# danieljfarrell/pvtrace

Measured on AMD Instinct MI355X. Metric: photons/sec on 5x5x1 cm Lumogen-F-Red LSC, higher is better.
Workload: dtype f64

## Files before the change

include/pvtrace_hip.h:

```cpp
#ifndef PVTRACE_HIP_H
#define PVTRACE_HIP_H

#include <stdint.h>

#ifdef __cplusplus
extern "C" {
#endif

#define PVT_ABI_VERSION 13

#define PVT_MAX_NODES 128
#define PVT_MAX_RECORDERS 256
#define PVT_MAX_HITS 512

enum {
    PVT_EV_GENERATE = 0, PVT_EV_REFLECT = 1, PVT_EV_TRANSMIT = 2, PVT_EV_ABSORB = 3,
    PVT_EV_NONRADIATIVE = 4, PVT_EV_SCATTER = 5, PVT_EV_EMIT = 6, PVT_EV_EXIT = 7,
    PVT_EV_REACT = 8, PVT_EV_KILL = 9
};
enum { PVT_GEOM_BOX = 0, PVT_GEOM_SPHERE = 1, PVT_GEOM_CYLINDER = 2, PVT_GEOM_MESH = 3 };
enum { PVT_SURF_FRESNEL = 0, PVT_SURF_NULL = 1 };
enum { PVT_COMP_ABSORBER = 0, PVT_COMP_SCATTERER = 1, PVT_COMP_LUMINOPHORE = 2, PVT_COMP_REACTOR = 3 };
enum { PVT_PHASE_ISOTROPIC = 0, PVT_PHASE_HG = 1, PVT_PHASE_CONE = 2,
       PVT_PHASE_LAMBERTIAN = 3,
// ... 213 lines not shown
    double* direction;
    double* normal;
    double* wavelength;
    double* travelled;
    double* duration;
} PvtEventLog;

typedef struct PvtEventRecords {
    int32_t* counts;
    uint64_t* rows;
} PvtEventRecords;

typedef struct PvtScene PvtScene;

int pvt_abi_version(void);
const char* pvt_last_error(void);
int pvt_device_count(void);

int pvt_scene_create(const PvtSceneTables* tables, int device, PvtScene** out);
int pvt_scene_create_ex(const PvtSceneTables* tables, const PvtIndexTables* index_tables, int device, PvtScene** out);
int pvt_scene_create_phase(const PvtSceneTables* tables, const PvtIndexTables* index_tables,
                           const PvtPhaseTables* phase_tables, int device, PvtScene** out);
int pvt_scene_create_rough(const PvtSceneTables* tables, const PvtIndexTables* index_tables,
                           const PvtPhaseTables* phase_tables, const PvtSurfaceTables* surface_tables, int device,
                           PvtScene** out);
int pvt_scene_create_field(const PvtSceneTables* tables, const PvtIndexTables* index_tables,
                           const PvtPhaseTables* phase_tables, const PvtSurfaceTables* surface_tables,
                           const PvtFieldTables* field_tables, int device, PvtScene** out);
int pvt_scene_create_maps(const PvtSceneTables* tables, const PvtIndexTables* index_tables,
                          const PvtPhaseTables* phase_tables, const PvtSurfaceTables* surface_tables,
                          const PvtFieldTables* field_tables, const PvtMapTables* map_tables, int device, PvtScene** out);
int64_t pvt_scene_map_slots(const PvtScene* scene);
int pvt_scene_set_emitter(PvtScene* scene, const PvtEmitterTables* emitter);
void pvt_scene_destroy(PvtScene* scene);

int pvt_trace_device(PvtScene* scene, const PvtRays* rays, const PvtTraceParams* params,
                     const PvtTallies* tallies, const PvtEventLog* log, void* stream);

int pvt_trace_device_records(PvtScene* scene, const PvtRays* rays, const PvtTraceParams* params,
                             const PvtTallies* tallies, const PvtEventRecords* records, void* stream);

int pvt_scene_carry_pending(PvtScene* scene, void* stream);
int pvt_scene_carry_discard(PvtScene* scene, void* stream);
int pvt_scene_trim(PvtScene* scene);

int pvt_unpack_records_device(const PvtEventRecords* records, int64_t n_recorded, int32_t max_events,
                              const PvtEventLog* out, int prefill, void* stream);

int pvt_trace_bundle(const PvtSceneTables* tables, const PvtEmitterTables* emitter,
                     const PvtRays* rays, const PvtTraceParams* params,
                     const PvtTallies* tallies, const PvtEventLog* log, int device,
                     double* kernel_ms);

void pvt_release_cached_memory(void);

int pvt_trace_bundle_multi(const PvtSceneTables* tables, const PvtEmitterTables* emitter,
                           const PvtRays* rays, const PvtTraceParams* params,
                           const PvtTallies* tallies, const PvtEventLog* log,
                           const int* devices, int n_devices, double* kernel_ms);

int pvt_last_multi_reduce(void);

int pvt_shard_range(int64_t n_rays, int shard, int n_shards, int64_t align, int64_t* start, int64_t* stop);

int pvt_emit_device(PvtScene* scene, const PvtTraceParams* params, double* position,
                    double* direction, double* wavelength, void* stream);

int pvt_selftest_math(int fn, const double* x_host, double* y_host, int64_t n, int device);

int pvt_scene_counters(PvtScene* scene, uint64_t* out, int reset);

int pvt_scene_clock(PvtScene* scene, uint64_t* out);

int pvt_scene_launch_span(PvtScene* scene, void* stream, uint64_t* out);

int pvt_scene_launch_info(PvtScene* scene, int32_t* grid, int32_t* block, int32_t* lds_bytes);

enum { PVT_VARIANT_LEAN = 0, PVT_VARIANT_W4 = 1, PVT_VARIANT_GRID = 2, PVT_VARIANT_ROUGH = 3, PVT_VARIANT_MESH = 4 };
int pvt_scene_variant(PvtScene* scene);
int pvt_scene_lean_check(const PvtSceneTables* tables, const PvtIndexTables* index_tables, const PvtPhaseTables* phase_tables,
                         const PvtSurfaceTables* surface_tables, const PvtFieldTables* field_tables,
                         const PvtMapTables* map_tables, int32_t* lean);

int pvt_mesh_bvh_check(const PvtSceneTables* tables, int32_t node, int32_t* n_bvh_nodes,
                       int32_t* n_leaves, int32_t* depth);

int pvt_node_grid_plan(const PvtSceneTables* tables, int32_t* dims, double* lo, double* cell, double* guard,
                       int32_t* odd, uint64_t* masks, int64_t masks_cap);

#ifdef __cplusplus
}
#endif
#endif
```

pvtrace_amd/csrc/pvt_scene_pack.h:

```cpp
#pragma once

namespace {

double cosine_threshold(double crit) {
    if (!(crit < INFINITY)) return -INFINITY;
    auto beyond = [&](double c) { return pvt_acos(c) > crit; };
    if (!beyond(0.0)) return -INFINITY;
    if (beyond(1.0)) return NAN;
    auto bits = [](double v) { uint64_t u; std::memcpy(&u, &v, 8); return u; };
    auto from = [](uint64_t u) { double v; std::memcpy(&v, &u, 8); return v; };
    uint64_t lo = bits(0.0), hi = bits(1.0);
    while (hi - lo > 1) {
        const uint64_t mid = lo + (hi - lo) / 2;
        if (beyond(from(mid))) lo = mid; else hi = mid;
    }
    for (uint64_t k = 1; k <= 1024; k++) {
        if (lo >= k && !beyond(from(lo - k))) return NAN;
        if (hi + k <= bits(1.0) && beyond(from(hi + k))) return NAN;
    }
    return from(hi);
}

bool dev_switch(const char* name) {
    if (!getenv(name)) return false;
// ... 194 lines not shown
                const int n0 = g->n[a];
                int pick = n0;
                for (int v = std::max(1, n0 / 2); v <= std::min(64, 2 * n0 + 1); v++) {
                    if (v == n0) continue;
                    int dims[3] = {g->n[0], g->n[1], g->n[2]};
                    dims[a] = v;
                    if ((long long)dims[0] * dims[1] * dims[2] > kMaxCells) break;
                    const double p = price(dims);
                    if (p < best * 0.98) { best = p; pick = v; }
                }
                g->n[a] = pick;
            }
    }
    g->words = W;
    g->guard = dev_switch("PVT_GRID_DEV_GUARD") ? -1e30 : m;
    file_nodes(g->n, g->cell, g->masks);
    return true;
}

double even_rcp(const double* xs, const double* ys, int n) {
    if (n < 2) return NAN;
    const double w = xs[1] - xs[0];
    if (!(w > 1e-100 && w < 1e100)) return NAN;
    for (int i = 1; i + 1 < n; i++) if (xs[i + 1] - xs[i] != w) return NAN;
    for (int i = 0; i < n; i++) {
        if (ys[i] == 0.0 && std::signbit(ys[i])) return NAN;
        if (!(std::fabs(ys[i]) < 1e100)) return NAN;
        if (i > 0 && ys[i] != ys[i - 1] && std::fabs(ys[i] - ys[i - 1]) < 1e-100) return NAN;
    }
    return 1.0 / w;
}

double even_w(const double* xs, int n, double rcp) {
    if (!(rcp == rcp) || n < 2 || n > (1 << 24)) return NAN;
    const double w = xs[1] - xs[0];
    auto grid = [&](int i) { volatile double prod = (double)i * w; volatile double at = xs[0] + prod; return (double)at; };
    for (int i = 0; i < n; i++)
        if (grid(i) != xs[i]) return NAN;
    auto lands = [&](double x, int want) {
        volatile double diff = x - xs[0];
        volatile double quot = diff * rcp;
        int i = (int)quot;
        i = i < 0 ? 0 : (i > n - 2 ? n - 2 : i);
        double xlo = grid(i);
        if (x < xlo) { i -= 1; xlo = grid(i); }
        double xhi = grid(i + 1);
        if (!(x < xhi)) { i += 1; xlo = xhi; xhi = grid(i + 1); }
        return i == want && xlo <= x && x < xhi;
    };
    for (int i = 0; i < n; i++) {
        const double below = std::nextafter(xs[i], -INFINITY), above = std::nextafter(xs[i], INFINITY);
        if (i > 0 && !lands(below, i - 1)) return NAN;
        if (i > 0 && i < n - 1 && !lands(xs[i], i)) return NAN;
        if (i < n - 1 && !lands(above, i)) return NAN;
    }
    return w;
}

double build_guide(const double* xs, int n, int* guide) {
    if (n < 2 || !(xs[n - 1] > xs[0])) return 0.0;
    const int Kb = n - 1;
    int i = 0;
    for (int b = 0; b <= Kb; b++) {
        const double edge = xs[0] + (double)b * ((xs[n - 1] - xs[0]) / (double)Kb);
        while (i + 1 <= n - 2 && xs[i + 1] <= edge) i++;
        guide[b] = i;
    }
    return (double)Kb / (xs[n - 1] - xs[0]);
}

struct PackedScene {
    Lay lay{};
    std::vector<double> gd;
    std::vector<int> gi;
    int nd_small = 0, ni_small = 0, n_ctab = 0, n_rtab = 0, n_ptab = 0, lazy_root = 0;
    int rough_d = -1;
    std::vector<double> fd;
    std::vector<double> md;
    long long map_slots = 0;
    double lazy_k = 0.0;
    bool exit_observed = false, fuse_exit = false, grid = false, hist_reads_position = false;
    bool lean_ok = false;
    bool lean_even = false;
    int grid_dims[3] = {0, 0, 0};
    std::vector<pvt::BvhNode> bvh_nodes;
    std::vector<pvt::MeshTri> bvh_tris;
    std::vector<int> bvh_roots;
};

int validate_tables(const PvtSceneTables* t, const PvtIndexTables* x, const PvtPhaseTables* ph, const PvtSurfaceTables* rs,
                    const PvtFieldTables* fr, const PvtMapTables* mp) {
    const int N = t->n_nodes, C = t->n_components, R = t->n_recorders, H = t->n_hists, K = t->n_coatings;
    if (t->root_id < 0 || t->root_id >= N) return fail(PVT_ERR_INVALID, "root node out of range");
    for (int n = 0; n < N; n++) {
        const int g = t->geom_type[n];
        if (g < PVT_GEOM_BOX || g > PVT_GEOM_MESH) return fail(PVT_ERR_INVALID, "unknown geometry type");
        if (g != PVT_GEOM_MESH) continue;
        if (!t->mesh_face_start || !t->mesh_face_count || !t->mesh_vertices || !t->mesh_faces || !t->mesh_normals)
            return fail(PVT_ERR_INVALID, "mesh node without mesh tables");
        const long long f0 = t->mesh_face_start[n], fc = t->mesh_face_count[n];
        if (fc <= 0 || f0 < 0 || f0 + fc > t->n_mesh_faces) return fail(PVT_ERR_INVALID, "mesh face range out of bounds");
        if (t->n_mesh_faces >= (1 << 27)) return fail(PVT_ERR_INVALID, "more than 2^27 mesh faces in one scene");
        for (long long k = 3 * f0; k < 3 * (f0 + fc); k++)
            if (t->mesh_faces[k] < 0 || t->mesh_faces[k] >= t->n_mesh_vertices)
                return fail(PVT_ERR_INVALID, "mesh face indexes a missing vertex");
    }
    if (K > 0 && t->n_coat_tables != 0) {
        const int NT = t->n_coat_tables;
        if (NT < 0 || !t->coat_table || !t->ctab_nw || !t->ctab_na || !t->ctab_wl_start || !t->ctab_angle_start ||
            !t->ctab_value_start || !t->ctab_wavelength || !t->ctab_angle || !t->ctab_value)
            return fail(PVT_ERR_INVALID, "coating tables: missing arrays");
        long long total = 0;
        for (int j = 0; j < NT; j++) {
            const long long nw = t->ctab_nw[j], na = t->ctab_na[j];
            const long long w0 = t->ctab_wl_start[j], a0 = t->ctab_angle_start[j], v0 = t->ctab_value_start[j];
            if (nw < 1 || na < 1 || w0 < 0 || a0 < 0 || v0 < 0 || w0 + nw > t->n_ctab_wavelength ||
                a0 + na > t->n_ctab_angle || v0 + nw * na > t->n_ctab_value)
                return fail(PVT_ERR_INVALID, "coating tables: axis or value range out of bounds");
            for (long long i = 0; i < nw; i++)
                if (!std::isfinite(t->ctab_wavelength[w0 + i]) || (i > 0 && !(t->ctab_wavelength[w0 + i] > t->ctab_wavelength[w0 + i - 1])))
                    return fail(PVT_ERR_INVALID, "coating tables: wavelengths must be finite and strictly increasing");
            for (long long i = 0; i < na; i++)
                if (!(t->ctab_angle[a0 + i] >= 0.0 && t->ctab_angle[a0 + i] <= 90.0) || (i > 0 && !(t->ctab_angle[a0 + i] > t->ctab_angle[a0 + i - 1])))
                    return fail(PVT_ERR_INVALID, "coating tables: angles must be strictly increasing, in [0, 90] degrees");
            for (long long i = 0; i < nw * na; i++)
                if (!(t->ctab_value[v0 + i] >= 0.0 && t->ctab_value[v0 + i] <= 1.0))
                    return fail(PVT_ERR_INVALID, "coating tables: values must be in [0, 1]");
            total += nw + na + nw * na;
        }
        if (total > (1ll << 27)) return fail(PVT_ERR_INVALID, "coating tables: more than 2^27 doubles");
        for (int k = 0; k < K; k++)
            if (t->coat_table[k] < -1 || t->coat_table[k] >= NT) return fail(PVT_ERR_INVALID, "coating row names a missing table");
    }
    for (int n = 0; n < N; n++) {
        const double v = t->refractive_index[n];
        if (!(std::isfinite(v) && v > 1e-100 && v < 1e100)) return fail(PVT_ERR_INVALID, "refractive indices must be finite and positive");
    }
    if (x && x->n_tables != 0) {
        const int NT = x->n_tables;
        if (NT < 0 || !x->node_table || !x->table_n || !x->table_start || !x->wavelength || !x->value)
            return fail(PVT_ERR_INVALID, "index tables: missing arrays");
        for (int n = 0; n < N; n++)
            if (x->node_table[n] < -1 || x->node_table[n] >= NT) return fail(PVT_ERR_INVALID, "index tables: node names a missing table");
        long long total = 0;
        for (int j = 0; j < NT; j++) {
            const long long np = x->table_n[j], p0 = x->table_start[j];
            if (np < 1 || p0 < 0 || p0 + np > x->n_points) return fail(PVT_ERR_INVALID, "index tables: point range out of bounds");
            for (long long i = 0; i < np; i++)
                if (!std::isfinite(x->wavelength[p0 + i]) || (i > 0 && !(x->wavelength[p0 + i] > x->wavelength[p0 + i - 1])))
                    return fail(PVT_ERR_INVALID, "index tables: wavelengths must be finite and strictly increasing");
            for (long long i = 0; i < np; i++) {
                const double v = x->value[p0 + i];
                if (!(std::isfinite(v) && v > 1e-100 && v < 1e100)) return fail(PVT_ERR_INVALID, "index tables: values must be finite and positive, in (1e-100, 1e100)");
            }
            total += 2 * np;
        }
        if (total > (1ll << 27)) return fail(PVT_ERR_INVALID, "index tables: more than 2^27 doubles");
    }
    const int NP = ph ? ph->n_tables : 0;
    if (NP < 0 || (NP > 0 && (!ph->comp_table || !ph->table_nw || !ph->table_nmu || !ph->wl_start || !ph->mu_start ||
                              !ph->cdf_start || !ph->wavelength || !ph->mu || !ph->cdf)))
        return fail(PVT_ERR_INVALID, "phase tables: missing arrays");
    for (int c = 0; c < C; c++) {
        const bool tagged = t->comp_phase_type[c] == PVT_PHASE_TABLE;
        if (tagged && NP == 0)
            return fail(PVT_ERR_INVALID, "a component has a tabulated phase function (PVT_PHASE_TABLE): pass its tables to pvt_scene_create_phase");
// ... 592 lines not shown
        for (int n = 0; n < N && inside; n++) {
            if (n == root) continue;
            const double* l2w = t->local_to_world + n * 16;
            const double* gp = t->geom_params + n * 4;
            double radius;
            switch (t->geom_type[n]) {
                case PVT_GEOM_BOX: radius = 0.5 * std::sqrt(gp[0] * gp[0] + gp[1] * gp[1] + gp[2] * gp[2]); break;
                case PVT_GEOM_SPHERE: radius = gp[0]; break;
                case PVT_GEOM_CYLINDER: radius = std::sqrt(gp[1] * gp[1] + 0.25 * gp[0] * gp[0]); break;
                default: radius = INFINITY; break;
            }
            radius *= 1.0 + 1e-12;
            double c[3];
            for (int a = 0; a < 3; a++)
                c[a] = w2l[a * 4] * l2w[3] + w2l[a * 4 + 1] * l2w[7] + w2l[a * 4 + 2] * l2w[11] + w2l[a * 4 + 3];
            if (box) {
                for (int a = 0; a < 3; a++)
                    if (!(0.5 * rp[a] - std::fabs(c[a]) - radius > margin)) inside = false;
            } else {
                if (!(rp[0] - std::sqrt(c[0] * c[0] + c[1] * c[1] + c[2] * c[2]) - radius > margin)) inside = false;
            }
        }
        if (inside) {
            p->lazy_root = box ? 1 : 2;
            p->lazy_k = box ? 0.0 : 1.0 / (2.0 * rp[0]);
        }
    }
    if (p->lazy_root && N == 2 && !getenv("PVT_NO_FUSED_EXIT")) {
        const int child = 1 - root;
        bool ok = t->geom_type[child] == PVT_GEOM_BOX && unrotated(t, child) && t->comp_count[root] == 0;
        for (int r = 0; r < R; r++)
            if (t->rec_node[r] == root) ok = false;
        p->fuse_exit = ok;
    }
}

void prove_lean(const PvtSceneTables* t, PackedScene* p) {
    const Lay& lay = p->lay;
    const std::vector<double>& gd = p->gd;
    const std::vector<int>& gi = p->gi;
    const int N = t->n_nodes, R = t->n_recorders;
    bool all_even = true;
    auto nearly_even = [&](int at, int n) {
        const double x0 = gd[(size_t)at], step = (gd[(size_t)at + n - 1] - x0) / (double)(n - 1);
        if (!(step > 0.0) || !std::isfinite(step)) return false;
        for (int i = 0; i < n; i++)
            if (!(std::fabs(gd[(size_t)at + i] - (x0 + (double)i * step)) <= 1e-9 * step)) return false;
        return true;
    };
    auto grid_kind = [&](int at, int n, double w) { return (n == 1 || w == w) ? 2 : (nearly_even(at, n) ? 1 : 0); };
    bool ok = t->n_coatings == 0 && p->n_ctab == 0 && p->n_rtab == 0 && p->n_ptab == 0 && p->rough_d < 0 && p->fd.empty() &&
              p->md.empty() && p->bvh_nodes.empty() && !p->grid && lay.by_node == 1 && R <= 64;
    for (int n = 0; n < N && ok; n++) {
        unsigned long long bits;
        std::memcpy(&bits, &gd[(size_t)n * ND + ND_BITS], 8);
        const bool ident = (bits & 1ull) != 0;
        const int geom = (int)(((unsigned int)bits >> 8) & 0xffu), rot_class = (int)(unsigned int)(bits >> 32);
        const int* q = gi.data() + n * NI;
        const bool shape_ok = geom == PVT_GEOM_BOX || (geom == PVT_GEOM_SPHERE && n == t->root_id);
        if (!ident || !shape_ok || rot_class != 0 || q[NI_KCOUNT] != 0 || q[NI_CCOUNT] > 2) ok = false;
        for (int k = 0; k < q[NI_CCOUNT] && ok; k++) {
            const int* ci = gi.data() + lay.comp_i + (q[NI_CREC] + k) * CI;
            const double* cd = gd.data() + lay.comp_d + (q[NI_CREC] + k) * CD;
            const bool luminophore = ci[CI_TYPE] == PVT_COMP_LUMINOPHORE;
            if (!luminophore && ci[CI_TYPE] != PVT_COMP_ABSORBER) ok = false;
            if (ci[CI_PHASE] != PVT_PHASE_ISOTROPIC) ok = false;
            const int ka = ci[CI_ABS_HIST] != 0 ? 0 : grid_kind(ci[CI_ABS_X], ci[CI_ABS_N], cd[CD_ABS_W]);
            const int ke = !luminophore ? 2 : (ci[CI_EMS_HIST] != 0 ? 0 : grid_kind(ci[CI_EMS_X], ci[CI_EMS_N], cd[CD_EMS_W]));
            if (ka == 0 || ke == 0) ok = false;
            if (ka != 2 || ke != 2) all_even = false;
        }
    }
    for (int block = 0; block < N * 7 && ok; block++) {
        const int* rec = gi.data() + lay.cand_i + block * 8;
        for (int b = 0; b < 6; b++)
            if (rec[2 + b] >= 0 && !(rec[2 + b] & kRecPlain)) ok = false;
        for (int j = 0; j < rec[1]; j++)
            if (!(gi[(size_t)lay.cand_list + rec[0] + j] & kRecPlain)) ok = false;
    }
    p->lean_ok = ok;
    p->lean_even = ok && all_even;
}

void pack_fields(const PvtSceneTables* t, const PvtFieldTables* fr, PackedScene* p) {
    p->fd.clear();
    if (!fr || fr->n_nodes == 0) return;
    const int N = t->n_nodes;
    bool any = false;
    for (int n = 0; n < N; n++) any = any || fr->node_field[n] >= 0;
    if (!any) return;
    std::vector<double>& fd = p->fd;
    fd.assign((size_t)N, -1.0);
    for (int n = 0; n < N; n++) {
        const int f = fr->node_field[n];
        if (f < 0) continue;
        fd[(size_t)n] = (double)fd.size();
        const size_t at = fd.size();
        fd.resize(at + kFrComp + (size_t)t->comp_count[n], 0.0);
        double* r = fd.data() + at;
        for (int a = 0; a < 3; a++) {
            const double lo = fr->field_lower[f * 3 + a], hi = fr->field_upper[f * 3 + a];
            const int na = fr->field_shape[f * 3 + a];
            r[kFrShape + a] = (double)na;
            r[kFrLower + a] = lo;
            r[kFrH + a] = (hi - lo) / (double)na;
            for (int c = 0; c < 3; c++) r[kFrRot + a * 3 + c] = t->world_to_local[n * 16 + a * 4 + c];
            r[kFrT + a] = t->world_to_local[n * 16 + a * 4 + 3];
        }
    }
    std::vector<long long> value_at((size_t)fr->n_values, -1);
    for (int n = 0; n < N; n++) {
        if (fr->node_field[n] < 0) continue;
        const size_t at = (size_t)fd[(size_t)n];
        for (int k = 0; k < t->comp_count[n]; k++) {
            const int v = fr->comp_values[t->comp_start[n] + k];
            if (value_at[(size_t)v] < 0) {
                value_at[(size_t)v] = (long long)fd.size();
                const double* src = fr->values + fr->values_start[v];
                fd.insert(fd.end(), src, src + fr->values_count[v]);
            }
            fd[at + kFrComp + (size_t)k] = (double)value_at[(size_t)v];
        }
    }
}

void pack_maps(const PvtSceneTables* t, const PvtMapTables* mp, PackedScene* p) {
    p->md.clear();
    p->map_slots = 0;
    if (!mp || mp->n_nodes == 0 || mp->n_maps == 0) return;
    const int N = t->n_nodes;
    std::vector<double>& md = p->md;
    md.assign((size_t)N, -1.0);
    for (int n = 0; n < N; n++) {
        const int count = mp->node_map_count[n];
        if (count == 0) continue;
        md[(size_t)n] = (double)md.size();
        const size_t at = md.size();
        md.resize(at + kMnRec + (size_t)count * kMr, 0.0);
        double* r = md.data() + at;
        r[kMnCount] = (double)count;
        for (int a = 0; a < 3; a++) {
            for (int c = 0; c < 3; c++) r[kMnRot + a * 3 + c] = t->world_to_local[n * 16 + a * 4 + c];
            r[kMnT + a] = t->world_to_local[n * 16 + a * 4 + 3];
        }
        for (int k = 0; k < count; k++) {
            const int m = mp->node_map_start[n] + k;
            double* q = r + kMnRec + k * kMr;
            q[kMrKind] = (double)mp->map_kind[m];
            q[kMrComp] = (double)mp->map_component[m];
            for (int a = 0; a < 3; a++) {
                q[kMrShape + a] = (double)mp->map_shape[m * 3 + a];
                q[kMrLower + a] = mp->map_lower[m * 3 + a];
                q[kMrH + a] = mp->map_h[m * 3 + a];
            }
            q[kMrNw] = (double)mp->map_nw[m];
            q[kMrWlo] = mp->map_wl_start[m];
            q[kMrWhi] = mp->map_wl_stop[m];
            q[kMrOff] = (double)mp->map_offset[m];
        }
    }
    p->map_slots = mp->map_slots;
}

int pack_scene(const PvtSceneTables* t, const PvtIndexTables* x, const PvtPhaseTables* ph, const PvtSurfaceTables* rs,
               const PvtFieldTables* fr, const PvtMapTables* mp, PackedScene* p) {
    int rc = validate_tables(t, x, ph, rs, fr, mp);
    if (rc != PVT_OK) return rc;
    const Classes classes = classify_nodes(t, x);
    Spectra spectra = pool_spectra(t);
    const Records records = component_records(t, ph, spectra, classes.by_node);
    NodeGrid grid;
    p->grid = plan_node_grid(t, &grid);
    for (int a = 0; a < 3; a++) p->grid_dims[a] = p->grid ? grid.n[a] : 0;
    p->n_ctab = t->n_coatings > 0 ? t->n_coat_tables : 0;
    p->n_rtab = 0;
    if (x)
        for (int n = 0; n < t->n_nodes; n++)
            if (x->n_tables > 0 && x->node_table[n] >= 0) p->n_rtab = x->n_tables;
    p->n_ptab = 0;
    if (ph)
        for (int c = 0; c < t->n_components; c++)
            if (ph->n_tables > 0 && ph->comp_table[c] >= 0) p->n_ptab = ph->n_tables;
    p->rough_d = -1;
    if (rs && rs->n_nodes > 0)
        for (int n = 0; n < t->n_nodes; n++)
            if (rs->node_roughness[n] > 0.0) p->rough_d = 0;
    std::vector<int> rtab_at, ptab_at;
    const std::vector<int> ctab_at = lay_out(t, x, ph, classes, spectra, records, grid, p, &rtab_at, &ptab_at);
    rc = fill(t, x, ph, rs, classes, spectra, records, grid, ctab_at, rtab_at, ptab_at, p);
    if (rc != PVT_OK) return rc;
    pack_fields(t, fr, p);
    pack_maps(t, mp, p);
    prove_shortcuts(t, p);
    prove_lean(t, p);
    return PVT_OK;
}

}
```

pvtrace_amd/csrc/pvt_trace.hip:

```cpp
#include <hip/hip_runtime.h>

#include <cmath>
#include <cstdio>
#include <cstdlib>
#include <algorithm>
#include <atomic>
#include <cstring>
#include <chrono>
#include <dlfcn.h>
#include <string>
#include <thread>
#include <mutex>
#include <vector>

#include "../../include/pvtrace_hip.h"
#include "pvt_math.h"
#include "pvt_bvh.h"

#include "pvt_trace_kernel.h"

namespace {

thread_local std::string g_error;

// ... 1 lines not shown
    g_error = msg;
    return code;
}
#define HIP_TRY(expr)                                                                     \
    do {                                                                                  \
        hipError_t e_ = (expr);                                                           \
        if (e_ != hipSuccess)                                                             \
            return fail(PVT_ERR_HIP, std::string(#expr) + ": " + hipGetErrorString(e_)); \
    } while (0)

#if PVT_TIMELINE
constexpr int kTlLaunches = 48, kTlWgs = 1024;
constexpr size_t kTlBytes = (size_t)kTlLaunches * kTlWgs * kWaves * 8 * 8;
unsigned long long* g_timeline = nullptr;
int g_tl_launch = 0, g_tl_grid[kTlLaunches] = {0};
long long g_tl_n[kTlLaunches] = {0};
void timeline_dump();
#endif

template <class T>
int push(std::vector<T>& blob, const T* src, size_t n) {
    int at = (int)blob.size();
    if (n && src) blob.insert(blob.end(), src, src + n);
    return at;
}

}

#include "pvt_scene_pack.h"

struct PvtScene {
    int device = 0;
    Lay lay{};
    EmitOff eoff{};
    int nd = 0, ni = 0;
    int nd_small = 0, ni_small = 0;
    int n_nodes = 0, root = 0, n_rec = 0, total_bins = 0, n_coat = 0, n_ctab = 0, n_rtab = 0, n_lights = 0;
    int rough_d = -1;
    double* d_fd = nullptr;
    double* d_md = nullptr;
    long long map_slots = 0;
    double* d_gd = nullptr;
    int* d_gi = nullptr;
    double* d_ed = nullptr;
    int* d_ei = nullptr;
    pvt::BvhNode* d_bvh = nullptr;
    pvt::MeshTri* d_tris = nullptr;
    pvt::BvhNode* d_bvh_top = nullptr;
    int top_n = 0;
    int meshq = 0;
    unsigned int* d_set_cursor = nullptr;
    unsigned long long* d_counters = nullptr;
    unsigned long long* d_stamp = nullptr;
    unsigned int* d_cursor = nullptr;
    std::mutex slot_mutex;
    std::vector<hipStream_t> slot_of;
    std::vector<unsigned long long*> stage;
    std::vector<size_t> stage_bytes;
    size_t stage_limit = (size_t)1 << 30;
    struct Carry {
        unsigned long long* buf[2] = {nullptr, nullptr};
        int parity = 0;
        int phase = 0;
        bool pending = false;
        long long bound = 0;
        int maxsteps = 0, emit_method = 0;
    };
    std::vector<Carry> carry;
    std::vector<double*> emit_pool;
    std::vector<size_t> emit_pool_bytes;
    unsigned int carry_cap = 0;
    int num_cu = 0;
    int last_grid = 0, last_lds = 0;
    size_t lds_limit = 0;
    int lazy_root = 0;
    double lazy_k = 0.0;
    bool exit_observed = false;
    bool grid = false;
    int grid_dims[3] = {0, 0, 0};
    bool fuse_exit = false;
    bool hist_reads_position = false;
    bool lean_ok = false;
    bool lean_even = false;
    int last_variant = -1;
};

extern "C" {

int pvt_abi_version(void) { return PVT_ABI_VERSION; }
const char* pvt_last_error(void) { return g_error.c_str(); }

int pvt_device_count(void) {
    int n = 0;
    if (hipGetDeviceCount(&n) != hipSuccess) return 0;
    return n;
}

int pvt_scene_set_emitter(PvtScene* s, const PvtEmitterTables* e) {
    if (!s || !e || e->n_lights <= 0) return fail(PVT_ERR_INVALID, "bad emitter");
    HIP_TRY(hipSetDevice(s->device));
    std::vector<double> ed;
    std::vector<int> ei;
    EmitOff o{};
    const int Lt = e->n_lights;
    o.wl_value = push(ed, e->wl_value, Lt);
    o.pos_param = push(ed, e->pos_param, (size_t)Lt * 3);
    o.dir_param = push(ed, e->dir_param, Lt);
    o.l2w = push(ed, e->light_to_world, (size_t)Lt * 16);
    o.spec_x = push(ed, e->spec_x, e->n_spec);
    o.spec_cdf = push(ed, e->spec_cdf, e->n_spec);
    o.wl_type = push(ei, e->wl_type, Lt);
    o.wl_spec_start = push(ei, e->wl_spec_start, Lt);
    o.wl_spec_n = push(ei, e->wl_spec_n, Lt);
    o.pos_type = push(ei, e->pos_type, Lt);
    o.dir_type = push(ei, e->dir_type, Lt);
    ed.push_back(0.0);
    ei.push_back(0);
    if (s->d_ed) { (void)hipFree(s->d_ed); s->d_ed = nullptr; }
    if (s->d_ei) { (void)hipFree(s->d_ei); s->d_ei = nullptr; }
    HIP_TRY(hipMalloc(&s->d_ed, ed.size() * sizeof(double)));
    HIP_TRY(hipMalloc(&s->d_ei, ei.size() * sizeof(int)));
    HIP_TRY(hipMemcpy(s->d_ed, ed.data(), ed.size() * sizeof(double), hipMemcpyHostToDevice));
    HIP_TRY(hipMemcpy(s->d_ei, ei.data(), ei.size() * sizeof(int), hipMemcpyHostToDevice));
    s->eoff = o;
    s->n_lights = Lt;
    return PVT_OK;
}

void pvt_scene_destroy(PvtScene* s) {
    if (!s) return;
#if PVT_TIMELINE
    timeline_dump();
#endif
    (void)hipSetDevice(s->device);
    if (s->d_gd) (void)hipFree(s->d_gd);
    if (s->d_fd) (void)hipFree(s->d_fd);
    if (s->d_md) (void)hipFree(s->d_md);
    if (s->d_gi) (void)hipFree(s->d_gi);
    if (s->d_ed) (void)hipFree(s->d_ed);
    if (s->d_ei) (void)hipFree(s->d_ei);
    if (s->d_cursor) (void)hipFree(s->d_cursor);
    if (s->d_set_cursor) (void)hipFree(s->d_set_cursor);
    if (s->d_counters) (void)hipFree(s->d_counters);
    if (s->d_stamp) (void)hipFree(s->d_stamp);
    if (s->d_bvh) (void)hipFree(s->d_bvh);
    if (s->d_bvh_top) (void)hipFree(s->d_bvh_top);
    if (s->d_tris) (void)hipFree(s->d_tris);
    for (auto* b : s->stage) if (b) (void)hipFree(b);
    for (auto& c : s->carry) for (auto* b : c.buf) if (b) (void)hipFree(b);
    for (auto* b : s->emit_pool) if (b) (void)hipFree(b);
    delete s;
}

}

namespace {

KArgs base_args(const PvtScene* s, const PvtTraceParams* p) {
    KArgs a{};
    a.gd = s->d_gd; a.gi = s->d_gi; a.ed = s->d_ed; a.ei = s->d_ei;
    a.bvh = s->d_bvh; a.tris = s->d_tris;
    a.lay = s->lay; a.eoff = s->eoff;
    a.nd = s->nd; a.ni = s->ni;
    a.nd_lds = 0; a.ni_lds = 0;
    a.n_nodes = s->n_nodes; a.root = s->root; a.n_rec = s->n_rec; a.total_bins = s->total_bins;
    a.n_coat = s->n_coat; a.n_ctab = s->n_ctab; a.n_rtab = s->n_rtab; a.n_lights = s->n_lights;
    a.rough_d = s->rough_d;
    a.fd = s->d_fd;
    a.md = s->d_md;
    a.n_rays = (unsigned int)p->n_rays;
    a.cursor = s->d_cursor;
    a.counters = s->d_counters;
    a.seed = p->seed + p->ray_offset;
    a.emit_seed = p->emit_seed;
    a.ray_offset = p->ray_offset;
    a.maxsteps = p->maxsteps; a.max_events = p->max_events; a.emit_method = p->emit_method;
    a.record_every = p->record_every;
    return a;
}

#ifndef PVT_DEV_VARIANTS
#define PVT_DEV_VARIANTS 0
#endif
template <bool RECORD, int TAB_LDS, int SEENW>
hipError_t launch_rough_variant(bool emit, int grid, size_t lds, hipStream_t st, const KArgs& a) {
#if PVT_DEV_VARIANTS
    (void)emit; (void)grid; (void)lds; (void)st; (void)a;
    return hipErrorNotSupported;
#else
    const bool mesh = a.bvh != nullptr;
    if constexpr (TAB_LDS == 1) {
        if (a.lay.grid_d >= 0 && !mesh) {
            if (emit) hipLaunchKernelGGL((trace_kernel_rough_grid<RECORD, SEENW, true>), dim3(grid), dim3(kBlock), lds, st, a);
            else hipLaunchKernelGGL((trace_kernel_rough_grid<RECORD, SEENW, false>), dim3(grid), dim3(kBlock), lds, st, a);
            return hipGetLastError();
        }
    }
    constexpr int MESH_TAB = TAB_LDS == 2 ? 0 : TAB_LDS;
    if (mesh && TAB_LDS == 2) return hipErrorNotSupported;
    if (emit) {
        if (mesh) hipLaunchKernelGGL((trace_kernel_rough<RECORD, MESH_TAB, SEENW, true, true>), dim3(grid), dim3(kBlock), lds, st, a);
        else hipLaunchKernelGGL((trace_kernel_rough_w4<RECORD, TAB_LDS, SEENW, true>), dim3(grid), dim3(kBlock), lds, st, a);
    } else {
        if (mesh) hipLaunchKernelGGL((trace_kernel_rough<RECORD, MESH_TAB, SEENW, false, true>), dim3(grid), dim3(kBlock), lds, st, a);
        else hipLaunchKernelGGL((trace_kernel_rough_w4<RECORD, TAB_LDS, SEENW, false>), dim3(grid), dim3(kBlock), lds, st, a);
    }
    return hipGetLastError();
#endif
}

int variant_of(const PvtScene* s, bool tab_lds) {
    if (s->rough_d >= 0 || s->d_fd || s->d_md) return PVT_VARIANT_ROUGH;
    if (s->d_bvh) return PVT_VARIANT_MESH;
    if (tab_lds && s->lay.grid_d >= 0) return PVT_VARIANT_GRID;
    if (tab_lds && s->lean_ok && s->n_rec <= 64) return PVT_VARIANT_LEAN;
    return PVT_VARIANT_W4;
}

template <bool RECORD>
hipError_t launch_lean_variant(bool even, bool emit, int grid, size_t lds, hipStream_t st, const KArgs& a) {
#if PVT_DEV_VARIANTS
    if (emit || RECORD) return hipErrorNotSupported;
    if (even) hipLaunchKernelGGL((trace_kernel_lean_w4<false, false, true>), dim3(grid), dim3(kBlock), lds, st, a);
    else hipLaunchKernelGGL((trace_kernel_lean_w4<false, false, false>), dim3(grid), dim3(kBlock), lds, st, a);
#else
    if (even) {
        if (emit) hipLaunchKernelGGL((trace_kernel_lean_w4<RECORD, true, true>), dim3(grid), dim3(kBlock), lds, st, a);
        else hipLaunchKernelGGL((trace_kernel_lean_w4<RECORD, false, true>), dim3(grid), dim3(kBlock), lds, st, a);
    } else {
        if (emit) hipLaunchKernelGGL((trace_kernel_lean_w4<RECORD, true, false>), dim3(grid), dim3(kBlock), lds, st, a);
        else hipLaunchKernelGGL((trace_kernel_lean_w4<RECORD, false, false>), dim3(grid), dim3(kBlock), lds, st, a);
    }
#endif
    return hipGetLastError();
}

template <bool RECORD, int TAB_LDS, int SEENW>
hipError_t launch_variant(bool emit, int grid, size_t lds, hipStream_t st, const KArgs& a) {
    if (a.rough_d >= 0 || a.fd != nullptr || a.md != nullptr) return launch_rough_variant<RECORD, TAB_LDS, SEENW>(emit, grid, lds, st, a);
    const bool mesh = a.bvh != nullptr;
    if constexpr (TAB_LDS == 1 && (!PVT_DEV_VARIANTS || SEENW == 1) && PVT_DEV_VARIANTS != 2) {
        if (a.lay.grid_d >= 0 && !mesh && (!PVT_DEV_VARIANTS || !emit)) {
            if (emit && !PVT_DEV_VARIANTS) hipLaunchKernelGGL((trace_kernel_grid<RECORD, SEENW, !PVT_DEV_VARIANTS>), dim3(grid), dim3(kBlock), lds, st, a);
            else hipLaunchKernelGGL((trace_kernel_grid<RECORD, SEENW, false>), dim3(grid), dim3(kBlock), lds, st, a);
            return hipGetLastError();
        }
    }
#if PVT_DEV_VARIANTS == 2
    if (emit || !mesh || TAB_LDS != 1 || SEENW != 1) return hipErrorNotSupported;
    if constexpr (TAB_LDS == 1 && SEENW == 1) hipLaunchKernelGGL((trace_kernel<RECORD, 1, 1, false, true>), dim3(grid), dim3(kBlock), lds, st, a);
#elif PVT_DEV_VARIANTS
    if (emit || mesh || TAB_LDS != 1 || SEENW != 1) return hipErrorNotSupported;
    if constexpr (TAB_LDS == 1 && SEENW == 1) {
        if constexpr (RECORD) hipLaunchKernelGGL((trace_kernel_w4<true, 1, 1, false>), dim3(grid), dim3(kBlock), lds, st, a);
        else hipLaunchKernelGGL((trace_kernel_w4<false, 1, 1, false>), dim3(grid), dim3(kBlock), lds, st, a);
    }
#else
    constexpr int MESH_TAB = TAB_LDS == 2 ? 0 : TAB_LDS;
    if (mesh && TAB_LDS == 2) return hipErrorNotSupported;
    if (emit) {
        if (mesh) hipLaunchKernelGGL((trace_kernel<RECORD, MESH_TAB, SEENW, true, true>), dim3(grid), dim3(kBlock), lds, st, a);
        else if constexpr (RECORD) hipLaunchKernelGGL((trace_kernel_w4<true, TAB_LDS, SEENW, true>), dim3(grid), dim3(kBlock), lds, st, a);
        else hipLaunchKernelGGL((trace_kernel_w4<false, TAB_LDS, SEENW, true>), dim3(grid), dim3(kBlock), lds, st, a);
    } else {
        if (mesh) hipLaunchKernelGGL((trace_kernel<RECORD, MESH_TAB, SEENW, false, true>), dim3(grid), dim3(kBlock), lds, st, a);
        else if constexpr (RECORD) hipLaunchKernelGGL((trace_kernel_w4<true, TAB_LDS, SEENW, false>), dim3(grid), dim3(kBlock), lds, st, a);
        else hipLaunchKernelGGL((trace_kernel_w4<false, TAB_LDS, SEENW, false>), dim3(grid), dim3(kBlock), lds, st, a);
    }
#endif
    return hipGetLastError();
}

template <bool RECORD, int TAB_LDS>
hipError_t launch_seen(int n_rec, int lean, bool emit, int grid, size_t lds, hipStream_t st, const KArgs& a) {
    if constexpr (TAB_LDS == 1 && PVT_DEV_VARIANTS != 2) {
        if (lean) return launch_lean_variant<RECORD>(lean == kLeanEven, emit, grid, lds, st, a);
    }
    if (n_rec <= 64) return launch_variant<RECORD, TAB_LDS, 1>(emit, grid, lds, st, a);
    return launch_variant<RECORD, TAB_LDS, 4>(emit, grid, lds, st, a);
}

}

namespace {

int slot_of_stream(PvtScene* s, hipStream_t st) {
    std::lock_guard<std::mutex> lock(s->slot_mutex);
    size_t slot = 0;
    while (slot < s->slot_of.size() && s->slot_of[slot] != st) slot++;
    if (slot == s->slot_of.size()) {
        if (slot >= (size_t)kCursorSlots) return -1;
        s->slot_of.push_back(st);
        s->stage.push_back(nullptr);
        s->stage_bytes.push_back(0);
        s->carry.emplace_back();
        s->emit_pool.push_back(nullptr);
        s->emit_pool_bytes.push_back(0);
    }
    return (int)slot;
}

int check_trace_args(PvtScene* s, const PvtRays* rays, const PvtTraceParams* p, const PvtTallies* tl) {
    if (!s || !p || !tl) return fail(PVT_ERR_INVALID, "null argument");
    if (p->n_rays < 0 || p->n_rays > 0x7fffffffLL)
        return fail(PVT_ERR_INVALID, "n_rays must fit in 31 bits per bundle");
    if (p->max_events < 2 && p->record_every > 0) return fail(PVT_ERR_INVALID, "max_events must be >= 2");
    if (!rays && !s->d_ed && p->n_rays > 0) return fail(PVT_ERR_INVALID, "no rays and no emitter");
    if ((p->flags & PVT_FLAG_CARRY_OUT) && (p->record_every > 0 || p->tally_bundle > 0))
        return fail(PVT_ERR_INVALID, "PVT_FLAG_CARRY_OUT is for plain tally launches (record_every == 0, no tally sets)");
    if (p->tally_bundle > 0 && p->record_every > 0) return fail(PVT_ERR_INVALID, "tally_bundle needs record_every == 0");
    return PVT_OK;
}

struct LdsPlan { size_t bytes; bool tab_lds, small_lds; int bins_in_lds, xslots, tq_pos; bool ok; };
LdsPlan plan_lds(const PvtScene* s, bool record) {
    LdsPlan lp{0, false, false, 0, 0, 0, true};
    const size_t reserved = (size_t)s->meshq * kBlock * 4 + (size_t)s->top_n * sizeof(pvt::BvhNode);
    const size_t acc_bytes = (size_t)s->n_rec * (8 * 8 + 8) + (size_t)((s->n_rec + 1) & ~1) * 4 + CTL_WORDS * 4;
    const size_t tab_bytes = (size_t)s->nd * 8 + (size_t)((s->ni + 1) & ~1) * 4;
    const size_t bins_bytes = ((size_t)s->total_bins * 4 + 7) & ~(size_t)7;
    const size_t lds_limit = s->lds_limit - reserved;
    const size_t budget = (64 * 1024 < s->lds_limit ? 64 * 1024 : s->lds_limit) - reserved;
    lp.tq_pos = s->hist_reads_position ? 1 : 0;
    const size_t tq_bytes = (size_t)kWaves * kTallyQ * ((lp.tq_pos ? 7 : 4) * 8 + 4);
    if (acc_bytes + tq_bytes > lds_limit) { lp.ok = false; return lp; }
    const char* force = getenv("PVT_TABLES");
    lp.tab_lds = acc_bytes + tq_bytes + tab_bytes <= budget && !force;
    const size_t small_bytes = (size_t)s->nd_small * 8 + (size_t)((s->ni_small + 1) & ~1) * 4;
    lp.small_lds = !lp.tab_lds && s->meshq == 0 && acc_bytes + tq_bytes + small_bytes <= 40 * 1024 && acc_bytes + tq_bytes + small_bytes <= budget &&
                   !(force && force[0] == 'g');
    size_t lds = acc_bytes + tq_bytes + (lp.tab_lds ? tab_bytes : lp.small_lds ? small_bytes : 0);
    lp.bins_in_lds = (lds + bins_bytes <= budget) ? 1 : 0;
    if (lp.bins_in_lds) lds += bins_bytes;
    const size_t xw = 14 + (s->n_rec <= 64 ? 1 : 4) + (record ? 1 : 0);
    const size_t xbytes = (size_t)kXSlots * xw * 8;
    if (s->meshq == 0 && lds + xbytes <= 40 * 1024 && lds + xbytes <= lds_limit) {
        lp.xslots = kXSlots;
        lds += xbytes;
    }
    lp.bytes = (lds + 15) & ~(size_t)15;
    return lp;
}

int trace_launch(PvtScene* s, const PvtRays* rays, const PvtTraceParams* p, const PvtTallies* tl,
                 unsigned long long* log_rows, int* log_counts, hipStream_t st) {
    const int slot = slot_of_stream(s, st);
    if (slot < 0)
        return fail(PVT_ERR_INVALID, "more than 64 HIP streams are tracing this scene; create one scene per group of streams");
    PvtScene::Carry& carry = s->carry[(size_t)slot];
    const bool carry_in = carry.pending;
    if (p->n_rays == 0 && !carry_in) return PVT_OK;
    if (carry_in && (p->record_every > 0 || p->tally_bundle > 0))
        return fail(PVT_ERR_INVALID, "photons parked by the previous launch on this stream (PVT_FLAG_CARRY_OUT) are waiting: "
                                     "finish them with a plain tally launch (n_rays may be 0) first");
    if (carry_in && (p->maxsteps != carry.maxsteps || p->emit_method != carry.emit_method))
        return fail(PVT_ERR_INVALID, "photons parked by the previous launch on this stream were traced with maxsteps " +
                                     std::to_string(carry.maxsteps) + ", emit_method " + std::to_string(carry.emit_method) +
                                     "; this launch asks for " + std::to_string(p->maxsteps) + ", " + std::to_string(p->emit_method) +
// ... 41 lines not shown
    static unsigned long long* g_stats = nullptr;
    if (!g_stats) (void)hipMalloc(&g_stats, 256);
    (void)hipMemsetAsync(g_stats, 0, 256, st);
    a.cursor = reinterpret_cast<unsigned int*>(g_stats);
    a.cursor_next = nullptr;
#endif

    const LdsPlan lp = plan_lds(s, record);
    if (!lp.ok) return fail(PVT_ERR_INVALID, "recorder accumulators exceed LDS");
    a.tq_pos = lp.tq_pos;
    a.bins_in_lds = lp.bins_in_lds;
    a.xslots = lp.xslots;
    const bool tab_lds = lp.tab_lds;
    if (lp.small_lds) { a.nd_lds = s->nd_small; a.ni_lds = s->ni_small; }
    size_t lds = lp.bytes;
    a.meshq_off = -1;
    a.top_off = 0; a.top_n = 0; a.bvh_top = nullptr;
    if (a.bvh) {
        a.meshq_off = (int)lds;
        lds += (size_t)s->meshq * kBlock * 4;
        a.top_off = (int)lds; a.top_n = s->top_n; a.bvh_top = s->d_bvh_top;
        lds += (size_t)s->top_n * sizeof(pvt::BvhNode);
        if (lds > s->lds_limit) return fail(PVT_ERR_INVALID, "mesh staging exceeds LDS");
    }

    long long blocks_for_rays = (p->n_rays + (carry_in ? carry.bound : 0) + kBlock - 1) / kBlock;
    double per_cu = p->workgroups_per_cu > 0 ? (double)p->workgroups_per_cu : 4.0;
    long long grid = (long long)((double)s->num_cu * per_cu);
    if (grid > blocks_for_rays) grid = blocks_for_rays;
    if (grid < 1) grid = 1;
    if (carry_in && grid * kBlock < carry.bound) grid = (carry.bound + kBlock - 1) / kBlock;
    if (n_sets) {
        long long per_set = grid / n_sets;
        const long long for_rays = (p->tally_bundle + kBlock - 1) / kBlock;
        if (per_set > for_rays) per_set = for_rays;
        if (per_set < 1) per_set = 1;
        grid = per_set * n_sets;
        a.set_size = (unsigned int)p->tally_bundle;
        a.wgs_per_set = (int)per_set;
        a.set_stride_i = p->tally_stride_i64;
        a.set_stride_d = p->tally_stride_f64;
    }
    s->last_grid = (int)grid;
    s->last_lds = (int)lds;

    bool carry_out = (p->flags & PVT_FLAG_CARRY_OUT) != 0 && !record && !n_sets;
    if (carry_in || carry_out) {
        if (!s->carry_cap) s->carry_cap = (unsigned int)((long long)s->num_cu * 4 * kBlock);
        if (grid * kBlock > (long long)s->carry_cap) carry_out = false;
        const size_t bytes = (size_t)s->carry_cap * kCarryStride * 8;
        for (int q = 0; q < 2; q++)
            if (!carry.buf[q]) HIP_TRY(hipMalloc(&carry.buf[q], bytes));
        a.carry_cap = s->carry_cap;
        a.carry_in = carry.buf[carry.parity ^ 1];
        a.carry_out = carry.buf[carry.parity];
        a.carry_in_count = blocks + 4 * ((carry.phase + 2) % 3) + 2;
        a.carry_flags = (carry_in ? 1 : 0) | (carry_out ? 2 : 0);
    }

#if PVT_TIMELINE
    if (getenv("PVT_TIMELINE_FILE")) {
        if (!g_timeline) { (void)hipMalloc(&g_timeline, kTlBytes); (void)hipMemset(g_timeline, 0, kTlBytes); }
        const int from = getenv("PVT_TIMELINE_FROM") ? atoi(getenv("PVT_TIMELINE_FROM")) : 0;
        const int k = g_tl_launch++ - from;
        if (k >= 0 && k < kTlLaunches && grid <= kTlWgs) {
            a.timeline = g_timeline + (size_t)k * kTlWgs * kWaves * 8;
            g_tl_grid[k] = (int)grid; g_tl_n[k] = p->n_rays;
        }
    }
#endif
    const bool emit = rays == nullptr && s->d_ed != nullptr;
    if (emit) {
        const size_t need = (size_t)grid * kWaves * 7 * 64 * sizeof(double);
        if (s->emit_pool_bytes[(size_t)slot] < need) {
            if (s->emit_pool[(size_t)slot]) { HIP_TRY(hipStreamSynchronize(st)); (void)hipFree(s->emit_pool[(size_t)slot]); s->emit_pool[(size_t)slot] = nullptr; s->emit_pool_bytes[(size_t)slot] = 0; }
            const size_t bytes = need < ((size_t)s->num_cu * 4 * kWaves * 7 * 64 * sizeof(double)) ? (size_t)s->num_cu * 4 * kWaves * 7 * 64 * sizeof(double) : need;
            HIP_TRY(hipMalloc(&s->emit_pool[(size_t)slot], bytes));
            s->emit_pool_bytes[(size_t)slot] = bytes;
        }
        a.emit_pool = s->emit_pool[(size_t)slot];
    }
    hipError_t e;
    s->last_variant = variant_of(s, tab_lds);
    const int lean = s->last_variant != PVT_VARIANT_LEAN ? kLeanOff : (s->lean_even ? kLeanEven : kLeanSearched);
    if (record) {
        e = tab_lds ? launch_seen<true, 1>(s->n_rec, lean, emit, (int)grid, lds, st, a)
            : lp.small_lds ? launch_seen<true, 2>(s->n_rec, lean, emit, (int)grid, lds, st, a)
                           : launch_seen<true, 0>(s->n_rec, lean, emit, (int)grid, lds, st, a);
    } else {
        e = tab_lds ? launch_seen<false, 1>(s->n_rec, lean, emit, (int)grid, lds, st, a)
            : lp.small_lds ? launch_seen<false, 2>(s->n_rec, lean, emit, (int)grid, lds, st, a)
                           : launch_seen<false, 0>(s->n_rec, lean, emit, (int)grid, lds, st, a);
    }
    if (e != hipSuccess) return fail(PVT_ERR_HIP, std::string("trace_kernel launch: ") + hipGetErrorString(e));
    if (!n_sets) carry.phase = (carry.phase + 1) % 3;
    if (carry_in || carry_out) {
        carry.pending = carry_out;
        carry.bound = carry_out ? grid * kBlock : 0;
        carry.maxsteps = p->maxsteps;
        carry.emit_method = p->emit_method;
        carry.parity ^= 1;
    }
#if PVT_STATS
    {
        unsigned long long c[32];
        (void)hipStreamSynchronize(st);
        (void)hipMemcpy(c, a.cursor, 256, hipMemcpyDeviceToHost);
        fprintf(stderr, "[pvt stats] waves %llu  wave-iterations %llu (drain %llu)  lane-steps %llu (drain %llu)  "
                "mean live lanes/iter %.1f (bulk %.1f, drain %.1f)  iters/wave %.1f (drain %.1f)\n",
                c[5], c[1], c[3], c[2], c[4], (double)c[2] / c[1], (double)(c[2] - c[4]) / (double)(c[1] - c[3] + 1e-9),
                (double)c[4] / (c[3] + 1e-9), (double)c[1] / c[5], (double)c[3] / c[5]);
        fprintf(stderr, "[pvt stats] solo-wave cycles: refill %llu nodes %llu absorb %llu frame %llu trig %llu surface %llu tally %llu (solo waves %llu)\n",
                c[9], c[10], c[11], c[12], c[13], c[14], c[15], c[16]);
        const double bi = (double)(c[1] - c[3]) + 1e-9;
        if (a.lay.grid_d >= 0)
            fprintf(stderr, "[pvt stats] grid walk per wave-iteration: cell rounds %.2f  node-test trips %.2f  (lanes per trip %.1f, lanes per cell round %.1f)\n",
                    (double)c[25] / c[1], (double)c[26] / c[1], (double)c[27] / (c[26] + 1e-9), (double)c[28] / (c[25] + 1e-9));
        if (a.bvh)
            fprintf(stderr, "[pvt stats] mesh walk per wave-iteration: box trips %.2f (lanes per trip %.1f)  triangle trips %.2f (lanes per trip %.1f);  per lane-step: boxes %.2f triangles %.2f\n",
                    (double)c[25] / c[1], (double)c[26] / (c[25] + 1e-9), (double)c[27] / c[1], (double)c[28] / (c[27] + 1e-9),
                    (double)c[26] / c[2], (double)c[28] / c[2]);
        fprintf(stderr, "[pvt stats] bulk lanes/iteration: live %.1f absorbed %.1f re-emitted %.1f surface %.1f exit %.1f terminal-selector %.1f terminal %.1f\n",
                c[17] / bi, c[18] / bi, c[19] / bi, c[20] / bi, c[21] / bi, c[22] / bi, c[23] / bi);
    }
#endif
    return PVT_OK;
}

#if PVT_TIMELINE
void timeline_dump() {
    const char* path = getenv("PVT_TIMELINE_FILE");
    if (!path || !g_timeline) return;
    (void)hipDeviceSynchronize();
    std::vector<unsigned long long> host(kTlBytes / 8);
    (void)hipMemcpy(host.data(), g_timeline, kTlBytes, hipMemcpyDeviceToHost);
    if (FILE* fp = fopen(path, "wb")) {
        for (int k = 0; k < kTlLaunches; k++) {
            if (!g_tl_grid[k]) continue;
            unsigned long long head[4] = {0xABCDull, (unsigned long long)k, (unsigned long long)g_tl_grid[k], (unsigned long long)g_tl_n[k]};
            fwrite(head, 8, 4, fp);
            fwrite(host.data() + (size_t)k * kTlWgs * kWaves * 8, 8, (size_t)g_tl_grid[k] * kWaves * 8, fp);
        }
        fclose(fp);
    }
}
#endif

int unpack_launch(const unsigned long long* rows, const int* counts, long long n_recorded, int max_events,
                  const PvtEventLog* out, bool prefill, hipStream_t st) {
    if (n_recorded <= 0) return PVT_OK;
    const int rays_per_block = max_events >= kBlock ? 1 : kBlock / max_events;
    const long long gx = (n_recorded + rays_per_block - 1) / rays_per_block;
    const int gy = rays_per_block > 1 ? 1 : (max_events + kBlock - 1) / kBlock;
    if (gx > 0x7fffffffLL) return fail(PVT_ERR_INVALID, "too many recorded rays for one unpack launch");
    hipLaunchKernelGGL(unpack_log_kernel, dim3((unsigned)gx, (unsigned)gy), dim3(kBlock), 0, st, rows, counts, *out,
                       n_recorded, max_events, rays_per_block, prefill ? 1 : 0);
    hipError_t e = hipGetLastError();
    if (e != hipSuccess) return fail(PVT_ERR_HIP, std::string("unpack_log_kernel launch: ") + hipGetErrorString(e));
    return PVT_OK;
}

}

extern "C" {

int pvt_scene_create(const PvtSceneTables* t, int device, PvtScene** out) {
    return pvt_scene_create_ex(t, nullptr, device, out);
}

int pvt_scene_create_ex(const PvtSceneTables* t, const PvtIndexTables* x, int device, PvtScene** out) {
    return pvt_scene_create_phase(t, x, nullptr, device, out);
}

int pvt_scene_create_phase(const PvtSceneTables* t, const PvtIndexTables* x, const PvtPhaseTables* ph, int device, PvtScene** out) {
    return pvt_scene_create_rough(t, x, ph, nullptr, device, out);
}

int pvt_scene_create_rough(const PvtSceneTables* t, const PvtIndexTables* x, const PvtPhaseTables* ph,
                           const PvtSurfaceTables* rs, int device, PvtScene** out) {
    return pvt_scene_create_field(t, x, ph, rs, nullptr, device, out);
}

int pvt_scene_create_field(const PvtSceneTables* t, const PvtIndexTables* x, const PvtPhaseTables* ph,
                           const PvtSurfaceTables* rs, const PvtFieldTables* fr, int device, PvtScene** out) {
    return pvt_scene_create_maps(t, x, ph, rs, fr, nullptr, device, out);
}

int64_t pvt_scene_map_slots(const PvtScene* s) { return s ? (int64_t)s->map_slots : 0; }

int pvt_scene_create_maps(const PvtSceneTables* t, const PvtIndexTables* x, const PvtPhaseTables* ph,
                          const PvtSurfaceTables* rs, const PvtFieldTables* fr, const PvtMapTables* mp, int device,
                          PvtScene** out) {
    if (!t || !out) return fail(PVT_ERR_INVALID, "null argument");
    if (t->n_nodes <= 0) return fail(PVT_ERR_INVALID, "scene has no nodes");
    if (t->n_nodes > PVT_MAX_NODES) return fail(PVT_ERR_TOO_MANY_NODES, "more than 128 geometry nodes");
    if (t->n_recorders > PVT_MAX_RECORDERS) return fail(PVT_ERR_INVALID, "more than 256 recorders");
    if (pvt_device_count() <= device) return fail(PVT_ERR_NO_DEVICE, "no such HIP device");
    HIP_TRY(hipSetDevice(device));
    PackedScene packed;
    const int rc = pack_scene(t, x, ph, rs, fr, mp, &packed);
    if (rc != PVT_OK) return rc;

    struct Owner {
        PvtScene* p;
        ~Owner() { if (p) pvt_scene_destroy(p); }
    } owner{new PvtScene()};
    PvtScene* s = owner.p;
    s->stage.reserve(kCursorSlots); s->stage_bytes.reserve(kCursorSlots); s->carry.reserve(kCursorSlots);
    s->emit_pool.reserve(kCursorSlots); s->emit_pool_bytes.reserve(kCursorSlots);
    s->device = device;
    s->lay = packed.lay;
    s->nd = (int)packed.gd.size(); s->ni = (int)packed.gi.size();
    s->nd_small = packed.nd_small; s->ni_small = packed.ni_small;
    s->n_nodes = t->n_nodes; s->root = t->root_id; s->n_rec = t->n_recorders;
    s->total_bins = t->total_bins; s->n_coat = t->n_coatings; s->n_ctab = packed.n_ctab; s->n_rtab = packed.n_rtab;
    s->rough_d = packed.rough_d;
    s->lazy_root = packed.lazy_root; s->lazy_k = packed.lazy_k;
    s->exit_observed = packed.exit_observed; s->fuse_exit = packed.fuse_exit; s->hist_reads_position = packed.hist_reads_position;
    s->grid = packed.grid;
    s->lean_ok = packed.lean_ok && !getenv("PVT_NO_LEAN");
    s->lean_even = s->lean_ok && packed.lean_even;
    for (int a = 0; a < 3; a++) s->grid_dims[a] = packed.grid_dims[a];
    hipDeviceProp_t prop;
    HIP_TRY(hipGetDeviceProperties(&prop, device));
    s->num_cu = prop.multiProcessorCount;
    s->lds_limit = prop.sharedMemPerBlock;
    if (const char* env = getenv("PVT_STAGE_BYTES")) s->stage_limit = (size_t)atoll(env);
    HIP_TRY(hipMalloc(&s->d_gd, packed.gd.size() * sizeof(double)));
    HIP_TRY(hipMalloc(&s->d_gi, packed.gi.size() * sizeof(int)));
    HIP_TRY(hipMalloc(&s->d_cursor, 64 * kCursorSlots + 256));
    HIP_TRY(hipMemset(s->d_cursor, 0, 64 * kCursorSlots + 256));
    HIP_TRY(hipMalloc(&s->d_set_cursor, (size_t)kCursorSlots * kMaxSets * 4));
    HIP_TRY(hipMalloc(&s->d_counters, 64 * 8 * 8));
    HIP_TRY(hipMemset(s->d_counters, 0, 64 * 8 * 8));
    HIP_TRY(hipMalloc(&s->d_stamp, (size_t)kCursorSlots * 2 * 8));
    HIP_TRY(hipMemset(s->d_stamp, 0, (size_t)kCursorSlots * 2 * 8));
    if (!packed.bvh_nodes.empty()) {
        s->meshq = 1;
        for (int r : packed.bvh_roots)
            if (packed.bvh_nodes[r].skip - r > 16) s->meshq = kMeshQ;
        const LdsPlan tally = plan_lds(s, false), hist = plan_lds(s, true);
        const size_t other = (tally.bytes > hist.bytes ? tally.bytes : hist.bytes) + (size_t)s->meshq * kBlock * 4;
        const size_t per_wg = (size_t)39 * 1024 * 4 / kMeshWaves;
        size_t room = tally.ok && hist.ok && other < per_wg ? per_wg - other : 0;
        if (room > 32 * 1024) room = 32 * 1024;
        if (const char* env = getenv("PVT_MESH_TOP_BYTES")) {
            const size_t asked = (size_t)atoll(env);
            room = asked < room ? asked : room;
        }
        std::vector<pvt::BvhNode> top;
        pvt::stage_top(packed.bvh_nodes, packed.bvh_roots, room / sizeof(pvt::BvhNode), top);
        s->top_n = (int)top.size();
        const LdsPlan tally2 = plan_lds(s, false), hist2 = plan_lds(s, true);
        const size_t with_top = (size_t)s->meshq * kBlock * 4 + (size_t)s->top_n * sizeof(pvt::BvhNode);
        if (tally2.ok != tally.ok || hist2.ok != hist.ok || tally2.tab_lds != tally.tab_lds || hist2.tab_lds != hist.tab_lds ||
            tally2.bytes + with_top > s->lds_limit || hist2.bytes + with_top > s->lds_limit)
            return fail(PVT_ERR_INVALID, "internal: the LDS plan of a mesh scene changed when the copy of its trees' top levels was added");
        if (s->top_n > 0) {
            HIP_TRY(hipMalloc(&s->d_bvh_top, top.size() * sizeof(pvt::BvhNode)));
            HIP_TRY(hipMemcpy(s->d_bvh_top, top.data(), top.size() * sizeof(pvt::BvhNode), hipMemcpyHostToDevice));
        }
        packed.bvh_nodes.push_back(pvt::BvhNode{});
        HIP_TRY(hipMalloc(&s->d_bvh, packed.bvh_nodes.size() * sizeof(pvt::BvhNode)));
        HIP_TRY(hipMalloc(&s->d_tris, packed.bvh_tris.size() * sizeof(pvt::MeshTri)));
        HIP_TRY(hipMemcpy(s->d_bvh, packed.bvh_nodes.data(), packed.bvh_nodes.size() * sizeof(pvt::BvhNode), hipMemcpyHostToDevice));
        HIP_TRY(hipMemcpy(s->d_tris, packed.bvh_tris.data(), packed.bvh_tris.size() * sizeof(pvt::MeshTri), hipMemcpyHostToDevice));
    }
    HIP_TRY(hipMemcpy(s->d_gd, packed.gd.data(), packed.gd.size() * sizeof(double), hipMemcpyHostToDevice));
    HIP_TRY(hipMemcpy(s->d_gi, packed.gi.data(), packed.gi.size() * sizeof(int), hipMemcpyHostToDevice));
    if (!packed.fd.empty()) {
        HIP_TRY(hipMalloc(&s->d_fd, packed.fd.size() * sizeof(double)));
        HIP_TRY(hipMemcpy(s->d_fd, packed.fd.data(), packed.fd.size() * sizeof(double), hipMemcpyHostToDevice));
    }
    if (!packed.md.empty()) {
        HIP_TRY(hipMalloc(&s->d_md, packed.md.size() * sizeof(double)));
        HIP_TRY(hipMemcpy(s->d_md, packed.md.data(), packed.md.size() * sizeof(double), hipMemcpyHostToDevice));
        s->map_slots = packed.map_slots;
    }
    owner.p = nullptr;
    *out = s;
    return PVT_OK;
}

int pvt_trace_device_records(PvtScene* s, const PvtRays* rays, const PvtTraceParams* p, const PvtTallies* tl,
                             const PvtEventRecords* rec, void* stream) {
    int rc = check_trace_args(s, rays, p, tl);
    if (rc != PVT_OK) return rc;
    if (p->record_every > 0 && (!rec || !rec->rows || !rec->counts))
        return fail(PVT_ERR_INVALID, "record_every > 0 needs event records");
    return trace_launch(s, rays, p, tl, rec ? reinterpret_cast<unsigned long long*>(rec->rows) : nullptr, rec ? rec->counts : nullptr,
                        reinterpret_cast<hipStream_t>(stream));
}

int pvt_scene_carry_pending(PvtScene* s, void* stream) {
    if (!s) return 0;
    std::lock_guard<std::mutex> lock(s->slot_mutex);
    for (size_t k = 0; k < s->slot_of.size(); k++)
        if (s->slot_of[k] == reinterpret_cast<hipStream_t>(stream)) return s->carry[k].pending ? 1 : 0;
    return 0;
}

int pvt_scene_carry_discard(PvtScene* s, void* stream) {
    if (!s) return fail(PVT_ERR_INVALID, "null scene");
    std::lock_guard<std::mutex> lock(s->slot_mutex);
// ... 98 lines not shown
    hipLaunchKernelGGL(emit_kernel, dim3(grid), dim3(kBlock), 0, reinterpret_cast<hipStream_t>(stream), a,
                       position, direction, wavelength);
    HIP_TRY(hipGetLastError());
    return PVT_OK;
}

int pvt_selftest_math(int fn, const double* x_host, double* y_host, int64_t n, int device) {
    if (!x_host || !y_host || n < 0) return fail(PVT_ERR_INVALID, "bad argument");
    if (n == 0) return PVT_OK;
    if (pvt_device_count() <= device) return fail(PVT_ERR_NO_DEVICE, "no such HIP device");
    HIP_TRY(hipSetDevice(device));
    double *dx = nullptr, *dy = nullptr;
    HIP_TRY(hipMalloc(&dx, (size_t)n * 8));
    HIP_TRY(hipMalloc(&dy, (size_t)n * 8));
    HIP_TRY(hipMemcpy(dx, x_host, (size_t)n * 8, hipMemcpyHostToDevice));
    hipLaunchKernelGGL(math_kernel, dim3((unsigned)((n + kBlock - 1) / kBlock)), dim3(kBlock), 0, nullptr, fn, dx, dy,
                       (long long)n);
    HIP_TRY(hipGetLastError());
    HIP_TRY(hipMemcpy(y_host, dy, (size_t)n * 8, hipMemcpyDeviceToHost));
    (void)hipFree(dx);
    (void)hipFree(dy);
    return PVT_OK;
}

int pvt_scene_counters(PvtScene* s, uint64_t* out, int reset) {
    if (!s || !out) return fail(PVT_ERR_INVALID, "null argument");
    HIP_TRY(hipSetDevice(s->device));
    unsigned long long rows[64 * 8];
    HIP_TRY(hipMemcpy(rows, s->d_counters, sizeof rows, hipMemcpyDeviceToHost));
    for (int k = 0; k < 4; k++) out[k] = 0;
    for (int r = 0; r < 64; r++)
        for (int k = 0; k < 4; k++) out[k] += rows[r * 8 + k];
    if (reset) HIP_TRY(hipMemset(s->d_counters, 0, sizeof rows));
    return PVT_OK;
}

int pvt_scene_clock(PvtScene* s, uint64_t* out) {
    if (!s || !out) return fail(PVT_ERR_INVALID, "null argument");
    HIP_TRY(hipSetDevice(s->device));
    unsigned long long rows[64 * 8];
    HIP_TRY(hipMemcpy(rows, s->d_counters, sizeof rows, hipMemcpyDeviceToHost));
    out[0] = out[1] = 0;
    for (int r = 0; r < 64; r++) { out[0] += rows[r * 8 + 4]; out[1] += rows[r * 8 + 5]; }
    return PVT_OK;
}

int pvt_scene_launch_span(PvtScene* s, void* stream, uint64_t* out) {
    if (!s || !out) return fail(PVT_ERR_INVALID, "null argument");
    HIP_TRY(hipSetDevice(s->device));
    out[0] = out[1] = 0;
    size_t k = 0;
    {
        std::lock_guard<std::mutex> lock(s->slot_mutex);
        while (k < s->slot_of.size() && s->slot_of[k] != reinterpret_cast<hipStream_t>(stream)) k++;
        if (k == s->slot_of.size()) return fail(PVT_ERR_INVALID, "no launch on this stream yet");
    }
    HIP_TRY(hipStreamSynchronize(reinterpret_cast<hipStream_t>(stream)));
    HIP_TRY(hipMemcpy(out, s->d_stamp + 2 * k, 16, hipMemcpyDeviceToHost));
    return PVT_OK;
}

int pvt_scene_launch_info(PvtScene* s, int32_t* grid, int32_t* block, int32_t* lds_bytes) {
    if (!s) return fail(PVT_ERR_INVALID, "null scene");
    if (grid) *grid = s->last_grid;
    if (block) *block = kBlock;
    if (lds_bytes) *lds_bytes = s->last_lds;
    return PVT_OK;
}

int pvt_scene_variant(PvtScene* s) {
    if (!s) return fail(PVT_ERR_INVALID, "null scene");
    if (s->last_variant >= 0) return s->last_variant;
    return variant_of(s, plan_lds(s, false).tab_lds);
}

int pvt_scene_lean_check(const PvtSceneTables* t, const PvtIndexTables* x, const PvtPhaseTables* ph, const PvtSurfaceTables* rs,
                         const PvtFieldTables* fr, const PvtMapTables* mp, int32_t* lean) {
    if (!t || !lean) return fail(PVT_ERR_INVALID, "null argument");
    if (t->n_nodes <= 0 || t->n_nodes > PVT_MAX_NODES || t->n_recorders > PVT_MAX_RECORDERS) return fail(PVT_ERR_INVALID, "bad argument");
    PackedScene packed;
    const int rc = pack_scene(t, x, ph, rs, fr, mp, &packed);
    if (rc != PVT_OK) return rc;
    *lean = packed.lean_ok ? (packed.lean_even ? 2 : 1) : 0;
    return PVT_OK;
}

int pvt_mesh_bvh_check(const PvtSceneTables* t, int32_t node, int32_t* n_bvh_nodes, int32_t* n_leaves,
                       int32_t* depth_out) {
    if (!t || node < 0 || node >= t->n_nodes || t->geom_type[node] != PVT_GEOM_MESH)
        return fail(PVT_ERR_INVALID, "not a mesh node");
    const int f0 = t->mesh_face_start[node], fc = t->mesh_face_count[node];
    if (fc <= 0 || f0 < 0 || f0 + fc > t->n_mesh_faces) return fail(PVT_ERR_INVALID, "mesh face range out of bounds");
    std::vector<pvt::BvhNode> nodes;
    std::vector<pvt::MeshTri> tris;
    double centre[3];
    const int root = pvt::BvhBuilder(t->mesh_vertices, t->mesh_faces, t->mesh_normals, nodes, tris).add_mesh(f0, fc, centre);
    if (root != 0 || nodes.size() < 2 || nodes[0].skip != (int)nodes.size()) return fail(PVT_ERR_INVALID, "root skip link");
    std::vector<int> seen(fc, 0);
    int leaves = 0, records = 0, max_depth = 0;
    struct Open { int id, parent, depth, skip; };
    std::vector<Open> todo{{0, -1, 1, (int)nodes.size()}};
    std::vector<char> visited(nodes.size(), 0);
    while (!todo.empty()) {
        const Open o = todo.back();
        todo.pop_back();
        if (o.id < 0 || o.id >= (int)nodes.size() || visited[o.id]++) return fail(PVT_ERR_INVALID, "child link out of range or shared");
        const pvt::BvhNode& b = nodes[o.id];
        records += 1;
        max_depth = std::max(max_depth, o.depth);
        if (b.skip != o.skip) return fail(PVT_ERR_INVALID, "skip link: a left child's is its sibling, a right child's its parent's");
        for (int a = 0; a < 3; a++) {
            if (!(b.lo[a] <= b.hi[a])) return fail(PVT_ERR_INVALID, "empty box");
            if (o.parent >= 0 && (b.lo[a] < nodes[o.parent].lo[a] || b.hi[a] > nodes[o.parent].hi[a]))
                return fail(PVT_ERR_INVALID, "child box not inside its parent");
        }
        if (b.link < 0) {
            leaves += 1;
            const int tri = b.link & pvt::kIndexMask;
            if (tri >= (int)tris.size()) return fail(PVT_ERR_INVALID, "triangle record out of range");
            const pvt::MeshTri& tr = tris[tri];
            const long long local = tr.face - f0;
            if (local < 0 || local >= fc || seen[local]++) return fail(PVT_ERR_INVALID, "face missing or duplicated");
            for (int c = 0; c < 3; c++)
                for (int a = 0; a < 3; a++) {
                    if (tr.v[3 * c + a] != t->mesh_vertices[3 * (size_t)t->mesh_faces[3 * (size_t)tr.face + c] + a])
                        return fail(PVT_ERR_INVALID, "gathered vertex differs from the table");
                    if (tr.v[3 * c + a] - centre[a] < b.lo[a] || tr.v[3 * c + a] - centre[a] > b.hi[a])
                        return fail(PVT_ERR_INVALID, "triangle outside its leaf box");
                }
        } else {
            const int c = b.link;
            if (c <= o.id || (c & 1) != 0) return fail(PVT_ERR_INVALID, "children not a pair on one 64-byte line after their parent");
            todo.push_back({c + 1, o.id, o.depth + 1, o.skip});
            todo.push_back({c, o.id, o.depth + 1, c + 1});
        }
    }
    for (int k = 0; k < fc; k++) if (seen[k] != 1) return fail(PVT_ERR_INVALID, "face missing from the tree");
    if (records + 1 != (int)nodes.size() || visited[1]) return fail(PVT_ERR_INVALID, "records outside the tree");
    auto replay = [](const std::vector<pvt::BvhNode>& plain, const std::vector<pvt::BvhNode>& staged,
                     const std::vector<pvt::BvhNode>& top, int root) -> const char* {
        const int end = plain[root].skip;
        std::vector<int> cursor_of((size_t)(end - root) + 1, -1);
        cursor_of[(size_t)(end - root)] = end;
        std::vector<int> order;
        int c = pvt::first_cursor(staged, root);
        for (int i = root; i != end; i = pvt::next_cursor(plain[i], true)) {
            if (c == end) return "staged walk ends early";
            if ((c & pvt::kTopFlag) ? (size_t)(c & pvt::kIndexMask) >= top.size() : (c < root || c >= end)) return "cursor out of range";
            if (cursor_of[(size_t)(i - root)] >= 0) return "plain walk visits a record twice";
            cursor_of[(size_t)(i - root)] = c;
            order.push_back(i);
            const pvt::BvhNode& rec = pvt::at_cursor(staged, top, c);
            for (int a = 0; a < 3; a++)
                if (rec.lo[a] != plain[i].lo[a] || rec.hi[a] != plain[i].hi[a]) return "staged walk out of order";
            if ((plain[i].link < 0) != (rec.link < 0) || (plain[i].link < 0 && rec.link != plain[i].link)) return "staged leaf differs";
            c = pvt::next_cursor(rec, true);
            if (order.size() > (size_t)(end - root)) return "plain walk does not end";
        }
        if (c != end) return "staged walk does not end at the tree's end";
        for (int i : order) {
            const pvt::BvhNode& rec = pvt::at_cursor(staged, top, cursor_of[(size_t)(i - root)]);
            if (pvt::next_cursor(rec, false) != cursor_of[(size_t)(plain[i].skip - root)]) return "staged skip link differs";
        }
        return nullptr;
    };
    for (size_t budget : {(size_t)3, (size_t)7, (size_t)64, (size_t)768, nodes.size()}) {
// ... 583 lines not shown
```

pvtrace_amd/csrc/pvt_trace_kernel.h:

```cpp
#pragma once
constexpr int kMeshWaves = 4;
#ifndef PVT_STATS
#define PVT_STATS 0
#endif
#ifndef PVT_TIMELINE
#define PVT_TIMELINE 0
#endif

namespace {

constexpr int kBlock = 256;
constexpr int kChunk = 64;
constexpr int kEndClaim = 64;
constexpr int kClaim = kChunk;
constexpr int kWaves = kBlock / 64;
constexpr int kCursorSlots = 64;
constexpr int kMaxSets = 1024;
constexpr int kRecPlain = 1 << 30;
constexpr int kTallyQ = 64;
constexpr int kXSlots = 72;
enum { CTL_EXHAUSTED = 0, CTL_DONE = 1, CTL_IN = 2, CTL_LIVE = 6, CTL_COUNT = 16, CTL_CLOCK = 22, CTL_WORDS = 26 };
constexpr double kEps = 2.220446049250313e-13;
constexpr double kAlphaZero = 1e-8;
constexpr double kCcm = 2.99792458e10;
// ... 112 lines not shown
    r.s2 = splitmix64(st);
    r.s3 = splitmix64(st);
}
__device__ __forceinline__ double rng_uniform(Rng& r) {
    unsigned long long result = r.s0 + r.s3;
    unsigned long long t = r.s1 << 17;
    r.s2 ^= r.s0;
    r.s3 ^= r.s1;
    r.s1 ^= r.s2;
    r.s0 ^= r.s3;
    r.s2 ^= t;
    r.s3 = (r.s3 << 45) | (r.s3 >> 19);
    const double hi = (double)(unsigned int)(result >> 32), lo = (double)(unsigned int)((unsigned int)result >> 11);
    return __builtin_fma(lo, 1.0 / 9007199254740992.0, hi * (1.0 / 4294967296.0));
}

__device__ __forceinline__ double div_normal(double x, double y) {
    double r = __builtin_amdgcn_rcp(y);
    double e = __builtin_fma(-y, r, 1.0);
    r = __builtin_fma(r, e, r);
    e = __builtin_fma(-y, r, 1.0);
    r = __builtin_fma(r, e, r);
    const double q = x * r;
    e = __builtin_fma(-y, q, x);
    return __builtin_fma(e, r, q);
}
__device__ __forceinline__ double sqrt_normal(double x) {
    const double y = __builtin_amdgcn_rsq(x);
    double g = x * y, h = y * 0.5;
    const double r = __builtin_fma(-h, g, 0.5);
    g = __builtin_fma(g, r, g);
    h = __builtin_fma(h, r, h);
    double d = __builtin_fma(-g, g, x);
    g = __builtin_fma(d, h, g);
    d = __builtin_fma(-g, g, x);
    g = __builtin_fma(d, h, g);
    return __builtin_amdgcn_class(x, 0x260) ? x : g;
}
__device__ __forceinline__ double sqrt1m2_normal(double c) { return sqrt_normal((1.0 - c) * (1.0 + c)); }
__device__ __forceinline__ double rcp_normal(double x) {
    double r = __builtin_amdgcn_rcp(x);
    double e = __builtin_fma(-x, r, 1.0);
    r = __builtin_fma(r, e, r);
    e = __builtin_fma(-x, r, 1.0);
    r = __builtin_fma(r, e, r);
    e = __builtin_fma(-x, r, 1.0);
    return __builtin_fma(e, r, r);
}

typedef const __attribute__((address_space(4))) double* CDoubles;
typedef const __attribute__((address_space(4))) int* CInts;

template <int TAB_LDS>
struct Tables {
    CDoubles gd;
    CInts gi;
    const double* ld;
    const int* li;
    const double* __restrict__ hd;
    const int* __restrict__ hi;
    __device__ __forceinline__ double du(int i) const { return gd[i]; }
    __device__ __forceinline__ int iu(int i) const { return gi[i]; }
    __device__ __forceinline__ double dv(int i) const { return TAB_LDS != 0 ? ld[i] : hd[i]; }
    __device__ __forceinline__ int iv(int i) const { return TAB_LDS != 0 ? li[i] : hi[i]; }
    __device__ __forceinline__ double sd(int i) const { return TAB_LDS == 1 ? ld[i] : hd[i]; }
    __device__ __forceinline__ int si(int i) const { return TAB_LDS == 1 ? li[i] : hi[i]; }
};

struct V3 {
    double x, y, z;
};
__device__ __forceinline__ double dot3(const V3& a, const V3& b) { return a.x * b.x + a.y * b.y + a.z * b.z; }

__device__ __forceinline__ double div_known(double x, double y, double z) {
    double q = x * z;
    double r = __builtin_fma(-q, y, x);
    q = __builtin_fma(r, z, q);
    r = __builtin_fma(-q, y, x);
    return __builtin_fma(r, z, q);
}
constexpr double kRcpCcm = 1.0 / kCcm;

enum { kInterpAny = 0, kInterpEven, kInterpByGuide, kInterpNoHist };
enum { kLeanOff = 0, kLeanSearched, kLeanEven };
template <int TAB_LDS, int KIND = kInterpAny>
__device__ __forceinline__ double interp_clamped(const Tables<TAB_LDS>& T, double x, int xs, int ys, int n,
                                                 int guide, double scale, int hist, double rcp,
                                                 double w = __builtin_nan(""), double yw = __builtin_nan("")) {
    auto end = [&](int i) { return T.sd(i); };
    if (n == 1) return end(ys);
    constexpr bool kAny = KIND == kInterpAny;
    constexpr bool kNoHist = KIND == kInterpNoHist;
    const bool even = KIND == kInterpEven || (kAny && !hist && w == w) || (kNoHist && w == w);
    const double x0 = end(xs), xl = even ? x0 + (double)(n - 1) * w : end(xs + n - 1);
    if (x <= x0) return end(ys);
    if ((kAny && hist) ? x > xl : x >= xl) return (KIND == kInterpByGuide || ((kAny || kNoHist) && yw == yw)) ? end(ys) + (double)(n - 1) * yw : end(ys + n - 1);
    if (even) {
        int i = (int)((x - x0) * rcp);
        double xlo = x0 + (double)i * w, xhi = x0 + (double)(i + 1) * w;
        if (__ballot(x < xlo || !(x < xhi)) != 0ull) {
            if (x < xlo) { i -= 1; xhi = xlo; xlo = x0 + (double)i * w; }
            else if (!(x < xhi)) { i += 1; xlo = xhi; xhi = x0 + (double)(i + 1) * w; }
        }
        const double ylo = T.sd(ys + i), yhi = T.sd(ys + i + 1);
        return ylo + div_known((yhi - ylo) * (x - xlo), xhi - xlo, rcp);
    }
    int b = (int)((x - x0) * scale);
    b = b < 0 ? 0 : (b > n - 2 ? n - 2 : b);
    int lo = T.si(guide + b), hi = T.si(guide + b + 1) + 1;
    if (hi > n - 1) hi = n - 1;
    double xlo = T.sd(xs + lo), xhi = T.sd(xs + hi);
    if (kAny && hist) {
        if (!(xlo < x)) lo = 0;
        if (!(x <= xhi)) hi = n - 1;
        while (hi - lo > 1) {
            const int mid = (lo + hi) >> 1;
            if (T.sd(xs + mid) < x) lo = mid; else hi = mid;
        }
        return T.sd(ys + hi);
    }
    if (__ballot(!(xlo <= x) || !(x < xhi)) != 0ull) {
        if (!(xlo <= x)) { lo = 0; xlo = x0; }
        if (!(x < xhi)) { hi = n - 1; xhi = xl; }
    }
    while (hi - lo > 1) {
        const int mid = (lo + hi) >> 1;
        const double xm = T.sd(xs + mid);
        if (xm <= x) { lo = mid; xlo = xm; } else { hi = mid; xhi = xm; }
    }
    double ylo, yhi;
    if (KIND == kInterpByGuide || ((kAny || kNoHist) && yw == yw)) {
        const double y0 = end(ys);
        ylo = y0 + (double)lo * yw; yhi = y0 + (double)hi * yw;
    } else {
        ylo = T.sd(ys + lo); yhi = T.sd(ys + hi);
    }
    if (xhi == xlo) return ylo;
    const double num = (yhi - ylo) * (x - xlo), width = xhi - xlo;
    return ylo + (rcp == rcp ? div_known(num, width, rcp) : num / width);
}
__device__ __forceinline__ void coat_bracket(const double* xs, int n, double x, int& lo, int& hi, double& t) {
    lo = 0; hi = 0; t = 0.0;
    if (!(x > xs[0])) return;
    if (!(x < xs[n - 1])) { lo = n - 1; hi = n - 1; return; }
    int a = 0, b = n - 1;
    while (b - a > 1) {
        const int m = (a + b) >> 1;
        if (xs[m] <= x) a = m; else b = m;
    }
    const double xa = xs[a];
    lo = a; hi = b; t = (x - xa) / (xs[b] - xa);
}
__device__ __forceinline__ double coat_table_r(const double* wls, int nw, const double* angs, int na, const double* vals,
                                               double wl, double c1) {
    int w0, w1, a0, a1;
    double tw, ta;
    coat_bracket(wls, nw, wl, w0, w1, tw);
    coat_bracket(angs, na, pvt_acos(c1), a0, a1, ta);
    const double* v0 = vals + a0 * nw;
    const double* v1 = vals + a1 * nw;
    const double p0 = v0[w0], r0 = p0 + tw * (v0[w1] - p0);
    const double p1 = v1[w0], r1 = p1 + tw * (v1[w1] - p1);
    return r0 + ta * (r1 - r0);
}
__device__ __attribute__((noinline)) double coat_table_r_call(const double* wls, int nw, const double* angs, int na,
                                                              const double* vals, double wl, double c1) {
    return coat_table_r(wls, nw, angs, na, vals, wl, c1);
// ... 469 lines not shown
}

struct Accum {
    unsigned int* cross;
    unsigned int* distinct;
    double* sums;
    unsigned int* bins;
};

template <int SEENW>
struct Seen {
    unsigned long long w[SEENW];
};

template <bool RECORD, int TAB_LDS, int SEENW, bool MESH, bool GRID, bool ROUGH = false, int LEAN = 0>
__device__ void tail_run(const KArgs* kernel_args, int total, unsigned int lds);

template <int TAB_LDS>
__device__ __attribute__((noinline)) void leave_workgroup(const KArgs* kernel_args) {
    extern __shared__ double smem[];
    const unsigned long long bits = (unsigned long long)kernel_args;
    const unsigned int lo = __builtin_amdgcn_readfirstlane((unsigned int)bits), hi = __builtin_amdgcn_readfirstlane((unsigned int)(bits >> 32));
    const __attribute__((address_space(4))) KArgs* ak = (const __attribute__((address_space(4))) KArgs*)(((unsigned long long)hi << 32) | lo);
    const KArgs& A = *(const KArgs*)ak;
    const int lane = threadIdx.x & 63;
    const int nd_lds = TAB_LDS == 1 ? A.nd : TAB_LDS == 2 ? A.nd_lds : 0;
    const int ni_stage = TAB_LDS == 1 ? A.ni : TAB_LDS == 2 ? A.ni_lds : 0;
    const int ni_lds = (ni_stage + 1) & ~1;
    int* lds_i = reinterpret_cast<int*>(smem + nd_lds);
    double* acc_sums = reinterpret_cast<double*>(lds_i + ni_lds);
    unsigned long long* acc_cross = reinterpret_cast<unsigned long long*>(acc_sums + A.n_rec * 8);
    unsigned int* acc_distinct = reinterpret_cast<unsigned int*>(acc_cross + A.n_rec);
    unsigned int* acc_bins = acc_distinct + ((A.n_rec + 1) & ~1);
    int* ctl = reinterpret_cast<int*>(acc_bins + ((A.bins_in_lds ? A.total_bins : 0) + 1 & ~1));
    const unsigned int set = A.set_size ? blockIdx.x / (unsigned int)A.wgs_per_set : 0u;
    __threadfence_block();
    int order = 0;
    if (lane == 0) order = atomicAdd(&ctl[CTL_DONE], 1);
    order = __builtin_amdgcn_readfirstlane(order);
    if (order != kWaves - 1) return;
    __threadfence_block();
    {
        unsigned long long* ctr = A.counters;
        if (ctr && lane < 4) {
            const unsigned long long* cnt = reinterpret_cast<const unsigned long long*>(ctl + CTL_COUNT);
            const unsigned long long v = lane == 3 ? (unsigned long long)kWaves : cnt[lane];
            if (v) atomicAdd(ctr + (blockIdx.x & 63u) * 8u + lane, v);
        }
        if (lane == 0) {
            const unsigned long long* t0 = reinterpret_cast<const unsigned long long*>(ctl + CTL_CLOCK);
            const unsigned long long real = wall_clock64(), cyc = __builtin_readcyclecounter();
            if (ctr) {
                atomicAdd(ctr + (blockIdx.x & 63u) * 8u + 4u, cyc - t0[1]);
                atomicAdd(ctr + (blockIdx.x & 63u) * 8u + 5u, real - t0[0]);
            }
            if (A.stamp) atomicMax(A.stamp + 1, real);
        }
    }
    unsigned long long* const out_distinct = reinterpret_cast<unsigned long long*>(A.rec_distinct) + (long long)set * A.set_stride_i;
    unsigned long long* const out_crossings = reinterpret_cast<unsigned long long*>(A.rec_crossings) + (long long)set * A.set_stride_i;
    unsigned long long* const out_bins = reinterpret_cast<unsigned long long*>(A.rec_bins) + (long long)set * A.set_stride_i;
    double* const out_sums = A.rec_sums + (long long)set * A.set_stride_d;
    for (int i = lane; i < A.n_rec; i += 64) {
        const unsigned long long c = acc_cross[i];
        const unsigned int d = acc_distinct[i];
        if (c) atomicAdd(out_crossings + i, c);
        if (d) atomicAdd(out_distinct + i, (unsigned long long)d);
    }
    for (int i = lane; i < A.n_rec * 8; i += 64) {
        double v = acc_sums[i];
        if (v != 0.0) atomicAdd(out_sums + i, v);
    }
    if (A.bins_in_lds)
        for (int i = lane; i < A.total_bins; i += 64) {
            unsigned int v = acc_bins[i];
            if (v) atomicAdd(out_bins + i, (unsigned long long)v);
        }
}

template <bool RECORD, int TAB_LDS, int SEENW, bool EMIT, bool MESH, bool GRID = false, bool TAIL = false, bool ROUGH = false,
          int LEAN = 0>
__device__ __forceinline__ void trace_body(const KArgs& A, int tail_total = 0, unsigned int tail_lds = 0u) {
    static_assert(!LEAN || (!MESH && !GRID && !ROUGH && TAB_LDS == 1 && SEENW == 1), "the lean variants: plain scenes only");
    extern __shared__ double smem_of_kernel[];
    double* const smem = TAIL ? (double*)(__attribute__((address_space(3))) double*)(unsigned long long)tail_lds
                              : (double*)smem_of_kernel;
    constexpr int kAbsKind = LEAN == kLeanEven ? kInterpEven : LEAN ? kInterpNoHist : kInterpAny;
    constexpr int kCdfKind = LEAN == kLeanEven ? kInterpByGuide : LEAN ? kInterpNoHist : kInterpAny;
    auto held = [](int v) __attribute__((always_inline)) -> int {
        if constexpr (TAIL) asm volatile("" : "+s"(v));
        return v;
    };
    const int k_root = held(A.root), k_maxsteps = held(A.maxsteps), k_nodes = held(A.n_nodes);
#if PVT_TIMELINE
    unsigned long long tl_t[6] = {(unsigned long long)wall_clock64(), 0, 0, 0, 0, 0};
    unsigned long long tl_iters = 0;
    const unsigned long long tl_c0 = __builtin_readcyclecounter();
#endif
    Lay L = A.lay;
    if constexpr (TAIL) {
        L.comp_d = held(L.comp_d); L.rec_d = held(L.rec_d); L.hist_d = held(L.hist_d); L.coat_d = held(L.coat_d);
        L.comp_i = held(L.comp_i); L.rec_i = held(L.rec_i); L.hist_i = held(L.hist_i); L.coat_i = held(L.coat_i);
        L.cand_i = held(L.cand_i); L.cand_list = held(L.cand_list); L.crit_d = held(L.crit_d); L.ccrit_d = held(L.ccrit_d);
        L.grid_d = held(L.grid_d); L.rot_d = held(L.rot_d); L.ncls_d = held(L.ncls_d); L.n_cls = held(L.n_cls);
    }
    enum { UF_COATED = 0, UF_FUSE_EXIT, UF_CRIT, UF_HAS_REC, UF_TQ_POS, UF_BINS_LDS, UF_EMIT_FULL, UF_EMIT_KT, UF_LAZY1, UF_LAZY2, UF_BY_NODE,
           UF_TAIL_LAZY1, UF_TAIL_LAZY2, UF_CTAB, UF_DISP, UF_ROUGH, UF_FIELD, UF_VMAP };
    unsigned int uflags_ =
        (A.n_coat > 0 ? 1u << UF_COATED : 0u) | (A.fuse_exit != 0 ? 1u << UF_FUSE_EXIT : 0u) | (L.crit_d >= 0 ? 1u << UF_CRIT : 0u) |
        (A.n_rec > 0 ? 1u << UF_HAS_REC : 0u) | (A.tq_pos ? 1u << UF_TQ_POS : 0u) | (A.bins_in_lds ? 1u << UF_BINS_LDS : 0u) |
        (A.emit_method == PVT_EMIT_FULL ? 1u << UF_EMIT_FULL : 0u) | (A.emit_method == PVT_EMIT_KT ? 1u << UF_EMIT_KT : 0u) |
        (A.lazy_root == 1 ? 1u << UF_LAZY1 : 0u) | (A.lazy_root == 2 ? 1u << UF_LAZY2 : 0u) | (L.by_node ? 1u << UF_BY_NODE : 0u) |
        (A.n_ctab > 0 ? 1u << UF_CTAB : 0u) | (A.n_rtab > 0 ? 1u << UF_DISP : 0u) |
        (ROUGH && A.rough_d >= 0 ? 1u << UF_ROUGH : 0u) |
        (ROUGH && A.fd != nullptr ? 1u << UF_FIELD : 0u) |
        (ROUGH && A.md != nullptr ? 1u << UF_VMAP : 0u);
    if constexpr (TAIL) {
        if (A.lazy_root == 0) uflags_ |= (A.lazy_tail == 1 ? 1u << UF_TAIL_LAZY1 : 0u) | (A.lazy_tail == 2 ? 1u << UF_TAIL_LAZY2 : 0u);
    }
    const unsigned int uflags = uflags_;
    auto uf = [&](int bit) -> bool {
        if constexpr (LEAN != kLeanOff) {
            if (bit == UF_COATED || bit == UF_CTAB || bit == UF_DISP || bit == UF_ROUGH || bit == UF_FIELD || bit == UF_VMAP) return false;
            if (bit == UF_BY_NODE) return true;
        }
        unsigned int f = uflags;
        asm volatile("" : "+s"(f));
        return ((f >> bit) & 1u) != 0u;
    };

    double* lds_d = smem;
    const int nd_lds = TAB_LDS == 1 ? A.nd : TAB_LDS == 2 ? A.nd_lds : 0;
    const int ni_stage = TAB_LDS == 1 ? A.ni : TAB_LDS == 2 ? A.ni_lds : 0;
    const int ni_lds = (ni_stage + 1) & ~1;
    int* lds_i = reinterpret_cast<int*>(lds_d + nd_lds);
    double* acc_sums = reinterpret_cast<double*>(lds_i + ni_lds);
    unsigned long long* acc_cross = reinterpret_cast<unsigned long long*>(acc_sums + A.n_rec * 8);
    unsigned int* acc_distinct = reinterpret_cast<unsigned int*>(acc_cross + A.n_rec);
    unsigned int* acc_bins = acc_distinct + ((A.n_rec + 1) & ~1);
    int* ctl = reinterpret_cast<int*>(acc_bins + ((A.bins_in_lds ? A.total_bins : 0) + 1 & ~1));
    unsigned long long* xbuf = reinterpret_cast<unsigned long long*>(ctl + CTL_WORDS);
    constexpr int kXWords = 14 + SEENW + (RECORD ? 1 : 0);
    const int tq_doubles = A.tq_pos ? 7 : 4;
    double* const tq_d = reinterpret_cast<double*>(xbuf + kXWords * A.xslots) + (threadIdx.x >> 6) * (tq_doubles * kTallyQ);
    int* const tq_r = reinterpret_cast<int*>(reinterpret_cast<double*>(xbuf + kXWords * A.xslots) + kWaves * tq_doubles * kTallyQ)
                      + (threadIdx.x >> 6) * kTallyQ;
    int tq_n = 0;
    if constexpr (!TAIL) {
    if (threadIdx.x < CTL_WORDS) ctl[threadIdx.x] = 0;
    if (blockIdx.x == 0 && threadIdx.x < 4 && A.cursor_next) A.cursor_next[threadIdx.x] = 0u;
    if constexpr (MESH) {
        typedef unsigned int Word4 __attribute__((ext_vector_type(4)));
        Word4* dst = reinterpret_cast<Word4*>(reinterpret_cast<char*>(smem) + A.top_off);
        const Word4* src = reinterpret_cast<const Word4*>(A.bvh_top);
        for (int i = threadIdx.x; i < A.top_n * 2; i += kBlock) dst[i] = src[i];
    }
    if constexpr (TAB_LDS != 0) {
        for (int i = threadIdx.x; i < nd_lds; i += kBlock) lds_d[i] = A.gd[i];
        for (int i = threadIdx.x; i < ni_stage; i += kBlock) lds_i[i] = A.gi[i];
    }
    for (int i = threadIdx.x; i < A.n_rec * 8; i += kBlock) acc_sums[i] = 0.0;
    for (int i = threadIdx.x; i < A.n_rec; i += kBlock) { acc_cross[i] = 0ull; acc_distinct[i] = 0u; }
    if (A.bins_in_lds)
        for (int i = threadIdx.x; i < A.total_bins; i += kBlock) acc_bins[i] = 0u;
    __syncthreads();
    if (threadIdx.x == 0) {
        unsigned long long* t0 = reinterpret_cast<unsigned long long*>(ctl + CTL_CLOCK);
        t0[0] = wall_clock64(); t0[1] = __builtin_readcyclecounter();
        if (blockIdx.x == 0 && A.stamp) A.stamp[0] = t0[0];
    }
    }
#if PVT_TIMELINE
    tl_t[1] = wall_clock64();
#endif

    Tables<TAB_LDS> T{(CDoubles)A.gd, (CInts)A.gi, TAB_LDS != 0 ? lds_d : A.gd, TAB_LDS != 0 ? lds_i : A.gi, A.gd, A.gi};

    auto node_bits = [&](int node) -> unsigned long long { return pvt_d2u(T.dv(node * ND + ND_BITS)); };
    auto node_ident = [](unsigned long long bits) -> bool { return LEAN || (bits & 1ull) != 0; };
    auto node_geom = [](unsigned long long bits) -> int {
        const int g = (int)(((unsigned int)bits >> 8) & 0xffu);
        return LEAN ? (g == PVT_GEOM_SPHERE ? (int)PVT_GEOM_SPHERE : (int)PVT_GEOM_BOX) : g;
    };
    auto node_rot = [&](unsigned long long bits) -> int { return L.rot_d + (int)(unsigned int)(bits >> 32) * RT; };

    auto shape_hits = [](int gt, double g0, double g1, double g2, const V3& o, const V3& d, double inv0, double inv1, double inv2,
                         auto&& fold) __attribute__((always_inline)) {
        if (gt == PVT_GEOM_BOX) {
            double tmin = -INFINITY, tmax = INFINITY;
            bool miss = false;
            const double oo[3] = {o.x, o.y, o.z}, dd[3] = {d.x, d.y, d.z}, gpar[3] = {g0, g1, g2}, inv[3] = {inv0, inv1, inv2};
            if (__ballot(pvt_fabs(dd[0]) < 1e-300 || pvt_fabs(dd[1]) < 1e-300 || pvt_fabs(dd[2]) < 1e-300) == 0ull) {
#pragma unroll
                for (int a = 0; a < 3; a++) {
                    const double sz = gpar[a];
                    const double ta = (-0.5 * sz - oo[a]) * inv[a], tb = (0.5 * sz - oo[a]) * inv[a];
                    tmin = __builtin_fmax(tmin, __builtin_fmin(ta, tb));
                    tmax = __builtin_fmin(tmax, __builtin_fmax(ta, tb));
                }
            } else
#pragma unroll
            for (int a = 0; a < 3; a++) {
                double sz = gpar[a];
                double lo = -0.5 * sz, hi = 0.5 * sz;
                if (pvt_fabs(dd[a]) < 1e-300) {
                    if (oo[a] < lo || oo[a] > hi) miss = true;
                } else {
                    const double ta = (lo - oo[a]) * inv[a], tb = (hi - oo[a]) * inv[a];
                    tmin = __builtin_fmax(tmin, __builtin_fmin(ta, tb));
                    tmax = __builtin_fmin(tmax, __builtin_fmax(ta, tb));
                }
            }
            if (!miss && !(tmax < tmin)) {
                if (tmin > kEps) fold(tmin);
                if (tmax > kEps) fold(tmax);
            }
        } else if (gt == PVT_GEOM_SPHERE) {
            double radius = g0;
            double a = dot3(d, d), b = 2.0 * dot3(d, o), c = dot3(o, o) - radius * radius;
            double disc = b * b - 4.0 * a * c;
            if (!(disc < 0.0)) {
                double sq = pvt_sqrt(disc);
                double t = (-b - sq) / (2.0 * a);
                if (t > kEps) fold(t);
                t = (-b + sq) / (2.0 * a);
                if (t > kEps) fold(t);
            }
        } else {
            double half = 0.5 * g0, radius = g1;
            double a = d.x * d.x + d.y * d.y;
            if (a > 1e-300) {
                double b = 2.0 * (o.x * d.x + o.y * d.y);
                double c = o.x * o.x + o.y * o.y - radius * radius;
                double disc = b * b - 4.0 * a * c;
                if (disc >= 0.0) {
                    double sq = pvt_sqrt(disc);
                    double t = (-b - sq) / (2.0 * a);
                    double z = o.z + t * d.z;
                    if (z > -half && z < half && t > kEps) fold(t);
                    t = (-b + sq) / (2.0 * a);
                    z = o.z + t * d.z;
                    if (z > -half && z < half && t > kEps) fold(t);
                }
            }
            if (pvt_fabs(d.z) > 1e-300) {
                double t = (-half - o.z) / d.z;
                double x = o.x + t * d.x, y = o.y + t * d.y;
                if (x * x + y * y <= radius * radius && t > kEps) fold(t);
                t = (half - o.z) / d.z;
                x = o.x + t * d.x;
                y = o.y + t * d.y;
                if (x * x + y * y <= radius * radius && t > kEps) fold(t);
            }
        }
    };

    const int lane = threadIdx.x & 63;
    auto rank_in = [](unsigned long long mask) -> unsigned int {
        return __builtin_amdgcn_mbcnt_hi((unsigned int)(mask >> 32), __builtin_amdgcn_mbcnt_lo((unsigned int)mask, 0u));
    };

    const unsigned int set = A.set_size ? blockIdx.x / (unsigned int)A.wgs_per_set : 0u;
    const unsigned int ray_lo = set * A.set_size;
    const unsigned int n_local = A.set_size ? (A.n_rays - ray_lo < A.set_size ? A.n_rays - ray_lo : A.set_size) : A.n_rays;
    unsigned int* const cursor = A.cursor + set;

    bool alive = false;
    V3 pos{0, 0, 0}, dir{0, 0, 1};
    double wl = 0.0, travelled = 0.0, duration = 0.0;
    Rng rng{0, 0, 0, 0};
    int count = 0, source = -1, nev = 0;
    unsigned int c_iters = 0u, c_steps = 0u, c_fused = 0u;
    int ac_node = -1;
    unsigned long long ac_wl = 0ull;
    double ac_alpha = 0.0, ac_pre0 = 0.0;
    unsigned long long* const ac_lds = xbuf + lane;
    V3 hr_t{0, 0, 0}, hr_g{0, 0, 0};
    unsigned long long hr_bits = 0ull;
    int hr_surf = 0;
    double hr_n2 = 0.0, hr_rn2 = 0.0, hr_cc = 0.0;
    constexpr bool kHoist = TAIL;
    auto index_at = [&](int node, double n) -> double {
        const int k = uf(UF_BY_NODE) ? node : T.iv(node * NI + NI_NCLS);
        const int q = L.ncls_d + 2 * L.n_cls;
        const double* tab = TAB_LDS == 1 ? T.ld : T.hd;
        if constexpr (MESH || SEENW == 1) return index_class_n_call((TAB_LDS != 0 ? T.ld : T.hd) + q, tab, k, n, wl);
        const int np = (int)T.dv(q + 2 * k + 1);
        if (np == 0) return n;
        return index_table_n(tab + (int)T.dv(q + 2 * k), np, wl);
    };
    int rec_slot = -1;
    Seen<SEENW> seen;
#pragma unroll
    for (int w = 0; w < SEENW; w++) seen.w[w] = 0ull;

#if PVT_STATS
    unsigned long long st_iters = 0, st_lane_steps = 0, st_drain_iters = 0, st_drain_lane_steps = 0;
    unsigned long long st_t[8] = {0, 0, 0, 0, 0, 0, 0, 0}, st_mark = 0;
#define PVT_MARK(k) do { unsigned long long now_ = __builtin_readcyclecounter(); if (ws & WS_SOLO) st_t[k] += now_ - st_mark; st_mark = now_; } while (0)
    unsigned long long st_c[8] = {0, 0, 0, 0, 0, 0, 0, 0};
    unsigned long long st_g[4] = {0, 0, 0, 0};
#define PVT_COUNT(k, pred) do { unsigned long long b_ = __ballot(pred); if (!(ws & WS_EXHAUSTED)) st_c[k] += __popcll(b_); } while (0)
#else
#define PVT_MARK(k) do {} while (0)
#define PVT_COUNT(k, pred) do {} while (0)
#endif
    const unsigned int wgs_in_set = A.set_size ? (unsigned int)A.wgs_per_set : gridDim.x;
    const unsigned int waves_in_set = wgs_in_set * kWaves;
    const unsigned int wave_in_set = (blockIdx.x - set * (A.set_size ? (unsigned int)A.wgs_per_set : 0u)) * kWaves +
                                     (unsigned int)__builtin_amdgcn_readfirstlane((int)(threadIdx.x >> 6));
    const unsigned int w_first = wave_in_set * (unsigned int)kClaim;
    unsigned int w_next = w_first, w_end = w_first, w_base = 0;
    unsigned int w_claim_end = w_first < n_local ? (n_local - w_first < (unsigned int)kClaim ? n_local : w_first + kClaim) : w_first;
    unsigned int c_next = 0, c_end = 0;
    enum { WS_EXHAUSTED = 1, WS_COUNTED = 2, WS_REGIME = 4, WS_SOLO = 8, WS_CARRY_IN = 16, WS_C_FIRST = 32 };
    unsigned int ws = WS_C_FIRST | ((!RECORD && (A.carry_flags & 1) != 0) ? WS_CARRY_IN : 0u);
    const bool seed_pool = A.xslots * (14 + SEENW) >= kWaves * 4 * 64;
    const int pool_at = __builtin_amdgcn_readfirstlane((int)(threadIdx.x >> 6)) * 4 * 64;
    const int wave = __builtin_amdgcn_readfirstlane((int)(threadIdx.x >> 6));
    int members = 0, parity = 0;
    int tail_n = 0;
    constexpr bool kTailCall = !TAIL && !MESH && !(GRID && RECORD);

    auto tally_flush = [&]() {
        if (lane < tq_n) {
            const int r = tq_r[lane];
            const double q_wl = tq_d[lane], q_angle = pvt_acos(tq_d[kTallyQ + lane]);
            const double q_duration = tq_d[2 * kTallyQ + lane], q_travelled = tq_d[3 * kTallyQ + lane];
            const int ri = L.rec_i + r * RI;
            atomicAdd(&acc_distinct[r], 1u);
            double* sp = acc_sums + r * 8;
            atomicAdd(&sp[0], q_wl); atomicAdd(&sp[1], q_wl * q_wl);
            atomicAdd(&sp[2], q_angle); atomicAdd(&sp[3], q_angle * q_angle);
            atomicAdd(&sp[4], q_duration); atomicAdd(&sp[5], q_duration * q_duration);
            atomicAdd(&sp[6], q_travelled); atomicAdd(&sp[7], q_travelled * q_travelled);
            const int h0 = T.iv(ri + RI_HSTART), h1 = h0 + T.iv(ri + RI_HN);
            for (int h = h0; h < h1; h++) {
                const int hi_ = L.hist_i + h * HI, hd_ = L.hist_d + h * HD;
                const int pa = T.iv(hi_ + HI_PA), pb = T.iv(hi_ + HI_PB);
                const int na = T.iv(hi_ + HI_NA), nb = T.iv(hi_ + HI_NB);
                auto prop = [&](int pr) -> double {
                    if (pr < 4) return pr == 0 ? q_wl : pr == 1 ? q_angle : pr == 2 ? q_duration : q_travelled;
                    return tq_d[pr * kTallyQ + lane];
                };
                const double la = T.dv(hd_ + HD_LO_A), ha = T.dv(hd_ + HD_HI_A);
                const double ra = T.dv(hd_ + HD_RA);
                const double qa = ra == ra ? div_known(prop(pa) - la, ha - la, ra) : (prop(pa) - la) / (ha - la);
                const int ia = (int)(qa * na);
                if (ia < 0 || ia >= na) continue;
                int slot = T.iv(hi_ + HI_OFF) + ia;
                if (pb >= 0) {
                    const double lb = T.dv(hd_ + HD_LO_B), hb = T.dv(hd_ + HD_HI_B);
                    const double rb = T.dv(hd_ + HD_RB);
                    const double qb = rb == rb ? div_known(prop(pb) - lb, hb - lb, rb) : (prop(pb) - lb) / (hb - lb);
                    const int ib = (int)(qb * nb);
                    if (ib < 0 || ib >= nb) continue;
                    slot = T.iv(hi_ + HI_OFF) + ia * nb + ib;
                }
                if (uf(UF_BINS_LDS)) atomicAdd(&acc_bins[slot], 1u);
                else atomicAdd(reinterpret_cast<unsigned long long*>(A.rec_bins) + (long long)set * A.set_stride_i + slot, 1ull);
            }
        }
        tq_n = 0;
    };
    if constexpr (TAIL) {
        constexpr int X = kXSlots;
        const int slot = lane;
        ws = WS_EXHAUSTED | WS_COUNTED | WS_SOLO;
        alive = slot < tail_total;
        if (alive) {
            pos = V3{pvt_u2d(xbuf[0 * X + slot]), pvt_u2d(xbuf[1 * X + slot]), pvt_u2d(xbuf[2 * X + slot])};
            dir = V3{pvt_u2d(xbuf[3 * X + slot]), pvt_u2d(xbuf[4 * X + slot]), pvt_u2d(xbuf[5 * X + slot])};
// ... 252 lines not shown
                if constexpr (kTailCall) {
                    if (keep == 1) {
                        tail_n = total;
                        alive = false;
                        break;
                    }
                }
                const int slot = pos_in_set * 64 + lane;
                alive = slot < total;
                if (alive) {
                    pos = V3{pvt_u2d(xbuf[0 * X + slot]), pvt_u2d(xbuf[1 * X + slot]), pvt_u2d(xbuf[2 * X + slot])};
                    dir = V3{pvt_u2d(xbuf[3 * X + slot]), pvt_u2d(xbuf[4 * X + slot]), pvt_u2d(xbuf[5 * X + slot])};
                    wl = pvt_u2d(xbuf[6 * X + slot]); travelled = pvt_u2d(xbuf[7 * X + slot]); duration = pvt_u2d(xbuf[8 * X + slot]);
                    rng.s0 = xbuf[9 * X + slot]; rng.s1 = xbuf[10 * X + slot]; rng.s2 = xbuf[11 * X + slot]; rng.s3 = xbuf[12 * X + slot];
                    const unsigned long long cs_ = xbuf[13 * X + slot];
                    count = (int)(unsigned int)cs_;
                    source = (int)(unsigned int)(cs_ >> 32);
#pragma unroll
                    for (int w = 0; w < SEENW; w++) seen.w[w] = xbuf[(14 + w) * X + slot];
                    if constexpr (RECORD) {
                        const unsigned long long rn_ = xbuf[(14 + SEENW) * X + slot];
                        rec_slot = (int)(unsigned int)rn_;
                        nev = (int)(unsigned int)(rn_ >> 32);
                    }
                }
                int kept = 0, m2 = 0;
#pragma unroll
                for (int w = 0; w < kWaves; w++)
                    if (((members >> w) & 1) && kept < keep) { m2 |= 1 << w; kept += 1; }
                members = m2;
                if (keep == 1) ws = (ws & ~(unsigned int)WS_REGIME) | WS_SOLO;
            }
        }
        }
#if PVT_STATS
        {
            unsigned long long live = __popcll(__ballot(alive));
            st_iters += 1; st_lane_steps += live;
            if (ws & WS_EXHAUSTED) { st_drain_iters += 1; st_drain_lane_steps += live; }
        }
#endif

        c_iters += 1u;
#if PVT_TIMELINE
        if (tl_iters == 0) tl_t[2] = wall_clock64();
        if ((ws & WS_EXHAUSTED) && tl_t[3] == 0) tl_t[3] = wall_clock64();
        tl_iters += 1;
#endif
        PVT_MARK(0);
        PVT_COUNT(0, alive);
        int ev_kind = -1, ev_hit = -1, ev_container = -1, ev_adjacent = -1, ev_component = -1;
        bool ev_normal = false, terminal = false;
        int t_sel = -1, t_node = -1;
        bool t_normal = false;
        double t_cos = 1.0;
        V3 nrm{0, 0, 0};
        int tri1 = -1;
        bool em = false;

        enum { CLS_NONE = 0, CLS_SURF, CLS_EXIT, CLS_ABS };
        int cls = CLS_NONE;
        int hit = -1, container = -1, adjacent = -1;
        double t0 = 0.0;
        bool pend = false;
        if (alive) {
            count += 1;
            bool budget_kill = false;
            if constexpr (RECORD) budget_kill = (rec_slot >= 0 && nev >= A.max_events - 1);
            if (budget_kill) {
                ev_kind = PVT_EV_KILL;
                terminal = true;
            } else {
                int nhits = 0, n1 = -1, n2 = -1, cnode = -1;
                tri1 = -1;
                double t1 = INFINITY, t2 = INFINITY, cbest = INFINITY;
                int c2node = -1;
                double c2best = INFINITY;
                V3 d{0, 0, 0};
                double inv[3] = {0, 0, 0};
                bool inv_ok = false;
                int rot = -1;
                const bool lazy_exact = TAIL && !MESH && (uf(UF_TAIL_LAZY1) || uf(UF_TAIL_LAZY2));
                const int lazy_root = MESH ? 0 : (lazy_exact ? (uf(UF_TAIL_LAZY1) ? 1 : 2)
                                                              : (RECORD ? 0 : (uf(UF_LAZY1) ? 1 : (uf(UF_LAZY2) ? 2 : 0))));
                auto fold_by_key = [&](double t, int node, int& nl, double& tfirst) __attribute__((always_inline)) {
                    const double a1 = t1, a2 = t2, tf = tfirst;
                    const int m1 = n1, m2 = n2, have = nhits, l = nl;
                    const bool none = have == 0;
                    const bool nearest = none || t < a1 || (t == a1 && node < m1);
                    const bool second = !nearest && (m2 < 0 || t < a2 || (t == a2 && node < m2));
                    const bool shift = nearest && !none;
                    tfirst = l == 0 ? t : tf;
                    nl = l + 1;
                    t1 = nearest ? t : a1;
                    n1 = nearest ? node : m1;
                    t2 = shift ? a1 : (second ? t : a2);
                    n2 = shift ? m1 : (second ? node : m2);
                    nhits = have + 1;
                };
                if constexpr (GRID) {
                    const int gb = L.grid_d;
                    const unsigned long long gbits = pvt_d2u(T.du(gb + 13));
                    const double guard = T.du(gb + 12);
                    const double invw0 = rcp_normal(dir.x), invw1 = rcp_normal(dir.y), invw2 = rcp_normal(dir.z);
                    const double invw[3] = {invw0, invw1, invw2};
                    const double pw[3] = {pos.x, pos.y, pos.z}, dw[3] = {dir.x, dir.y, dir.z};
                    double t_in = 0.0, t_out = INFINITY;
                    bool walk = true;
#pragma unroll
                    for (int a = 0; a < 3; a++) {
                        const double lo = T.du(gb + a), hi = T.du(gb + 3 + a);
                        if (pvt_fabs(dw[a]) < 1e-20) {
                            if (pw[a] < lo || pw[a] > hi) walk = false;
                        } else {
                            const double ta = (lo - pw[a]) * invw[a], tb = (hi - pw[a]) * invw[a];
                            t_in = __builtin_fmax(t_in, __builtin_fmin(ta, tb));
                            t_out = __builtin_fmin(t_out, __builtin_fmax(ta, tb));
                        }
                    }
                    if (!(t_in <= t_out)) walk = false;
                    double tm0 = INFINITY, tm1 = INFINITY, tm2 = INFINITY;
                    unsigned int remv = 0;
                    int ci = 0;
                    {
                        int stride = 1;
#pragma unroll
                        for (int a = 0; a < 3; a++) {
                            const int na = (int)((unsigned int)(gbits >> (8 * a)) & 0xffu);
                            const double lo = T.du(gb + a), cell = T.du(gb + 6 + a), rcell = T.du(gb + 9 + a);
                            const double at = pw[a] + dw[a] * t_in;
                            int c = (int)((at - lo) * rcell);
                            c = c < 0 ? 0 : (c > na - 1 ? na - 1 : c);
                            const bool par = pvt_fabs(dw[a]) < 1e-20, neg = dw[a] < 0.0;
                            const double tma = par ? INFINITY : ((lo + (double)(c + (neg ? 0 : 1)) * cell) - pw[a]) * invw[a];
                            if (a == 0) tm0 = tma; else if (a == 1) tm1 = tma; else tm2 = tma;
                            remv |= (unsigned int)(neg ? c : na - 1 - c) << (8 * a);
                            if (neg) remv |= 1u << (24 + a);
                            ci += c * stride;
                            stride *= na;
                        }
                    }
                    const int words = (int)((unsigned int)(gbits >> 24) & 0xfu);
                    const bool odd = ((gbits >> 28) & 1ull) != 0;
                    unsigned long long seen_lo = 0ull, seen_hi = 0ull;
                    auto visit = [&](int node) __attribute__((always_inline)) {
                        const int hn = node * ND;
                        const double tx = T.dv(hn + ND_T), ty = T.dv(hn + ND_T + 1), tz = T.dv(hn + ND_T + 2);
                        const double g0 = T.dv(hn + ND_PARAMS), g1 = T.dv(hn + ND_PARAMS + 1), g2 = T.dv(hn + ND_PARAMS + 2);
                        const unsigned long long hb = pvt_d2u(T.dv(hn + ND_BITS));
                        int gt = (int)(((unsigned int)hb >> 8) & 0xffu);
                        V3 o, dl;
                        double il0, il1, il2;
                        if ((hb & 1ull) != 0) {
                            o.x = pos.x + tx; o.y = pos.y + ty; o.z = pos.z + tz;
                            dl = dir;
                            il0 = invw0; il1 = invw1; il2 = invw2;
                        } else {
                            const int rm = L.rot_d + (int)(unsigned int)(hb >> 32) * RT + RT_W2L;
                            o.x = T.dv(rm + 0) * pos.x + T.dv(rm + 1) * pos.y + T.dv(rm + 2) * pos.z + tx;
                            o.y = T.dv(rm + 3) * pos.x + T.dv(rm + 4) * pos.y + T.dv(rm + 5) * pos.z + ty;
                            o.z = T.dv(rm + 6) * pos.x + T.dv(rm + 7) * pos.y + T.dv(rm + 8) * pos.z + tz;
                            dl.x = T.dv(rm + 0) * dir.x + T.dv(rm + 1) * dir.y + T.dv(rm + 2) * dir.z;
                            dl.y = T.dv(rm + 3) * dir.x + T.dv(rm + 4) * dir.y + T.dv(rm + 5) * dir.z;
                            dl.z = T.dv(rm + 6) * dir.x + T.dv(rm + 7) * dir.y + T.dv(rm + 8) * dir.z;
                            il0 = rcp_normal(dl.x); il1 = rcp_normal(dl.y); il2 = rcp_normal(dl.z);
                        }
                        bool root_known = false;
                        if (lazy_root && node == k_root) {
                            double bound;
                            if (lazy_root == 1) {
                                bound = __builtin_fmin(__builtin_fmin(0.5 * g0 - pvt_fabs(o.x), 0.5 * g1 - pvt_fabs(o.y)), 0.5 * g2 - pvt_fabs(o.z));
                            } else {
                                bound = (g0 * g0 - dot3(o, o)) * A.lazy_k;
                            }
                            const bool undecided = !(bound > 0.0) || (nhits > 0 && !(t1 < bound)) || (nhits >= 2 && !(t2 < bound)) ||
                                                   (cnode >= 0 && !(cbest < bound)) || (lazy_exact && nhits == 0);
                            {
                                const double a1 = t1, a2 = t2;
                                const int m1 = n1, m2 = n2, have = nhits, cn = cnode;
                                const bool known = !undecided;
                                t1 = known && have == 0 ? bound : a1; n1 = known && have == 0 ? node : m1;
                                t2 = known && have == 1 ? INFINITY : a2; n2 = known && have == 1 ? node : m2;
                                nhits = have + (known ? 1 : 0);
                                cnode = known && cn < 0 ? node : cn;
                                root_known = known;
                                gt = known ? -1 : gt;
                            }
                        }
                        int nl = 0;
                        double tfirst = 0.0;
                        auto fold = [&](double t) __attribute__((always_inline)) { fold_by_key(t, node, nl, tfirst); };
                        if (gt >= 0) shape_hits(gt, g0, g1, g2, o, dl, il0, il1, il2, fold);
                        {
                            const double cb = cbest;
                            const int cn = cnode;
                            const bool holds = nl == 1 && !root_known && (tfirst < cb || (tfirst == cb && node < cn));
                            cbest = holds ? tfirst : cb;
                            cnode = holds ? node : cn;
                        }
                    };
                    auto next_cell = [&]() __attribute__((always_inline)) {
                        const double t_cell = __builtin_fmin(tm0, __builtin_fmin(tm1, tm2));
                        const bool enough = nhits >= 2 && t2 + guard < t_cell && (!odd || (cnode >= 0 && cbest + guard < t_cell));
                        const int ax = (tm0 <= tm1 && tm0 <= tm2) ? 0 : (tm1 <= tm2 ? 1 : 2);
                        const unsigned int left = (remv >> (8 * ax)) & 0xffu;
                        if (enough || left == 0u || !(t_cell < INFINITY)) {
                            walk = false;
                        } else {
                            remv -= 1u << (8 * ax);
                            const int nx = (int)((unsigned int)gbits & 0xffu), ny = (int)((unsigned int)(gbits >> 8) & 0xffu);
                            const int stride = ax == 0 ? 1 : (ax == 1 ? nx : nx * ny);
                            ci += ((remv >> (24 + ax)) & 1u) ? -stride : stride;
                            if (ax == 0) tm0 = __builtin_fma(pvt_fabs(invw0), T.du(gb + 6), tm0);
                            else if (ax == 1) tm1 = __builtin_fma(pvt_fabs(invw1), T.du(gb + 7), tm1);
                            else tm2 = __builtin_fma(pvt_fabs(invw2), T.du(gb + 8), tm2);
                        }
                    };
                    bool root_todo = true;
                    auto untested = [&](unsigned long long& m_lo, unsigned long long& m_hi) __attribute__((always_inline)) {
                        const int at = gb + 14 + ci * words;
                        m_lo = pvt_d2u(T.dv(at)) & ~seen_lo;
                        m_hi = words > 1 ? pvt_d2u(T.dv(at + 1)) & ~seen_hi : 0ull;
                    };
                    for (;;) {
                        if (__ballot(walk || root_todo) == 0ull) break;
                        unsigned long long m_lo = 0ull, m_hi = 0ull;
                        if (walk) {
                            untested(m_lo, m_hi);
                            if ((m_lo | m_hi) == 0ull) {
                                next_cell();
                                if (walk) untested(m_lo, m_hi);
                            }
                        }
                        bool test = false;
                        int node = k_root;
                        if (m_lo != 0ull) { node = __builtin_ctzll(m_lo); seen_lo |= m_lo & (0ull - m_lo); test = true; }
                        else if (m_hi != 0ull) { node = 64 + __builtin_ctzll(m_hi); seen_hi |= m_hi & (0ull - m_hi); test = true; }
                        else if (!walk && root_todo) { root_todo = false; test = true; }
#if PVT_STATS
                        st_g[0] += 1; st_g[1] += 1; st_g[2] += __popcll(__ballot(test)); st_g[3] += __popcll(__ballot(!test));
#endif
                        if (test) visit(node);
                    }
                }
                for (int k = 0; k < (GRID ? 0 : k_nodes); k++) {
                    const int node = !lazy_root ? k : (k == k_nodes - 1 ? k_root : (k < k_root ? k : k + 1));
                    const int hn = node * ND;
                    const double tx = T.du(hn + ND_T), ty = T.du(hn + ND_T + 1), tz = T.du(hn + ND_T + 2);
                    const double gpar[3] = {T.du(hn + ND_PARAMS), T.du(hn + ND_PARAMS + 1), T.du(hn + ND_PARAMS + 2)};
                    const unsigned long long hbits = pvt_d2u(T.du(hn + ND_BITS));
                    const bool ident = node_ident(hbits);
                    const int rc = LEAN ? 0 : (int)(unsigned int)(hbits >> 32);
                    V3 o;
                    if (ident) {
                        o.x = pos.x + tx; o.y = pos.y + ty; o.z = pos.z + tz;
                    } else {
                        const int rm = L.rot_d + rc * RT + RT_W2L;
                        o.x = T.du(rm + 0) * pos.x + T.du(rm + 1) * pos.y + T.du(rm + 2) * pos.z + tx;
                        o.y = T.du(rm + 3) * pos.x + T.du(rm + 4) * pos.y + T.du(rm + 5) * pos.z + ty;
                        o.z = T.du(rm + 6) * pos.x + T.du(rm + 7) * pos.y + T.du(rm + 8) * pos.z + tz;
                    }
                    if (rc != rot) {
                        if (ident) {
                            d = dir;
                        } else {
                            const int rm = L.rot_d + rc * RT + RT_W2L;
                            d.x = T.du(rm + 0) * dir.x + T.du(rm + 1) * dir.y + T.du(rm + 2) * dir.z;
                            d.y = T.du(rm + 3) * dir.x + T.du(rm + 4) * dir.y + T.du(rm + 5) * dir.z;
                            d.z = T.du(rm + 6) * dir.x + T.du(rm + 7) * dir.y + T.du(rm + 8) * dir.z;
                        }
                        rot = rc;
                        inv_ok = false;
                    }
                const int gt = node_geom(hbits);
                int nl = 0;
                double tfirst = 0.0;
                bool root_known = false;
                if (lazy_root && node == k_root) {
                    double bound;
                    if (lazy_root == 1) {
                        const double mx = 0.5 * gpar[0] - pvt_fabs(o.x), my = 0.5 * gpar[1] - pvt_fabs(o.y),
                                     mz = 0.5 * gpar[2] - pvt_fabs(o.z);
                        bound = __builtin_fmin(__builtin_fmin(mx, my), mz);
                    } else {
                        const double radius = gpar[0];
                        bound = (radius * radius - dot3(o, o)) * A.lazy_k;
                    }
                    const bool undecided = !(bound > 0.0) || (nhits > 0 && !(t1 < bound)) || (nhits >= 2 && !(t2 < bound)) ||
                                           (cnode >= 0 && !(cbest < bound)) || (lazy_exact && nhits == 0);
                    if (!undecided) {
                        if (nhits == 0) { t1 = bound; n1 = node; }
                        else if (nhits == 1) { t2 = INFINITY; n2 = node; }
                        nhits += 1;
                        if (cnode < 0) cnode = node;
                        root_known = true;
                    }
                }
                auto fold = [&](double t) __attribute__((always_inline)) {
                    if (nl == 0) tfirst = t;
                    nl += 1;
                    if (nhits == 0) { t1 = t; n1 = node; }
                    else if (t < t1) { t2 = t1; n2 = n1; t1 = t; n1 = node; }
                    else if (n2 < 0 || t < t2) { t2 = t; n2 = node; }
                    nhits += 1;
                };
                if (root_known) {
                } else if (MESH && gt == PVT_GEOM_MESH) {
                    const double oo[3] = {o.x, o.y, o.z}, dd[3] = {d.x, d.y, d.z};
                    const double ax = pvt_fabs(d.x), ay = pvt_fabs(d.y), az = pvt_fabs(d.z);
                    const int kz = (ax >= ay && ax >= az) ? 0 : (ay >= az ? 1 : 2);
                    int kx = kz == 2 ? 0 : kz + 1, ky = kx == 2 ? 0 : kx + 1;
                    auto pick = [](const double* v, int k) { return k == 0 ? v[0] : (k == 1 ? v[1] : v[2]); };
                    const double dz = pick(dd, kz);
                    if (dz < 0.0) { int tmp = kx; kx = ky; ky = tmp; }
                    double shx, shy, shz;
                    {
                        const double sx_ = pick(dd, kx), sy_ = pick(dd, ky);
                        auto ordinary = [](double x) { return x == 0.0 || (pvt_fabs(x) > 1e-280 && pvt_fabs(x) < 1e280); };
                        if (__ballot(!(pvt_fabs(dz) > 1e-100 && pvt_fabs(dz) < 1e100) || !ordinary(sx_) || !ordinary(sy_)) == 0ull) {
                            shx = div_normal(sx_, dz); shy = div_normal(sy_, dz); shz = rcp_normal(dz);
                        } else {
                            shx = sx_ / dz; shy = sy_ / dz; shz = 1.0 / dz;
                        }
                    }
                    double minv[3];
#pragma unroll
                    for (int a = 0; a < 3; a++) minv[a] = pvt_fabs(dd[a]) < 1e-300 ? 1e300 : rcp_normal(dd[a]);
                    long long f1 = -1, f2 = -1;
// ... 151 lines not shown
                        tmin = __builtin_fmax(tmin, __builtin_fmin(ta, tb));
                        tmax = __builtin_fmin(tmax, __builtin_fmax(ta, tb));
                    }
                }
                if (!miss && !(tmax < tmin)) {
                    if (tmin > kEps) fold(tmin);
                    if (tmax > kEps) fold(tmax);
                }
            } else if (gt == PVT_GEOM_SPHERE) {
                    double radius = gpar[0];
                    double a = dot3(d, d), b = 2.0 * dot3(d, o), c = dot3(o, o) - radius * radius;
                    double disc = b * b - 4.0 * a * c;
                    if (!(disc < 0.0)) {
                        double sq = pvt_sqrt(disc);
                        double t = (-b - sq) / (2.0 * a);
                        if (t > kEps) fold(t);
                        t = (-b + sq) / (2.0 * a);
                        if (t > kEps) fold(t);
                    }
                } else {
                    double half = 0.5 * gpar[0], radius = gpar[1];
                    double a = d.x * d.x + d.y * d.y;
                    if (a > 1e-300) {
                        double b = 2.0 * (o.x * d.x + o.y * d.y);
                        double c = o.x * o.x + o.y * o.y - radius * radius;
                        double disc = b * b - 4.0 * a * c;
                        if (disc >= 0.0) {
                            double sq = pvt_sqrt(disc);
                            double t = (-b - sq) / (2.0 * a);
                            double z = o.z + t * d.z;
                            if (z > -half && z < half && t > kEps) fold(t);
                            t = (-b + sq) / (2.0 * a);
                            z = o.z + t * d.z;
                            if (z > -half && z < half && t > kEps) fold(t);
                        }
                    }
                    if (pvt_fabs(d.z) > 1e-300) {
                        double t = (-half - o.z) / d.z;
                        double x = o.x + t * d.x, y = o.y + t * d.y;
                        if (x * x + y * y <= radius * radius && t > kEps) fold(t);
                        t = (half - o.z) / d.z;
                        x = o.x + t * d.x;
                        y = o.y + t * d.y;
                        if (x * x + y * y <= radius * radius && t > kEps) fold(t);
                    }
                }
                    const bool holds = (MESH && gt == PVT_GEOM_MESH) ? (nl & 1) != 0 : nl == 1;
                    if (holds && !root_known) {
                        if (tfirst < cbest) {
                            if constexpr (MESH) { c2best = cbest; c2node = cnode; }
                            cbest = tfirst; cnode = node;
                        } else if (MESH && tfirst < c2best) { c2best = tfirst; c2node = node; }
                    }
                }

                PVT_MARK(1);
                if (nhits == 0) {
                    terminal = true;
                } else {
                    hit = n1;
                    t0 = t1;
                    if (nhits == 1) { container = hit; adjacent = -1; }
                    else {
                        container = (cnode >= 0) ? cnode : hit;
                        adjacent = (container == hit) ? n2 : hit;
                        if constexpr (MESH) {
                            if (container == hit && c2node >= 0 && node_geom(node_bits(hit)) == PVT_GEOM_MESH) adjacent = c2node;
                        }
                    }
                    ev_container = container;
                    if (count > k_maxsteps) {
                        ev_kind = PVT_EV_KILL;
                        terminal = true;
                        t_sel = PVT_REC_KILLED; t_node = container;
                    } else {
                        pend = true;
                    }
                }
            }
        }
        double alpha = 0.0, pre0 = 0.0, n_container = 1.0;
        int cbase = 0, ccount = 0, crec = 0;
        if (pend) {
            n_container = T.dv(container * ND + ND_N);
            if (uf(UF_DISP)) n_container = index_at(container, n_container);
            cbase = T.iv(container * NI + NI_CSTART); ccount = T.iv(container * NI + NI_CCOUNT);
            if (uf(UF_BY_NODE)) crec = cbase;
            else crec = T.iv(container * NI + NI_CREC);
            if constexpr (TAIL) {
                const int hn = hit * ND;
                hr_t = V3{T.dv(hn + ND_T), T.dv(hn + ND_T + 1), T.dv(hn + ND_T + 2)};
                hr_g = V3{T.dv(hn + ND_PARAMS), T.dv(hn + ND_PARAMS + 1), T.dv(hn + ND_PARAMS + 2)};
                hr_bits = pvt_d2u(T.dv(hn + ND_BITS));
                hr_surf = T.iv(hit * NI + NI_SURF);
                if (adjacent >= 0) {
                    int kc = container, ka = adjacent;
                    if (!uf(UF_BY_NODE)) { kc = T.iv(container * NI + NI_NCLS); ka = T.iv(adjacent * NI + NI_NCLS); }
                    hr_n2 = T.dv(adjacent * ND + ND_N);
                    hr_rn2 = T.dv(L.ncls_d + ka * 2 + 1);
                    hr_cc = uf(UF_CRIT) ? T.dv(L.ccrit_d + kc * L.n_cls + ka) : __builtin_nan("");
                    if (uf(UF_DISP)) { hr_n2 = index_at(adjacent, hr_n2); hr_rn2 = div_normal(1.0, hr_n2); }
                }
            }
            bool known = false;
            if constexpr (TAIL) {
                ac_node = (int)(unsigned int)ac_lds[0]; ac_wl = ac_lds[64];
                ac_alpha = pvt_u2d(ac_lds[128]); ac_pre0 = pvt_u2d(ac_lds[192]);
            }
            if constexpr (TAIL) known = container == ac_node && pvt_d2u(wl) == ac_wl;
            if (hit != k_root && !known) {
                for (int k = 0; k < ccount; k++) {
                    const int ci = L.comp_i + (crec + k) * CI, cd = L.comp_d + (crec + k) * CD;
                    alpha += interp_clamped<TAB_LDS, kAbsKind>(T, wl, T.iv(ci + CI_ABS_X), T.iv(ci + CI_ABS_Y), T.iv(ci + CI_ABS_N),
                                                            T.iv(ci + CI_ABS_G), T.dv(cd + CD_ABS_SCALE), T.iv(ci + CI_ABS_HIST),
                                                            T.dv(cd + CD_ABS_RCP), T.dv(cd + CD_ABS_W));
                    if (k == 0) pre0 = alpha;
                }
                if constexpr (TAIL) {
                    ac_lds[0] = (unsigned long long)(unsigned int)container; ac_lds[64] = pvt_d2u(wl);
                    ac_lds[128] = pvt_d2u(alpha); ac_lds[192] = pvt_d2u(pre0);
                }
            }
            if constexpr (TAIL) {
                if (known && hit != k_root) { alpha = ac_alpha; pre0 = ac_pre0; }
            }
        }
        int comp = -1;
        int frec = -1, fcell = 0;
        if (pend) {
            double depth = INFINITY;
            if constexpr (!ROUGH) {
                if (hit != k_root && alpha > kAlphaZero) depth = div_normal(-pvt_log(1.0 - rng_uniform(rng)), alpha);
            } else {
                if (hit != k_root && alpha > kAlphaZero) {
                    const double tau = -pvt_log(1.0 - rng_uniform(rng));
                    if (uf(UF_FIELD)) frec = (int)A.fd[container];
                    if (frec >= 0) {
                        const FieldMarch fm = field_march_call<TAB_LDS>(T, A.fd, frec, L.comp_i + crec * CI, L.comp_d + crec * CD, ccount,
                                                                        wl, pos.x, pos.y, pos.z, dir.x, dir.y, dir.z, tau, t0);
                        depth = fm.depth;
                        if (fm.depth < t0) { alpha = fm.alpha; pre0 = fm.pre0; fcell = fm.cell; }
                    } else {
                        depth = div_normal(tau, alpha);
                    }
                }
            }
            {
                const double adv = __builtin_fmin(depth, t0);
                pos.x = pos.x + dir.x * adv; pos.y = pos.y + dir.y * adv; pos.z = pos.z + dir.z * adv;
                travelled += adv;
                duration += div_known(adv * n_container, kCcm, kRcpCcm);
            }
            if (hit == k_root) {
                ev_kind = PVT_EV_EXIT; ev_hit = hit; ev_adjacent = adjacent;
                terminal = true;
                t_sel = PVT_REC_EXIT; t_node = hit; t_normal = true;
                cls = CLS_EXIT;
            } else {
                if (depth < t0) {
                    const double target = rng_uniform(rng) * alpha;
                    comp = cbase;
                    if (LEAN || ccount <= 2) {
                        comp = (ccount == 2 && !(target <= pre0)) ? cbase + 1 : cbase;
                    } else {
                        double running = 0.0;
                        for (int k = 0; k < ccount; k++) {
                            const int ci = L.comp_i + (crec + k) * CI, cd = L.comp_d + (crec + k) * CD;
                            double term = interp_clamped<TAB_LDS>(T, wl, T.iv(ci + CI_ABS_X), T.iv(ci + CI_ABS_Y), T.iv(ci + CI_ABS_N),
                                                                  T.iv(ci + CI_ABS_G), T.dv(cd + CD_ABS_SCALE), T.iv(ci + CI_ABS_HIST),
                                                                  T.dv(cd + CD_ABS_RCP), T.dv(cd + CD_ABS_W));
                            if constexpr (ROUGH) {
                                if (frec >= 0) term = term * A.fd[(int)A.fd[frec + kFrComp + k] + fcell];
                            }
                            running += term;
                            if (target <= running) { comp = cbase + k; break; }
                        }
                    }
                    log_row<RECORD, TAIL>(A, rec_slot, nev, PVT_EV_ABSORB, -1, container, -1, comp, source, pos,
                                    dir, false, pos, wl, travelled, duration);
                    ev_component = comp;
                    cls = CLS_ABS;
                } else {
                    ev_hit = hit;
// ... 40 lines not shown
                        em_turn = g2;
                        em_c = sqrt1m2_normal(em_s);
                    } else {
                        if (tabled && ptab[0] > 1.0) u1 = rng_uniform(rng);
                        double g1 = rng_uniform(rng), g2 = rng_uniform(rng);
                        em_turn = g1;
                        em_c = 2.0 * g2 - 1.0;
                        em_s = sqrt1m2_normal(em_c);
                        u3 = g2;
                    }
                    if (tabled) {
                        if constexpr (MESH || SEENW == 1) dir = phase_table_turn_call(ptab, wl, u1, em_turn, u3, dir.x, dir.y, dir.z);
                        else dir = phase_table_turn(ptab, wl, u1, em_turn, u3, dir.x, dir.y, dir.z);
                    } else {
                        double sp, cp;
                        pvt_sincos2pi(em_turn, &sp, &cp);
                        dir = V3{em_s * cp, em_s * sp, em_c};
                    }
                    em = true;
                    source = cu;
                    if (LEAN || ctype == PVT_COMP_LUMINOPHORE) {
                        const int ex = T.iv(ci + CI_EMS_X), ec = T.iv(ci + CI_EMS_CDF), en = T.iv(ci + CI_EMS_N);
                        const int eh = T.iv(ci + CI_EMS_HIST);
                        const double ew = T.dv(cd + CD_EMS_W);
                        double p1;
                        if (uf(UF_EMIT_FULL)) {
                            p1 = 0.0;
                        } else {
                            double e_nm = wl;
                            if (uf(UF_EMIT_KT)) {
                                const double kb_ev = 1.380649e-23 / 1.60217662e-19;
                                double e_ev = div_normal(1240.0, e_nm) + 1.5 * kb_ev * 300.0;
                                e_nm = div_normal(1240.0, e_ev);
                            }
                            p1 = interp_clamped<TAB_LDS, kAbsKind>(T, e_nm, ex, ec, en, T.iv(ci + CI_EMS_GX), T.dv(cd + CD_EMS_SCALE_X),
                                                                              eh, T.dv(cd + CD_EMS_RCP_X), ew);
                        }
                        double gamma = p1 + (1.0 - p1) * rng_uniform(rng);
                        wl = interp_clamped<TAB_LDS, kCdfKind>(T, gamma, ec, ex, en, T.iv(ci + CI_EMS_GC), T.dv(cd + CD_EMS_SCALE_C), eh,
                                                                    T.dv(cd + CD_EMS_RCP_C), __builtin_nan(""), eh ? __builtin_nan("") : ew);
                        tau = T.dv(cd + CD_TAU_RAD);
                        ev_kind = PVT_EV_EMIT;
                    } else {
                        ev_kind = PVT_EV_SCATTER;
                    }
                } else {
                    tau = T.dv(cd + CD_TAU_NR);
                    if (!LEAN && ctype == PVT_COMP_REACTOR) { ev_kind = PVT_EV_REACT; t_sel = PVT_REC_REACTED; }
                    else { ev_kind = PVT_EV_NONRADIATIVE; t_sel = PVT_REC_LOST; }
                    t_node = container;
                    terminal = true;
                }
                if (tau > 0.0) duration += -pvt_log(1.0 - rng_uniform(rng)) * tau;
            }
        }

        if constexpr (ROUGH) {
            if (uf(UF_VMAP)) {
                if (cls == CLS_ABS)
                    volume_map_call(A.md, reinterpret_cast<unsigned long long*>(A.rec_bins) + (long long)set * A.set_stride_i + A.total_bins,
                                    container, comp, ev_kind, pos.x, pos.y, pos.z, wl_abs, wl);
            }
        }
        PVT_MARK(2);
        PVT_COUNT(1, alive && ev_component >= 0);
        PVT_COUNT(2, em);
        PVT_COUNT(3, alive && t_normal && ev_kind != PVT_EV_EXIT);
        PVT_COUNT(4, alive && ev_kind == PVT_EV_EXIT);
        PVT_COUNT(5, alive && t_sel >= 0);
        PVT_COUNT(6, alive && terminal);
        auto local_point = [&]() -> V3 {
            if constexpr (kHoist) {
                if (t_normal) {
                    if (node_ident(hr_bits)) return V3{pos.x + hr_t.x, pos.y + hr_t.y, pos.z + hr_t.z};
                    const int m = node_rot(hr_bits) + RT_W2L;
                    return V3{T.dv(m + 0) * pos.x + T.dv(m + 1) * pos.y + T.dv(m + 2) * pos.z + hr_t.x,
                              T.dv(m + 3) * pos.x + T.dv(m + 4) * pos.y + T.dv(m + 5) * pos.z + hr_t.y,
                              T.dv(m + 6) * pos.x + T.dv(m + 7) * pos.y + T.dv(m + 8) * pos.z + hr_t.z};
                }
            }
            const int tr = t_node * ND + ND_T;
            const unsigned long long tb = node_bits(t_node);
            if (node_ident(tb))
                return V3{pos.x + T.dv(tr), pos.y + T.dv(tr + 1), pos.z + T.dv(tr + 2)};
            const int m = node_rot(tb) + RT_W2L;
            return V3{T.dv(m + 0) * pos.x + T.dv(m + 1) * pos.y + T.dv(m + 2) * pos.z + T.dv(tr),
                      T.dv(m + 3) * pos.x + T.dv(m + 4) * pos.y + T.dv(m + 5) * pos.z + T.dv(tr + 1),
                      T.dv(m + 6) * pos.x + T.dv(m + 7) * pos.y + T.dv(m + 8) * pos.z + T.dv(tr + 2)};
        };
        auto local_normal = [&](const V3& lp) -> V3 {
            const int gp = t_node * ND + ND_PARAMS;
            const int gt = kHoist ? node_geom(hr_bits) : node_geom(node_bits(t_node));
            auto param = [&](int a) -> double {
                if constexpr (kHoist) return a == 0 ? hr_g.x : (a == 1 ? hr_g.y : hr_g.z);
                return T.dv(gp + a);
            };
            if (MESH && gt == PVT_GEOM_MESH) {
                const pvt::MeshTri* tr = A.tris + tri1;
                return V3{tr->n[0], tr->n[1], tr->n[2]};
            }
            if (gt == PVT_GEOM_BOX) {
                const double hx = 0.5 * param(0), hy = 0.5 * param(1), hz = 0.5 * param(2);
                const double mx = pvt_fabs(lp.x - (-1.0) * hx), px = pvt_fabs(lp.x - hx);
                const double my = pvt_fabs(lp.y - (-1.0) * hy), py = pvt_fabs(lp.y - hy);
                const double mz = pvt_fabs(lp.z - (-1.0) * hz), pz = pvt_fabs(lp.z - hz);
                const double cx = __builtin_fmin(px, mx), cy = __builtin_fmin(py, my), cz = __builtin_fmin(pz, mz);
                const bool use_y = cy < cx;
                const double cxy = __builtin_fmin(cy, cx);
                const bool use_z = cz < cxy;
                const double sx = px < mx ? 1.0 : -1.0, sy = py < my ? 1.0 : -1.0, sz = pz < mz ? 1.0 : -1.0;
                return V3{(!use_y && !use_z) ? sx : 0.0, (use_y && !use_z) ? sy : 0.0, use_z ? sz : 0.0};
            }
            if (gt == PVT_GEOM_SPHERE) {
                double mag = pvt_sqrt(dot3(lp, lp));
                return V3{lp.x / mag, lp.y / mag, lp.z / mag};
            }
            double half = 0.5 * param(0);
            double tol = 1e-8 + 1e-5 * pvt_fabs(half);
            if (pvt_fabs(lp.z + half) <= tol) return V3{0.0, 0.0, -1.0};
            if (pvt_fabs(lp.z - half) <= tol) return V3{0.0, 0.0, 1.0};
            double r = pvt_sqrt(lp.x * lp.x + lp.y * lp.y);
            return V3{lp.x / r, lp.y / r, 0.0};
        };
        if (alive && t_normal) {
            const V3 nloc = local_normal(local_point());
            const unsigned long long tb = kHoist ? hr_bits : node_bits(t_node);
            if (node_ident(tb)) {
                nrm = nloc;
            } else {
                const int q = node_rot(tb) + RT_L2W;
                nrm.x = T.dv(q + 0) * nloc.x + T.dv(q + 1) * nloc.y + T.dv(q + 2) * nloc.z;
                nrm.y = T.dv(q + 3) * nloc.x + T.dv(q + 4) * nloc.y + T.dv(q + 5) * nloc.z;
                nrm.z = T.dv(q + 6) * nloc.x + T.dv(q + 7) * nloc.y + T.dv(q + 8) * nloc.z;
            }
        }

        PVT_MARK(3);
        const bool surf = alive && t_normal && ev_kind != PVT_EV_EXIT;
        bool flip = false;
        double ddot = 0.0;
        double ac_arg = 1.0;
        if (alive && t_normal) {
            if (ev_kind == PVT_EV_EXIT) {
                ac_arg = __builtin_fmin(pvt_fabs(dot3(nrm, dir)), 1.0);
            } else {
                ddot = dot3(nrm, dir);
                if (ddot < 0.0) {
                    flip = true;
                    ddot = -ddot;
                }
                ac_arg = __builtin_fmin(ddot, 1.0);
            }
        }
        if (alive && t_normal) t_cos = ac_arg;
        const bool fres = surf && (kHoist ? hr_surf : T.iv(ev_hit * NI + NI_SURF)) == PVT_SURF_FRESNEL;
        const double c1 = ac_arg, s1 = fres ? sqrt1m2_normal(ac_arg) : 0.0;

        PVT_MARK(4);
        if (surf) {
            const int hit = ev_hit, container = ev_container, adjacent = ev_adjacent;
            double r = 0.0, n1 = 0.0, n2 = 0.0, rn2 = 0.0;
            if (fres) {
                n1 = kHoist ? n_container : T.dv(container * ND + ND_N);
                n2 = kHoist ? hr_n2 : T.dv(adjacent * ND + ND_N);
                int kc = container, ka = adjacent;
                if (!kHoist && !uf(UF_BY_NODE)) { kc = T.iv(container * NI + NI_NCLS); ka = T.iv(adjacent * NI + NI_NCLS); }
                const int ncls_d = L.ncls_d, n_cls = L.n_cls;
                rn2 = kHoist ? hr_rn2 : T.dv(ncls_d + ka * 2 + 1);
                if (!kHoist && uf(UF_DISP)) {
                    n1 = n_container;
                    n2 = index_at(adjacent, n2);
                    rn2 = div_normal(1.0, n2);
                }
                bool tir;
                const bool crit_tab = uf(UF_CRIT);
                const double cc = kHoist ? hr_cc : (crit_tab ? T.dv(L.ccrit_d + kc * n_cls + ka) : __builtin_nan(""));
                if (cc == cc) tir = c1 < cc;
                else {
                    if (kHoist && !uf(UF_BY_NODE)) { kc = T.iv(container * NI + NI_NCLS); ka = T.iv(adjacent * NI + NI_NCLS); }
                    const double crit = crit_tab ? T.dv(L.crit_d + kc * n_cls + ka) : __builtin_nan("");
                    if (crit == crit) tir = pvt_acos(c1) > crit;
                    else tir = n2 < n1 && pvt_acos(c1) > pvt_asin(uf(UF_DISP) ? div_normal(n2, n1) : div_known(n2, n1, T.dv(ncls_d + kc * 2 + 1)));
                }
                if (tir) {
                    r = 1.0;
                } else {
                    double q = div_known(n1, n2, rn2) * s1;
                    double k = sqrt_normal(1.0 - q * q);
                    double rs1 = n1 * c1 - n2 * k, rs2 = n1 * c1 + n2 * k;
                    const double as = div_normal(rs1, rs2);
                    double rs = as * as;
                    double rp1 = n1 * k - n2 * c1, rp2 = n1 * k + n2 * c1;
                    const double ap = div_normal(rp1, rp2);
                    double rp = ap * ap;
                    r = 0.5 * (rs + rp);
                }
            }
            int coat = -1;
            if (uf(UF_COATED) && fres) {
                const int cs = T.iv(hit * NI + NI_KSTART), ce = cs + T.iv(hit * NI + NI_KCOUNT);
                V3 lpos{0, 0, 0}, nloc = nrm;
                if (cs < ce) {
                    lpos = local_point();
                    if (!node_ident(kHoist ? hr_bits : node_bits(hit))) nloc = local_normal(lpos);
                }
                const double nl3[3] = {nloc.x, nloc.y, nloc.z}, pl3[3] = {lpos.x, lpos.y, lpos.z};
                for (int c = cs; c < ce && coat < 0; c++) {
                    bool ok = true;
#pragma unroll
                    for (int a = 0; a < 3; a++) {
                        double f = T.dv(L.coat_d + c * KD + KD_FACET + a);
                        if (pvt_fabs(nl3[a] - f) > 1e-8 + 1e-5 * pvt_fabs(f)) ok = false;
                        if (!(pl3[a] > T.dv(L.coat_d + c * KD + KD_LO + a) && pl3[a] < T.dv(L.coat_d + c * KD + KD_HI + a))) ok = false;
                    }
                    if (ok) coat = c;
                }
                if (coat >= 0) {
                    double cr = T.dv(L.coat_d + coat * KD + KD_REFL);
                    const bool keep_tir = r == 1.0 && T.iv(L.coat_i + coat * KI + KI_TMODE) != 1;
                    if (uf(UF_CTAB) && !keep_tir) {
                        const int q = L.coat_i + coat * KI, nw = T.iv(q + KI_TNW);
                        if (nw > 0) {
                            const double* tab = TAB_LDS == 1 ? T.ld : T.hd;
                            const double *wls = tab + T.iv(q + KI_TW), *angs = tab + T.iv(q + KI_TA), *vals = tab + T.iv(q + KI_TV);
                            const int na = T.iv(q + KI_TNA);
                            if constexpr (MESH) cr = coat_table_r_call(wls, nw, angs, na, vals, wl, c1);
                            else cr = coat_table_r(wls, nw, angs, na, vals, wl, c1);
                        }
                    }
                    if (cr >= 0.0 && !keep_tir) r = cr;
                }
            }
            bool rough = false, rough_reflect = false;
            if constexpr (ROUGH) {
              if (uf(UF_ROUGH) && fres && coat < 0) {
                const double alpha = T.sd(A.rough_d + hit);
                if (alpha > 0.0) {
                    const RoughEvent e = rough_event_call(alpha, nrm.x, nrm.y, nrm.z, dir.x, dir.y, dir.z, n1, n2, rng.s0, rng.s1,
                                                          rng.s2, rng.s3);
                    dir = V3{e.dx, e.dy, e.dz};
                    rng = Rng{e.s0, e.s1, e.s2, e.s3};
                    rough = true;
                    rough_reflect = e.reflect != 0;
                }
              }
            }
            double u = 1.0;
            if (r > 0.0 && !rough) u = rng_uniform(rng);
            if (rough ? rough_reflect : u < r) {
                bool lamb = false;
                if (coat >= 0) lamb = T.iv(L.coat_i + coat * KI + KI_RMODE) == 1;
                if (lamb) {
                    double side = dot3(nrm, dir) < 0.0 ? 1.0 : -1.0;
                    V3 nloc = nrm;
                    if (!node_ident(node_bits(hit))) nloc = local_normal(local_point());
                    V3 mm{side * nloc.x, side * nloc.y, side * nloc.z};
                    double p1 = rng_uniform(rng), p2 = rng_uniform(rng);
                    V3 sd = lambert_direction(p1, p2);
                    double sign = mm.z < 0.0 ? -1.0 : 1.0;
                    double a = -1.0 / (sign + mm.z);
                    double b = mm.x * mm.y * a;
                    V3 t1v{1.0 + sign * mm.x * mm.x * a, sign * b, -sign * mm.x};
                    V3 t2v{b, sign + mm.y * mm.y * a, -mm.y};
                    V3 dl{sd.x * t1v.x + sd.y * t2v.x + sd.z * mm.x, sd.x * t1v.y + sd.y * t2v.y + sd.z * mm.y,
                          sd.x * t1v.z + sd.y * t2v.z + sd.z * mm.z};
                    const int q = node_rot(node_bits(hit)) + RT_L2W;
                    dir.x = T.dv(q + 0) * dl.x + T.dv(q + 1) * dl.y + T.dv(q + 2) * dl.z;
                    dir.y = T.dv(q + 3) * dl.x + T.dv(q + 4) * dl.y + T.dv(q + 5) * dl.z;
                    dir.z = T.dv(q + 6) * dl.x + T.dv(q + 7) * dl.y + T.dv(q + 8) * dl.z;
                } else if (!rough) {
                    const V3 nf{flip ? -nrm.x : nrm.x, flip ? -nrm.y : nrm.y, flip ? -nrm.z : nrm.z};
                    const double dd = ddot;
                    dir = V3{dir.x - 2.0 * dd * nf.x, dir.y - 2.0 * dd * nf.y, dir.z - 2.0 * dd * nf.z};
                }
                ev_kind = PVT_EV_REFLECT;
                t_sel = (container != hit) ? PVT_REC_REFLECTED : -1;
            } else {
                bool matched = false;
                if (coat >= 0) matched = T.iv(L.coat_i + coat * KI + KI_TMODE) == 1;
                if (fres && !matched && !rough) {
                    double n = div_known(n1, n2, rn2);
                    const V3 nf{flip ? -nrm.x : nrm.x, flip ? -nrm.y : nrm.y, flip ? -nrm.z : nrm.z};
                    const double dd = ddot;
                    double c = sqrt_normal(1.0 - n * n * (1.0 - dd * dd));
                    double sign = dd < 0.0 ? -1.0 : 1.0;
                    double k = sign * (c - sign * n * dd);
                    dir = V3{n * dir.x + k * nf.x, n * dir.y + k * nf.y, n * dir.z + k * nf.z};
                }
                ev_kind = PVT_EV_TRANSMIT;
                t_sel = (container == hit) ? PVT_REC_ESCAPING : PVT_REC_ENTERING;
            }
            if (!RECORD && !MESH && uf(UF_FUSE_EXIT) && !terminal && count < k_maxsteps &&
                (ev_kind == PVT_EV_REFLECT ? container == k_root : adjacent == k_root)) {
                const V3 lp = local_point();
                const int gp = hit * ND + ND_PARAMS;
                const double h = kHoist ? 0.5 * (pvt_fabs(nrm.x) * hr_g.x + pvt_fabs(nrm.y) * hr_g.y + pvt_fabs(nrm.z) * hr_g.z)
                                        : 0.5 * (pvt_fabs(nrm.x) * T.dv(gp) + pvt_fabs(nrm.y) * T.dv(gp + 1) + pvt_fabs(nrm.z) * T.dv(gp + 2));
                const double g = h - dot3(nrm, lp), dn = dot3(nrm, dir);
                if (dn > 0.0 && g <= (0.5 * kEps) * dn) {
                    terminal = true;
                    c_fused += 1u;
                }
            }
        }

        PVT_MARK(5);
        if (alive && ev_kind >= 0)
            log_row<RECORD, TAIL>(A, rec_slot, nev, ev_kind, ev_hit, ev_container, ev_adjacent, ev_component, source, pos,
                            dir, ev_normal, nrm, wl, travelled, duration);

        if (uf(UF_HAS_REC)) {
            int cs = 0, cn = 0, rbin = -1;
            if (alive && t_sel >= 0) {
                int cb = t_node;
                bool listened = true;
                if (!uf(UF_BY_NODE)) {
                    cb = T.iv(t_node * NI + NI_CAND);
                    listened = cb >= 0;
                    cb = listened ? cb : 0;
                }
                const int key = L.cand_i + (cb * 7 + t_sel) * 8;
                if (listened) {
                    cs = T.iv(key);
                    cn = T.iv(key + 1);
                }
                if (listened && t_normal) {
                    const double ax = pvt_fabs(nrm.x), ay = pvt_fabs(nrm.y), az = pvt_fabs(nrm.z);
                    int b = (ax >= ay && ax >= az) ? (nrm.x > 0.0 ? 1 : 0)
                          : (ay >= az)             ? (nrm.y > 0.0 ? 3 : 2)
                                                   : (nrm.z > 0.0 ? 5 : 4);
                    rbin = T.iv(key + 2 + b);
                }
            }
            const int nb = rbin >= 0 ? 1 : 0, ntrips = nb + cn;
            for (int j = 0;; j++) {
                const unsigned long long trip = __ballot(j < ntrips);
                if (trip == 0ull) break;
                if (tq_n + __popcll(trip) > kTallyQ) tally_flush();
                bool push = false;
                int push_r = 0;
                if (j < ntrips) {
                    const int entry = j < nb ? rbin : T.iv(L.cand_list + cs + j - nb);
                    const int r = entry & (kRecPlain - 1);
                    const int ri = L.rec_i + r * RI;
                    bool match = true;
                    const bool plain = LEAN || (entry & kRecPlain) != 0;
                    const int smode = plain ? 0 : T.iv(ri + RI_SRC_MODE);
                    if (smode != 0) {
                        if (smode == 1) match = source < 0;
                        else if (smode == 2) match = source >= 0;
                        else match = source == T.iv(ri + RI_SRC_ID);
                    }
                    if (!plain && match && T.iv(ri + RI_HAS_FACET) != 0) {
                        const int rd = L.rec_d + r * RD;
                        const double atol = T.dv(rd + RD_ATOL);
                        if (!t_normal) match = false;
                        else if (pvt_fabs(T.dv(rd + RD_FACET) - nrm.x) > atol) match = false;
                        else if (pvt_fabs(T.dv(rd + RD_FACET + 1) - nrm.y) > atol) match = false;
                        else if (pvt_fabs(T.dv(rd + RD_FACET + 2) - nrm.z) > atol) match = false;
                    }
                    if (match) {
                        atomicAdd(&acc_cross[r], 1ull);
                        const unsigned long long bit = 1ull << (r & 63);
                        bool first;
                        if constexpr (SEENW == 1) {
                            first = !(seen.w[0] & bit);
                            seen.w[0] |= bit;
                        } else {
                            const int w = r >> 6;
                            const unsigned long long cur = w == 0 ? seen.w[0] : w == 1 ? seen.w[1] : w == 2 ? seen.w[2] : seen.w[3];
                            first = !(cur & bit);
                            if (w == 0) seen.w[0] |= bit; else if (w == 1) seen.w[1] |= bit;
                            else if (w == 2) seen.w[2] |= bit; else seen.w[3] |= bit;
                        }
                        push = first;
                        push_r = r;
                    }
                }
                const unsigned long long pm = __ballot(push);
                if (pm != 0ull) {
                    const int at = tq_n + (int)rank_in(pm);
                    if (push) {
                        tq_r[at] = push_r;
                        tq_d[at] = wl; tq_d[kTallyQ + at] = t_cos; tq_d[2 * kTallyQ + at] = duration; tq_d[3 * kTallyQ + at] = travelled;
// ... 27 lines not shown
        atomicAdd(c + 15, (ws & WS_SOLO) ? 1ull : 0ull);
        for (int k = 0; k < 8; k++) atomicAdd(c + 16 + k, st_c[k]);
        for (int k = 0; k < 4; k++) atomicAdd(c + 24 + k, st_g[k]);
    }
#endif
#if PVT_TIMELINE
    if (!TAIL && A.timeline && lane == 0) {
        unsigned long long* o = A.timeline + ((unsigned long long)blockIdx.x * kWaves + (threadIdx.x >> 6)) * 8;
        o[0] = tl_t[0]; o[1] = tl_t[1]; o[2] = tl_t[2]; o[3] = tl_t[3]; o[4] = wall_clock64(); o[5] = tl_iters;
        o[6] = __builtin_readcyclecounter() - tl_c0;
        o[7] = 1ull | ((ws & WS_SOLO) || tail_n > 0 ? 2ull : 0ull) | ((unsigned long long)(__builtin_amdgcn_s_getreg(20 | (3 << 11)) & 15u) << 2) |
               ((unsigned long long)__builtin_amdgcn_s_getreg(4 | (31 << 11)) << 32);
    }
#endif
    tally_flush();
    {
        unsigned long long* const cnt = reinterpret_cast<unsigned long long*>(ctl + CTL_COUNT);
        if (lane == 0) atomicAdd(cnt, (unsigned long long)c_iters);
        atomicAdd(cnt + 1, (unsigned long long)c_steps);
        atomicAdd(cnt + 2, (unsigned long long)c_fused);
    }
#if PVT_TIMELINE
    if constexpr (TAIL) {
        if (A.timeline && lane == 0) {
            unsigned long long* o = A.timeline + ((unsigned long long)blockIdx.x * kWaves + (threadIdx.x >> 6)) * 8;
            o[1] = tl_t[0]; o[4] = wall_clock64(); o[5] |= tl_iters << 32;
        }
    }
#endif
    if constexpr (TAIL) return;
    {
        const __attribute__((address_space(4))) KArgs* ak =
            (const __attribute__((address_space(4))) KArgs*)__builtin_amdgcn_kernarg_segment_ptr();
        if constexpr (kTailCall) {
            if (tail_n > 0) {
                unsigned int lds_at = (unsigned int)(unsigned long long)(__attribute__((address_space(3))) double*)smem_of_kernel;
                asm volatile("" : "+s"(lds_at));
                tail_run<RECORD, TAB_LDS, SEENW, MESH, GRID, ROUGH, LEAN>((const KArgs*)ak, tail_n, lds_at);
            }
        }
        leave_workgroup<TAB_LDS>((const KArgs*)ak);
    }

}

template <bool RECORD, int TAB_LDS, int SEENW, bool MESH, bool GRID, bool ROUGH, int LEAN>
__device__ __attribute__((noinline)) void tail_run(const KArgs* kernel_args, int total, unsigned int lds) {
    const unsigned long long bits = (unsigned long long)kernel_args;
    const unsigned int lo = __builtin_amdgcn_readfirstlane((unsigned int)bits), hi = __builtin_amdgcn_readfirstlane((unsigned int)(bits >> 32));
    const __attribute__((address_space(4))) KArgs* ak = (const __attribute__((address_space(4))) KArgs*)(((unsigned long long)hi << 32) | lo);
    trace_body<RECORD, TAB_LDS, SEENW, false, MESH, GRID, true, ROUGH, LEAN>(*(const KArgs*)ak, __builtin_amdgcn_readfirstlane(total),
                                                                __builtin_amdgcn_readfirstlane(lds));
}

template <bool RECORD, int TAB_LDS, int SEENW, bool EMIT, bool MESH>
__global__ void __launch_bounds__(kBlock) __attribute__((amdgpu_waves_per_eu(kMeshWaves, kMeshWaves))) trace_kernel(KArgs A) {
    trace_body<RECORD, TAB_LDS, SEENW, EMIT, MESH>(A);
}
template <bool RECORD, int TAB_LDS, int SEENW, bool EMIT>
__global__ void __launch_bounds__(kBlock) __attribute__((amdgpu_waves_per_eu(4, 4))) trace_kernel_w4(KArgs A) {
    trace_body<RECORD, TAB_LDS, SEENW, EMIT, false>(A);
}
template <bool RECORD, int SEENW, bool EMIT>
__global__ void __launch_bounds__(kBlock) __attribute__((amdgpu_waves_per_eu(4, 4))) trace_kernel_grid(KArgs A) {
    trace_body<RECORD, 1, SEENW, EMIT, false, true>(A);
}
template <bool RECORD, int TAB_LDS, int SEENW, bool EMIT, bool MESH>
__global__ void __launch_bounds__(kBlock) __attribute__((amdgpu_waves_per_eu(kMeshWaves, kMeshWaves))) trace_kernel_rough(KArgs A) {
    trace_body<RECORD, TAB_LDS, SEENW, EMIT, MESH, false, false, true>(A);
}
template <bool RECORD, int TAB_LDS, int SEENW, bool EMIT>
__global__ void __launch_bounds__(kBlock) __attribute__((amdgpu_waves_per_eu(4, 4))) trace_kernel_rough_w4(KArgs A) {
    trace_body<RECORD, TAB_LDS, SEENW, EMIT, false, false, false, true>(A);
}
template <bool RECORD, int SEENW, bool EMIT>
__global__ void __launch_bounds__(kBlock) __attribute__((amdgpu_waves_per_eu(4, 4))) trace_kernel_rough_grid(KArgs A) {
    trace_body<RECORD, 1, SEENW, EMIT, false, true, false, true>(A);
}
template <bool RECORD, bool EMIT, bool EVEN>
__global__ void __launch_bounds__(kBlock) __attribute__((amdgpu_waves_per_eu(4, 4))) trace_kernel_lean_w4(KArgs A) {
    trace_body<RECORD, 1, 1, EMIT, false, false, false, false, EVEN ? kLeanEven : kLeanSearched>(A);
}

}
```

pvtrace_amd/engine/native.py:

```python
import ctypes as C
import os
import threading

import numpy as np

_HERE = os.path.dirname(os.path.abspath(__file__))
LIB_PATH = os.environ.get(
    "PVT_LIB", os.path.join(os.path.dirname(_HERE), "csrc", "libpvtrace_hip.so"))

_p_i32 = C.POINTER(C.c_int32)
_p_f64 = C.POINTER(C.c_double)
_p_i64 = C.POINTER(C.c_int64)
_p_u8 = C.POINTER(C.c_uint8)


class EngineUnavailableError(RuntimeError):
    """The HIP engine cannot run here (library not built, or no MI355X visible)."""


class PvtSceneTables(C.Structure):
    _fields_ = [
        ("n_nodes", C.c_int32), ("root_id", C.c_int32), ("n_components", C.c_int32),
        ("n_abs", C.c_int32), ("n_ems", C.c_int32), ("n_recorders", C.c_int32),
        ("n_hists", C.c_int32), ("total_bins", C.c_int32), ("n_coatings", C.c_int32),
# ... 295 lines not shown

def num_recorded(n_rays, record_every):
    return (n_rays + record_every - 1) // record_every if record_every > 0 else 0


EVENT_LOG_COLUMNS = (
    ("kind", np.uint8, 1), ("hit", np.int32, 1), ("container", np.int32, 1),
    ("adjacent", np.int32, 1), ("component", np.int32, 1), ("source", np.int32, 1),
    ("position", np.float64, 3), ("direction", np.float64, 3), ("normal", np.float64, 3),
    ("wavelength", np.float64, 1), ("travelled", np.float64, 1), ("duration", np.float64, 1),
)


RECORD_WORDS = 16
_ID_COLUMNS = ("hit", "container", "adjacent", "component", "source")


def decode_records(rows):
    rows = np.ascontiguousarray(rows).reshape(-1, RECORD_WORDS)
    i32 = rows.view(np.int32).reshape(-1, 2 * RECORD_WORDS)
    f64 = rows.view(np.float64).reshape(-1, RECORD_WORDS)
    return {
        "kind": i32[:, 5].astype(np.uint8), "hit": i32[:, 0].copy(), "container": i32[:, 1].copy(),
        "adjacent": i32[:, 2].copy(), "component": i32[:, 3].copy(), "source": i32[:, 4].copy(),
        "position": f64[:, 3:6].copy(), "direction": f64[:, 6:9].copy(), "normal": f64[:, 9:12].copy(),
        "wavelength": f64[:, 12].copy(), "travelled": f64[:, 13].copy(), "duration": f64[:, 14].copy(),
    }


def declare_signatures(lib, names):
    vp = C.c_void_p
    sigs = {
        "pvt_abi_version": ([], C.c_int),
        "pvt_last_error": ([], C.c_char_p),
        "pvt_device_count": ([], C.c_int),
        "pvt_scene_create": ([C.POINTER(PvtSceneTables), C.c_int, C.POINTER(vp)], C.c_int),
        "pvt_scene_create_ex": ([C.POINTER(PvtSceneTables), C.POINTER(PvtIndexTables), C.c_int, C.POINTER(vp)], C.c_int),
        "pvt_scene_create_phase": ([C.POINTER(PvtSceneTables), C.POINTER(PvtIndexTables), C.POINTER(PvtPhaseTables), C.c_int,
                                    C.POINTER(vp)], C.c_int),
        "pvt_scene_create_rough": ([C.POINTER(PvtSceneTables), C.POINTER(PvtIndexTables), C.POINTER(PvtPhaseTables),
                                    C.POINTER(PvtSurfaceTables), C.c_int, C.POINTER(vp)], C.c_int),
        "pvt_scene_create_field": ([C.POINTER(PvtSceneTables), C.POINTER(PvtIndexTables), C.POINTER(PvtPhaseTables),
                                    C.POINTER(PvtSurfaceTables), C.POINTER(PvtFieldTables), C.c_int, C.POINTER(vp)],
                                   C.c_int),
        "pvt_scene_create_maps": ([C.POINTER(PvtSceneTables), C.POINTER(PvtIndexTables), C.POINTER(PvtPhaseTables),
                                   C.POINTER(PvtSurfaceTables), C.POINTER(PvtFieldTables), C.POINTER(PvtMapTables), C.c_int,
                                   C.POINTER(vp)], C.c_int),
        "pvt_scene_map_slots": ([vp], C.c_int64),
        "pvt_scene_set_emitter": ([vp, C.POINTER(PvtEmitterTables)], C.c_int),
        "pvt_scene_destroy": ([vp], None),
        "pvt_trace_device": (
            [vp, C.POINTER(PvtRays), C.POINTER(PvtTraceParams), C.POINTER(PvtTallies),
             C.POINTER(PvtEventLog), vp], C.c_int),
        "pvt_trace_device_records": (
            [vp, C.POINTER(PvtRays), C.POINTER(PvtTraceParams), C.POINTER(PvtTallies),
             C.POINTER(PvtEventRecords), vp], C.c_int),
        "pvt_scene_carry_pending": ([vp, vp], C.c_int),
        "pvt_scene_carry_discard": ([vp, vp], C.c_int),
        "pvt_scene_trim": ([vp], C.c_int),
        "pvt_last_multi_reduce": ([], C.c_int),
        "pvt_unpack_records_device": (
            [C.POINTER(PvtEventRecords), C.c_int64, C.c_int32, C.POINTER(PvtEventLog), C.c_int, vp], C.c_int),
        "pvt_trace_bundle": (
            [C.POINTER(PvtSceneTables), C.POINTER(PvtEmitterTables), C.POINTER(PvtRays),
             C.POINTER(PvtTraceParams), C.POINTER(PvtTallies), C.POINTER(PvtEventLog), C.c_int,
             C.POINTER(C.c_double)], C.c_int),
        "pvt_trace_bundle_multi": (
            [C.POINTER(PvtSceneTables), C.POINTER(PvtEmitterTables), C.POINTER(PvtRays),
             C.POINTER(PvtTraceParams), C.POINTER(PvtTallies), C.POINTER(PvtEventLog), C.POINTER(C.c_int),
             C.c_int, C.POINTER(C.c_double)], C.c_int),
        "pvt_release_cached_memory": ([], None),
        "pvt_shard_range": ([C.c_int64, C.c_int, C.c_int, C.c_int64, C.POINTER(C.c_int64), C.POINTER(C.c_int64)], C.c_int),
        "pvt_emit_device": ([vp, C.POINTER(PvtTraceParams), vp, vp, vp, vp], C.c_int),
        "pvt_selftest_math": ([C.c_int, vp, vp, C.c_int64, C.c_int], C.c_int),
        "pvt_mesh_bvh_check": (
            [C.POINTER(PvtSceneTables), C.c_int32, C.POINTER(C.c_int32), C.POINTER(C.c_int32),
             C.POINTER(C.c_int32)], C.c_int),
        "pvt_scene_launch_info": (
            [vp, C.POINTER(C.c_int32), C.POINTER(C.c_int32), C.POINTER(C.c_int32)], C.c_int),
        "pvt_scene_variant": ([vp], C.c_int),
        "pvt_scene_lean_check": ([C.POINTER(PvtSceneTables), C.POINTER(PvtIndexTables), C.POINTER(PvtPhaseTables),
                                  C.POINTER(PvtSurfaceTables), C.POINTER(PvtFieldTables), C.POINTER(PvtMapTables),
                                  C.POINTER(C.c_int32)], C.c_int),
        "pvt_scene_counters": ([vp, C.POINTER(C.c_uint64), C.c_int], C.c_int),
        "pvt_scene_clock": ([vp, C.POINTER(C.c_uint64)], C.c_int),
        "pvt_scene_launch_span": ([vp, vp, C.POINTER(C.c_uint64)], C.c_int),
        "pvt_node_grid_plan": (
            [C.POINTER(PvtSceneTables), C.POINTER(C.c_int32), C.POINTER(C.c_double), C.POINTER(C.c_double),
             C.POINTER(C.c_double), C.POINTER(C.c_int32), C.POINTER(C.c_uint64), C.c_int64], C.c_int),
    }
    for name in names:
        argtypes, restype = sigs[name]
        fn = getattr(lib, name)
        fn.argtypes = argtypes
        fn.restype = restype
    return sigs


ABI_SYMBOLS = (
    "pvt_abi_version", "pvt_last_error", "pvt_device_count", "pvt_scene_create",
    "pvt_scene_set_emitter", "pvt_scene_destroy", "pvt_trace_device", "pvt_trace_bundle",
    "pvt_emit_device", "pvt_selftest_math", "pvt_scene_launch_info", "pvt_mesh_bvh_check",
    "pvt_trace_bundle_multi", "pvt_shard_range", "pvt_trace_device_records", "pvt_unpack_records_device",
    "pvt_scene_carry_pending", "pvt_last_multi_reduce", "pvt_node_grid_plan", "pvt_scene_carry_discard", "pvt_scene_trim",
    "pvt_scene_counters", "pvt_scene_clock", "pvt_scene_launch_span", "pvt_release_cached_memory",
    "pvt_scene_create_ex", "pvt_scene_create_phase", "pvt_scene_create_rough", "pvt_scene_create_field",
    "pvt_scene_create_maps", "pvt_scene_map_slots", "pvt_scene_variant", "pvt_scene_lean_check",
)
VARIANT_NAMES = ("lean", "w4", "grid", "rough", "mesh")

_lib = None
ABI_VERSION = 13
FLAG_NO_LOG_PREFILL = 1
FLAG_CARRY_OUT = 2


def library_built():
    return os.path.exists(LIB_PATH)


def _preload_torch_hip_runtime():
    import importlib.util

    try:
        spec = importlib.util.find_spec("torch")
    except (ImportError, ValueError):
        spec = None
    if spec is None or not spec.origin:
        return None
    path = os.path.join(os.path.dirname(spec.origin), "lib", "libamdhip64.so")
    if not os.path.exists(path):
        return None
    try:
        return C.CDLL(path, mode=C.RTLD_GLOBAL)
    except OSError:
        return None


def load_library():
    global _lib
    if _lib is None:
        if not library_built():
            raise EngineUnavailableError(
                f"{LIB_PATH} is not built; run `python -c 'import __graft_entry__ as g; g.build()'`"
                " (hipcc --offload-arch=gfx950)."
            )
        _preload_torch_hip_runtime()
        lib = C.CDLL(LIB_PATH)
        declare_signatures(lib, ABI_SYMBOLS)
        if lib.pvt_abi_version() != ABI_VERSION:
            raise EngineUnavailableError(
                f"{LIB_PATH} implements ABI v{lib.pvt_abi_version()}, this package needs v{ABI_VERSION}; "
                "rebuild it (`python -c 'import __graft_entry__ as g; g.build()'`)."
            )
        _lib = lib
    return _lib


def check(code, what):
    if code == 0:
        return
    lib = load_library()
    detail = lib.pvt_last_error()
    detail = detail.decode() if detail else ""
    if code == -2:
        raise ValueError("Engine supports at most 128 geometry nodes.")
    if code == -1:
        raise ValueError(f"{what}: invalid argument ({detail})")
    raise EngineUnavailableError(f"{what} failed with code {code}: {detail}")


def device_count():
    return int(load_library().pvt_device_count())


def is_available():
    if not library_built():
        return False
    try:
        return device_count() > 0
    except OSError:
        return False


def shard_range(n_rays, shard, n_shards, align=1):
    lib = load_library()
    a, b = C.c_int64(), C.c_int64()
    check(lib.pvt_shard_range(int(n_rays), int(shard), int(n_shards), int(align), C.byref(a), C.byref(b)),
          "pvt_shard_range")
    return a.value, b.value


def selftest_math(fn, x, device=0):
    lib = load_library()
    x = np.ascontiguousarray(x, dtype=np.float64)
    y = np.empty_like(x)
    check(lib.pvt_selftest_math(int(fn), x.ctypes.data, y.ctypes.data, x.size, int(device)),
          "pvt_selftest_math")
    return y


def mesh_bvh_check(compiled, node):
    lib = load_library()
    st, keep = scene_tables_struct(compiled)
    out = [C.c_int32(0) for _ in range(3)]
    check(lib.pvt_mesh_bvh_check(C.byref(st), int(node), *(C.byref(v) for v in out)), "pvt_mesh_bvh_check")
    del keep
    return tuple(int(v.value) for v in out)


def lean_check(compiled):
    return lean_kind(compiled) != 0


def lean_kind(compiled):
    lib = load_library()
    st, keep = scene_tables_struct(compiled)
    others = [f(compiled) for f in (index_tables_struct, phase_tables_struct, surface_tables_struct, field_tables_struct,
                                    map_tables_struct)]
    lean = C.c_int32(0)
    check(lib.pvt_scene_lean_check(C.byref(st), *(None if s is None else C.byref(s) for s, _ in others), C.byref(lean)),
          "pvt_scene_lean_check")
    del keep, others
    return int(lean.value)


def node_grid_plan(compiled):
    import numpy as np

    lib = load_library()
    st, keep = scene_tables_struct(compiled)
    dims = (C.c_int32 * 3)()
    lo, cell = (C.c_double * 3)(), (C.c_double * 3)()
    guard, odd = C.c_double(0.0), C.c_int32(0)
    check(lib.pvt_node_grid_plan(C.byref(st), dims, lo, cell, C.byref(guard), C.byref(odd), None, 0), "pvt_node_grid_plan")
    if dims[0] == 0:
        del keep
        return None
    cells = int(dims[0]) * int(dims[1]) * int(dims[2])
    masks = np.zeros((cells, 2), dtype=np.uint64)
    check(lib.pvt_node_grid_plan(C.byref(st), dims, lo, cell, C.byref(guard), C.byref(odd),
                                 masks.ctypes.data_as(C.POINTER(C.c_uint64)), masks.size), "pvt_node_grid_plan")
    del keep
    return {"dims": tuple(int(v) for v in dims), "lo": np.array(list(lo)), "cell": np.array(list(cell)),
            "guard": float(guard.value), "odd": bool(odd.value), "masks": masks}


class DeviceScene:

    def __init__(self, compiled, device=0, emitter=None):
        self.lib = load_library()
        if device_count() <= 0:
            raise EngineUnavailableError("No HIP device visible; the engine has no CPU path.")
        self.compiled = compiled
        self.device = int(device)
        st, keep = scene_tables_struct(compiled)
        xt, xkeep = index_tables_struct(compiled)
        pt, pkeep = phase_tables_struct(compiled)
        rt, rkeep = surface_tables_struct(compiled)
        ft, fkeep = field_tables_struct(compiled)
        mt, mkeep = map_tables_struct(compiled)
        handle = C.c_void_p()
        if mt is not None:
            check(self.lib.pvt_scene_create_maps(C.byref(st), None if xt is None else C.byref(xt),
                                                 None if pt is None else C.byref(pt), None if rt is None else C.byref(rt),
                                                 None if ft is None else C.byref(ft), C.byref(mt), self.device,
                                                 C.byref(handle)),
                  "pvt_scene_create_maps")
        elif ft is not None:
            check(self.lib.pvt_scene_create_field(C.byref(st), None if xt is None else C.byref(xt),
                                                  None if pt is None else C.byref(pt), None if rt is None else C.byref(rt),
                                                  C.byref(ft), self.device, C.byref(handle)),
                  "pvt_scene_create_field")
        elif rt is not None:
            check(self.lib.pvt_scene_create_rough(C.byref(st), None if xt is None else C.byref(xt),
                                                  None if pt is None else C.byref(pt), C.byref(rt), self.device,
                                                  C.byref(handle)),
                  "pvt_scene_create_rough")
        elif pt is None:
            check(self.lib.pvt_scene_create_ex(C.byref(st), None if xt is None else C.byref(xt), self.device,
                                               C.byref(handle)),
                  "pvt_scene_create_ex")
        else:
            check(self.lib.pvt_scene_create_phase(C.byref(st), None if xt is None else C.byref(xt), C.byref(pt),
                                                  self.device, C.byref(handle)),
                  "pvt_scene_create_phase")
        self.handle = handle
        self.has_emitter = False
        self._stream_owners = {}
        self._owners_lock = threading.Lock()
        if emitter is not None:
            self.set_emitter(emitter)

    def set_emitter(self, emitter):
        st, keep = emitter_tables_struct(emitter)
        check(self.lib.pvt_scene_set_emitter(self.handle, C.byref(st)), "pvt_scene_set_emitter")
        self.has_emitter = True

    def close(self):
        if getattr(self, "handle", None):
            self.lib.pvt_scene_destroy(self.handle)
            self.handle = None

    def __del__(self):
        try:
            self.close()
        except Exception:
            pass

    def counters(self, reset=False):
        import torch

        torch.cuda.synchronize(self.device)
        out = (C.c_uint64 * 4)()
        check(self.lib.pvt_scene_counters(self.handle, out, 1 if reset else 0), "pvt_scene_counters")
        it, ls, fused, waves = (int(v) for v in out)
        return {"wave_iterations": it, "lane_steps": ls, "fused_exits": fused, "waves": waves,
                "steps": ls + fused, "lane_utilisation": ls / (64.0 * it) if it else 0.0}

    def clock(self):
        import torch

        torch.cuda.synchronize(self.device)
        out = (C.c_uint64 * 2)()
        check(self.lib.pvt_scene_clock(self.handle, out), "pvt_scene_clock")
        cycles, ticks = int(out[0]), int(out[1])
        return {"shader_cycles": cycles, "ticks_100mhz": ticks, "shader_clock_mhz": 100.0 * cycles / ticks if ticks else 0.0}

    def launch_span_ms(self, stream=None):
        import torch

        if stream is None:
            stream = torch.cuda.current_stream(self.device).cuda_stream
        out = (C.c_uint64 * 2)()
        check(self.lib.pvt_scene_launch_span(self.handle, C.c_void_p(stream), out), "pvt_scene_launch_span")
        return (int(out[1]) - int(out[0])) * 1e-5

    def launch_info(self):
        g, b, l = C.c_int32(), C.c_int32(), C.c_int32()
        check(self.lib.pvt_scene_launch_info(self.handle, C.byref(g), C.byref(b), C.byref(l)),
              "pvt_scene_launch_info")
        variant = int(self.lib.pvt_scene_variant(self.handle))
        if variant < 0:
            check(variant, "pvt_scene_variant")
        return {"grid": g.value, "block": b.value, "lds_bytes": l.value, "variant": VARIANT_NAMES[variant]}

    def new_tallies(self, sets=1):
        import torch

        dev = torch.device("cuda", self.device)
        c = self.compiled
        nrec = max(int(c.rec_node.shape[0]), 1)
        nbins = max(int(c.total_bins) + int(getattr(c, "map_slots", 0)), 1)
        ints = torch.zeros(sets * (2 * nrec + nbins), dtype=torch.int64, device=dev)
        sums = torch.zeros(sets * nrec * 8, dtype=torch.float64, device=dev)
        return {
            "rec_distinct": ints[:nrec],
            "rec_crossings": ints[nrec:2 * nrec],
            "rec_sums": sums,
            "rec_bins": ints[2 * nrec:],
            "_ints": ints,
            "_sums": sums,
            "sets": sets, "stride_i64": 2 * nrec + nbins, "stride_f64": nrec * 8,
        }

    def new_event_log(self, n_rays, record_every, max_events):
        import torch

        dev = torch.device("cuda", self.device)
        nrec = num_recorded(n_rays, record_every)
        rows = nrec * max_events
        return {"counts": torch.empty(max(nrec, 1), dtype=torch.int32, device=dev),
                "rows": torch.empty((max(rows, 1), RECORD_WORDS), dtype=torch.int64, device=dev)}

    def new_event_columns(self, n_rays, record_every, max_events):
        import torch

        dev = torch.device("cuda", self.device)
        nrec = num_recorded(n_rays, record_every)
        rows = nrec * max_events
        log = {"counts": torch.empty(max(nrec, 1), dtype=torch.int32, device=dev)}
        tmap = {np.uint8: torch.uint8, np.int32: torch.int32, np.float64: torch.float64}
        for name, dtype, width in EVENT_LOG_COLUMNS:
            log[name] = torch.empty(max(rows, 1) * width, dtype=tmap[dtype], device=dev)
        return log

    @staticmethod
    def _columns_struct(log):
        el = PvtEventLog()
        el.counts = addr_ptr(log["counts"].data_ptr(), C.c_int32)
        for name, dtype, _ in EVENT_LOG_COLUMNS:
            setattr(el, name, addr_ptr(log[name].data_ptr(), _CTYPE_OF[np.dtype(dtype)]))
        return el

    def unpack_records(self, records, columns, n_recorded, max_events, prefill=True, stream=None):
        import torch

        if stream is None:
            stream = torch.cuda.current_stream(self.device).cuda_stream
        rec = PvtEventRecords(addr_ptr(records["counts"].data_ptr(), C.c_int32),
                              addr_ptr(records["rows"].data_ptr(), C.c_uint64))
        el = self._columns_struct(columns)
        check(self.lib.pvt_unpack_records_device(C.byref(rec), int(n_recorded), int(max_events), C.byref(el),
                                                 1 if prefill else 0, C.c_void_p(stream)), "pvt_unpack_records_device")

    def trace(self, rays, n_rays, seed, tallies, log=None, ray_offset=0, emit_seed=0,
              record_every=0, maxsteps=1000, max_events=128, emit_method=0, stream=None,
              workgroups_per_cu=0, tally_bundle=0, log_prefill=True, carry_out=False):
        import torch

        if stream is None:
            stream = torch.cuda.current_stream(self.device).cuda_stream
        if tally_bundle:
            need = -(-int(n_rays) // int(tally_bundle))
            if record_every > 0:
                raise ValueError("tally_bundle needs record_every == 0")
            if tallies.get("sets", 1) < need:
                raise ValueError(f"{need} tally sets needed, the buffers hold {tallies.get('sets', 1)}")
            if need > 1 and not ("stride_i64" in tallies and "stride_f64" in tallies):
                raise ValueError("tally_bundle needs the buffers of new_tallies(sets=...) (stride_i64 / stride_f64)")
        params = trace_params(n_rays, seed, ray_offset, emit_seed, record_every, maxsteps,
                              max_events, emit_method, workgroups_per_cu, tally_bundle,
                              tallies.get("stride_i64", 0) if tally_bundle else 0,
                              tallies.get("stride_f64", 0) if tally_bundle else 0,
                              (0 if log_prefill else FLAG_NO_LOG_PREFILL) | (FLAG_CARRY_OUT if carry_out else 0))
        tl = PvtTallies(
            addr_ptr(tallies["rec_distinct"].data_ptr(), C.c_int64),
            addr_ptr(tallies["rec_crossings"].data_ptr(), C.c_int64),
# ... 97 lines not shown
```

Baseline: 4.016 billion.

## Add solo kernel variant specialized for two-node world-plus-box scenes

Adds a host-side proof (prove_solo) that detects scenes with exactly one box inside a lazy root, no recorders, and finite critical-cosine thresholds, then launches a new trace_kernel_solo_w4 specialization. In that variant the node count is a compile-time constant, node and class table reads become uniform scalar selects, the intersection loop is unrolled for box then root, and several flag checks are fixed at compile time. The aim is to cut per-step table indexing, branching and register pressure for the common single-slab LSC case. The cost is another kernel instantiation, more code to keep in sync, and a narrow eligibility test that may not match the benchmark scene.

```diff
diff --git a/include/pvtrace_hip.h b/include/pvtrace_hip.h
--- a/include/pvtrace_hip.h
+++ b/include/pvtrace_hip.h
@@ -319,6 +319,12 @@
                          const PvtSurfaceTables* surface_tables, const PvtFieldTables* field_tables,
                          const PvtMapTables* map_tables, int32_t* lean);
 
+enum { PVT_LEAN_LEVEL_OFF = 0, PVT_LEAN_LEVEL_SEARCHED = 1, PVT_LEAN_LEVEL_EVEN = 2, PVT_LEAN_LEVEL_SOLO = 3 };
+int pvt_scene_lean_level(PvtScene* scene);
+int pvt_scene_solo_check(const PvtSceneTables* tables, const PvtIndexTables* index_tables, const PvtPhaseTables* phase_tables,
+                         const PvtSurfaceTables* surface_tables, const PvtFieldTables* field_tables,
+                         const PvtMapTables* map_tables, const double* thresholds, int32_t* solo);
+
 int pvt_mesh_bvh_check(const PvtSceneTables* tables, int32_t node, int32_t* n_bvh_nodes,
                        int32_t* n_leaves, int32_t* depth);
 
diff --git a/pvtrace_amd/csrc/pvt_scene_pack.h b/pvtrace_amd/csrc/pvt_scene_pack.h
--- a/pvtrace_amd/csrc/pvt_scene_pack.h
+++ b/pvtrace_amd/csrc/pvt_scene_pack.h
@@ -300,6 +300,7 @@
     bool exit_observed = false, fuse_exit = false, grid = false, hist_reads_position = false;
     bool lean_ok = false;
     bool lean_even = false;
+    bool solo_ok = false;
     int grid_dims[3] = {0, 0, 0};
     std::vector<pvt::BvhNode> bvh_nodes;
     std::vector<pvt::MeshTri> bvh_tris;
@@ -1058,6 +1059,30 @@
     p->lean_even = ok && all_even;
 }
 
+void prove_solo(const PvtSceneTables* t, PackedScene* p, const double* thresholds = nullptr) {
+    const Lay& lay = p->lay;
+    const std::vector<double>& gd = p->gd;
+    const std::vector<int>& gi = p->gi;
+    bool ok = p->lean_ok && t->n_nodes == 2 && lay.by_node == 1 && lay.n_cls == 2 && lay.crit_d >= 0 && lay.ccrit_d >= 0 &&
+              lay.ncls_d == lay.ccrit_d + 4 + RT &&
+              p->lazy_root != 0 && p->fuse_exit && !p->exit_observed && (t->root_id == 0 || t->root_id == 1);
+    if (ok) {
+        const int root = t->root_id, box = 1 - root;
+        auto geom = [&](int n) {
+            unsigned long long bits;
+            std::memcpy(&bits, &gd[(size_t)n * ND + ND_BITS], 8);
+            return (int)(((unsigned int)bits >> 8) & 0xffu);
+        };
+        if (geom(box) != PVT_GEOM_BOX || geom(root) != (p->lazy_root == 1 ? PVT_GEOM_BOX : PVT_GEOM_SPHERE)) ok = false;
+        if (gi[(size_t)root * NI + NI_CCOUNT] != 0) ok = false;
+        for (int k = 0; k < 4; k++) {
+            const double cc = thresholds ? thresholds[k] : gd[(size_t)lay.ccrit_d + k];
+            if (!(cc == cc)) ok = false;
+        }
+    }
+    p->solo_ok = ok;
+}
+
 void pack_fields(const PvtSceneTables* t, const PvtFieldTables* fr, PackedScene* p) {
     p->fd.clear();
     if (!fr || fr->n_nodes == 0) return;
@@ -1169,6 +1194,7 @@
     pack_maps(t, mp, p);
     prove_shortcuts(t, p);
     prove_lean(t, p);
+    prove_solo(t, p);
     return PVT_OK;
 }
 
diff --git a/pvtrace_amd/csrc/pvt_trace.hip b/pvtrace_amd/csrc/pvt_trace.hip
--- a/pvtrace_amd/csrc/pvt_trace.hip
+++ b/pvtrace_amd/csrc/pvt_trace.hip
@@ -107,6 +107,8 @@
     bool hist_reads_position = false;
     bool lean_ok = false;
     bool lean_even = false;
+    bool solo_ok = false;
+    bool last_solo = false;
     int last_variant = -1;
 };
 
@@ -260,6 +262,23 @@
     return hipGetLastError();
 }
 
+hipError_t launch_solo_variant(bool even, bool emit, int grid, size_t lds, hipStream_t st, const KArgs& a) {
+#if PVT_DEV_VARIANTS
+    if (emit) return hipErrorNotSupported;
+    if (even) hipLaunchKernelGGL((trace_kernel_solo_w4<false, true>), dim3(grid), dim3(kBlock), lds, st, a);
+    else hipLaunchKernelGGL((trace_kernel_solo_w4<false, false>), dim3(grid), dim3(kBlock), lds, st, a);
+#else
+    if (even) {
+        if (emit) hipLaunchKernelGGL((trace_kernel_solo_w4<true, true>), dim3(grid), dim3(kBlock), lds, st, a);
+        else hipLaunchKernelGGL((trace_kernel_solo_w4<false, true>), dim3(grid), dim3(kBlock), lds, st, a);
+    } else {
+        if (emit) hipLaunchKernelGGL((trace_kernel_solo_w4<true, false>), dim3(grid), dim3(kBlock), lds, st, a);
+        else hipLaunchKernelGGL((trace_kernel_solo_w4<false, false>), dim3(grid), dim3(kBlock), lds, st, a);
+    }
+#endif
+    return hipGetLastError();
+}
+
 template <bool RECORD, int TAB_LDS, int SEENW>
 hipError_t launch_variant(bool emit, int grid, size_t lds, hipStream_t st, const KArgs& a) {
     if (a.rough_d >= 0 || a.fd != nullptr || a.md != nullptr) return launch_rough_variant<RECORD, TAB_LDS, SEENW>(emit, grid, lds, st, a);
@@ -299,6 +318,9 @@
 template <bool RECORD, int TAB_LDS>
 hipError_t launch_seen(int n_rec, int lean, bool emit, int grid, size_t lds, hipStream_t st, const KArgs& a) {
     if constexpr (TAB_LDS == 1 && PVT_DEV_VARIANTS != 2) {
+        if constexpr (!RECORD) {
+            if (lean >= kLeanSoloSearched) return launch_solo_variant(lean == kLeanSoloEven, emit, grid, lds, st, a);
+        }
         if (lean) return launch_lean_variant<RECORD>(lean == kLeanEven, emit, grid, lds, st, a);
     }
     if (n_rec <= 64) return launch_variant<RECORD, TAB_LDS, 1>(emit, grid, lds, st, a);
@@ -506,7 +528,10 @@
     }
     hipError_t e;
     s->last_variant = variant_of(s, tab_lds);
-    const int lean = s->last_variant != PVT_VARIANT_LEAN ? kLeanOff : (s->lean_even ? kLeanEven : kLeanSearched);
+    s->last_solo = s->last_variant == PVT_VARIANT_LEAN && s->solo_ok && !record && a.lazy_root != 0 && a.fuse_exit != 0;
+    const int lean = s->last_variant != PVT_VARIANT_LEAN ? kLeanOff
+                     : s->last_solo ? (s->lean_even ? kLeanSoloEven : kLeanSoloSearched)
+                                    : (s->lean_even ? kLeanEven : kLeanSearched);
     if (record) {
         e = tab_lds ? launch_seen<true, 1>(s->n_rec, lean, emit, (int)grid, lds, st, a)
             : lp.small_lds ? launch_seen<true, 2>(s->n_rec, lean, emit, (int)grid, lds, st, a)
@@ -644,6 +669,7 @@
     s->grid = packed.grid;
     s->lean_ok = packed.lean_ok && !getenv("PVT_NO_LEAN");
     s->lean_even = s->lean_ok && packed.lean_even;
+    s->solo_ok = s->lean_ok && packed.solo_ok && !getenv("PVT_NO_SOLO");
     for (int a = 0; a < 3; a++) s->grid_dims[a] = packed.grid_dims[a];
     hipDeviceProp_t prop;
     HIP_TRY(hipGetDeviceProperties(&prop, device));
@@ -908,6 +934,26 @@
     const int rc = pack_scene(t, x, ph, rs, fr, mp, &packed);
     if (rc != PVT_OK) return rc;
     *lean = packed.lean_ok ? (packed.lean_even ? 2 : 1) : 0;
+    return PVT_OK;
+}
+
+int pvt_scene_lean_level(PvtScene* s) {
+    if (!s) return fail(PVT_ERR_INVALID, "null scene");
+    const bool lean = s->last_variant >= 0 ? s->last_variant == PVT_VARIANT_LEAN : variant_of(s, plan_lds(s, false).tab_lds) == PVT_VARIANT_LEAN;
+    if (!lean) return PVT_LEAN_LEVEL_OFF;
+    const bool solo = s->last_variant >= 0 ? s->last_solo : (s->solo_ok && !s->exit_observed && s->lazy_root != 0 && s->fuse_exit);
+    return solo ? PVT_LEAN_LEVEL_SOLO : (s->lean_even ? PVT_LEAN_LEVEL_EVEN : PVT_LEAN_LEVEL_SEARCHED);
+}
+
+int pvt_scene_solo_check(const PvtSceneTables* t, const PvtIndexTables* x, const PvtPhaseTables* ph, const PvtSurfaceTables* rs,
+                         const PvtFieldTables* fr, const PvtMapTables* mp, const double* thresholds, int32_t* solo) {
+    if (!t || !solo) return fail(PVT_ERR_INVALID, "null argument");
+    if (t->n_nodes <= 0 || t->n_nodes > PVT_MAX_NODES || t->n_recorders > PVT_MAX_RECORDERS) return fail(PVT_ERR_INVALID, "bad argument");
+    PackedScene packed;
+    const int rc = pack_scene(t, x, ph, rs, fr, mp, &packed);
+    if (rc != PVT_OK) return rc;
+    if (thresholds) prove_solo(t, &packed, thresholds);
+    *solo = packed.solo_ok && !getenv("PVT_NO_SOLO") ? 1 : 0;
     return PVT_OK;
 }
 
diff --git a/pvtrace_amd/csrc/pvt_trace_kernel.h b/pvtrace_amd/csrc/pvt_trace_kernel.h
--- a/pvtrace_amd/csrc/pvt_trace_kernel.h
+++ b/pvtrace_amd/csrc/pvt_trace_kernel.h
@@ -218,7 +218,7 @@
 constexpr double kRcpCcm = 1.0 / kCcm;
 
 enum { kInterpAny = 0, kInterpEven, kInterpByGuide, kInterpNoHist };
-enum { kLeanOff = 0, kLeanSearched, kLeanEven };
+enum { kLeanOff = 0, kLeanSearched, kLeanEven, kLeanSoloSearched, kLeanSoloEven };
 template <int TAB_LDS, int KIND = kInterpAny>
 __device__ __forceinline__ double interp_clamped(const Tables<TAB_LDS>& T, double x, int xs, int ys, int n,
                                                  int guide, double scale, int hist, double rcp,
@@ -854,16 +854,20 @@
           int LEAN = 0>
 __device__ __forceinline__ void trace_body(const KArgs& A, int tail_total = 0, unsigned int tail_lds = 0u) {
     static_assert(!LEAN || (!MESH && !GRID && !ROUGH && TAB_LDS == 1 && SEENW == 1), "the lean variants: plain scenes only");
+    constexpr bool kSolo = LEAN >= kLeanSoloSearched;
+    constexpr bool kLeanEvenGrids = LEAN == kLeanEven || LEAN == kLeanSoloEven;
+    static_assert(!kSolo || !RECORD, "the solo variants: tally launches only");
     extern __shared__ double smem_of_kernel[];
     double* const smem = TAIL ? (double*)(__attribute__((address_space(3))) double*)(unsigned long long)tail_lds
                               : (double*)smem_of_kernel;
-    constexpr int kAbsKind = LEAN == kLeanEven ? kInterpEven : LEAN ? kInterpNoHist : kInterpAny;
-    constexpr int kCdfKind = LEAN == kLeanEven ? kInterpByGuide : LEAN ? kInterpNoHist : kInterpAny;
+    constexpr int kAbsKind = kLeanEvenGrids ? kInterpEven : LEAN ? kInterpNoHist : kInterpAny;
+    constexpr int kCdfKind = kLeanEvenGrids ? kInterpByGuide : LEAN ? kInterpNoHist : kInterpAny;
     auto held = [](int v) __attribute__((always_inline)) -> int {
         if constexpr (TAIL) asm volatile("" : "+s"(v));
         return v;
     };
-    const int k_root = held(A.root), k_maxsteps = held(A.maxsteps), k_nodes = held(A.n_nodes);
+    const int k_root = held(A.root), k_maxsteps = held(A.maxsteps), k_nodes = kSolo ? 2 : held(A.n_nodes);
+    const int k_box = kSolo ? 1 - k_root : 0;
 #if PVT_TIMELINE
     unsigned long long tl_t[6] = {(unsigned long long)wall_clock64(), 0, 0, 0, 0, 0};
     unsigned long long tl_iters = 0;
@@ -895,6 +899,10 @@
         if constexpr (LEAN != kLeanOff) {
             if (bit == UF_COATED || bit == UF_CTAB || bit == UF_DISP || bit == UF_ROUGH || bit == UF_FIELD || bit == UF_VMAP) return false;
             if (bit == UF_BY_NODE) return true;
+        }
+        if constexpr (kSolo) {
+            if (bit == UF_FUSE_EXIT || bit == UF_CRIT) return true;
+            if (bit == UF_TAIL_LAZY1 || bit == UF_TAIL_LAZY2) return false;
         }
         unsigned int f = uflags;
         asm volatile("" : "+s"(f));
@@ -948,7 +956,24 @@
 
     Tables<TAB_LDS> T{(CDoubles)A.gd, (CInts)A.gi, TAB_LDS != 0 ? lds_d : A.gd, TAB_LDS != 0 ? lds_i : A.gi, A.gd, A.gi};
 
-    auto node_bits = [&](int node) -> unsigned long long { return pvt_d2u(T.dv(node * ND + ND_BITS)); };
+    auto node_d = [&](int node, int word) __attribute__((always_inline)) -> double {
+        if constexpr (kSolo) {
+            const double of_0 = T.du(word), of_1 = T.du(ND + word);
+            return node == 0 ? of_0 : of_1;
+        }
+        return T.dv(node * ND + word);
+    };
+    auto node_i = [&](int node, int word) __attribute__((always_inline)) -> int {
+        if constexpr (kSolo) {
+            const int of_0 = T.iu(word), of_1 = T.iu(NI + word);
+            return node == 0 ? of_0 : of_1;
+        }
+        return T.iv(node * NI + word);
+    };
+    auto node_bits = [&](int node) -> unsigned long long {
+        if constexpr (kSolo) return pvt_d2u(node_d(node, ND_BITS));
+        else return pvt_d2u(T.dv(node * ND + ND_BITS));
+    };
     auto node_ident = [](unsigned long long bits) -> bool { return LEAN || (bits & 1ull) != 0; };
     auto node_geom = [](unsigned long long bits) -> int {
         const int g = (int)(((unsigned int)bits >> 8) & 0xffu);
@@ -1060,6 +1085,21 @@
         const int np = (int)T.dv(q + 2 * k + 1);
         if (np == 0) return n;
         return index_table_n(tab + (int)T.dv(q + 2 * k), np, wl);
+    };
+    constexpr int kSoloClasses = 4 + RT;
+    auto class_rn = [&](int k) __attribute__((always_inline)) -> double {
+        if constexpr (kSolo) {
+            const double of_0 = T.du(L.ccrit_d + kSoloClasses + 1), of_1 = T.du(L.ccrit_d + kSoloClasses + 3);
+            return k == 0 ? of_0 : of_1;
+        }
+        return T.dv(L.ncls_d + k * 2 + 1);
+    };
+    auto pair_cc = [&](int kc, int ka) __attribute__((always_inline)) -> double {
+        if constexpr (kSolo) {
+            const double c00 = T.du(L.ccrit_d), c01 = T.du(L.ccrit_d + 1), c10 = T.du(L.ccrit_d + 2), c11 = T.du(L.ccrit_d + 3);
+            return kc == 0 ? (ka == 0 ? c00 : c01) : (ka == 0 ? c10 : c11);
+        }
+        return T.dv(L.ccrit_d + kc * L.n_cls + ka);
     };
     int rec_slot = -1;
     Seen<SEENW> seen;
@@ -1478,7 +1518,7 @@
                 int rot = -1;
                 const bool lazy_exact = TAIL && !MESH && (uf(UF_TAIL_LAZY1) || uf(UF_TAIL_LAZY2));
                 const int lazy_root = MESH ? 0 : (lazy_exact ? (uf(UF_TAIL_LAZY1) ? 1 : 2)
-                                                              : (RECORD ? 0 : (uf(UF_LAZY1) ? 1 : (uf(UF_LAZY2) ? 2 : 0))));
+                                                              : (RECORD ? 0 : (uf(UF_LAZY1) ? 1 : ((kSolo || uf(UF_LAZY2)) ? 2 : 0))));
                 auto fold_by_key = [&](double t, int node, int& nl, double& tfirst) __attribute__((always_inline)) {
                     const double a1 = t1, a2 = t2, tf = tfirst;
                     const int m1 = n1, m2 = n2, have = nhits, l = nl;
@@ -1639,7 +1679,68 @@
                         if (test) visit(node);
                     }
                 }
-                for (int k = 0; k < (GRID ? 0 : k_nodes); k++) {
+                if constexpr (kSolo) {
+                    const double inv0 = rcp_normal(dir.x), inv1 = rcp_normal(dir.y), inv2 = rcp_normal(dir.z);
+                    {
+                        const int node = k_box;
+                        int hn = node * ND;
+                        asm volatile("" : "+s"(hn));
+                        const double tx = T.du(hn + ND_T), ty = T.du(hn + ND_T + 1), tz = T.du(hn + ND_T + 2);
+                        const double g0 = T.du(hn + ND_PARAMS), g1 = T.du(hn + ND_PARAMS + 1), g2 = T.du(hn + ND_PARAMS + 2);
+                        const V3 o{pos.x + tx, pos.y + ty, pos.z + tz};
+                        int nl = 0;
+                        double tfirst = 0.0;
+                        auto fold = [&](double t) __attribute__((always_inline)) {
+                            if (nl == 0) tfirst = t;
+                            nl += 1;
+                            if (nhits == 0) { t1 = t; n1 = node; }
+                            else if (t < t1) { t2 = t1; n2 = n1; t1 = t; n1 = node; }
+                            else if (n2 < 0 || t < t2) { t2 = t; n2 = node; }
+                            nhits += 1;
+                        };
+                        shape_hits((int)PVT_GEOM_BOX, g0, g1, g2, o, dir, inv0, inv1, inv2, fold);
+                        if (nl == 1 && tfirst < cbest) { cbest = tfirst; cnode = node; }
+                    }
+                    {
+                        const int node = k_root;
+                        int hn = node * ND;
+                        asm volatile("" : "+s"(hn));
+                        const double tx = T.du(hn + ND_T), ty = T.du(hn + ND_T + 1), tz = T.du(hn + ND_T + 2);
+                        const double g0 = T.du(hn + ND_PARAMS), g1 = T.du(hn + ND_PARAMS + 1), g2 = T.du(hn + ND_PARAMS + 2);
+                        const V3 o{pos.x + tx, pos.y + ty, pos.z + tz};
+                        int nl = 0;
+                        double tfirst = 0.0;
+                        bool root_known = false;
+                        double bound;
+                        if (lazy_root == 1) {
+                            const double mx = 0.5 * g0 - pvt_fabs(o.x), my = 0.5 * g1 - pvt_fabs(o.y), mz = 0.5 * g2 - pvt_fabs(o.z);
+                            bound = __builtin_fmin(__builtin_fmin(mx, my), mz);
+                        } else {
+                            bound = (g0 * g0 - dot3(o, o)) * A.lazy_k;
+                        }
+                        const bool undecided = !(bound > 0.0) || (nhits > 0 && !(t1 < bound)) || (nhits >= 2 && !(t2 < bound)) ||
+                                               (cnode >= 0 && !(cbest < bound));
+                        if (!undecided) {
+                            if (nhits == 0) { t1 = bound; n1 = node; }
+                            else if (nhits == 1) { t2 = INFINITY; n2 = node; }
+                            nhits += 1;
+                            if (cnode < 0) cnode = node;
+                            root_known = true;
+                        }
+                        auto fold = [&](double t) __attribute__((always_inline)) {
+                            if (nl == 0) tfirst = t;
+                            nl += 1;
+                            if (nhits == 0) { t1 = t; n1 = node; }
+                            else if (t < t1) { t2 = t1; n2 = n1; t1 = t; n1 = node; }
+                            else if (n2 < 0 || t < t2) { t2 = t; n2 = node; }
+                            nhits += 1;
+                        };
+                        if (!root_known)
+                            shape_hits(lazy_root == 1 ? (int)PVT_GEOM_BOX : (int)PVT_GEOM_SPHERE, g0, g1, g2, o, dir, inv0, inv1, inv2, fold);
+                        if (nl == 1 && !root_known && tfirst < cbest) { cbest = tfirst; cnode = node; }
+                    }
+                }
+                for (int k = 0; k < ((GRID || kSolo) ? 0 : k_nodes); k++) {
                     const int node = !lazy_root ? k : (k == k_nodes - 1 ? k_root : (k < k_root ? k : k + 1));
                     const int hn = node * ND;
                     const double tx = T.du(hn + ND_T), ty = T.du(hn + ND_T + 1), tz = T.du(hn + ND_T + 2);
@@ -1957,23 +2058,40 @@
         double alpha = 0.0, pre0 = 0.0, n_container = 1.0;
         int cbase = 0, ccount = 0, crec = 0;
         if (pend) {
-            n_container = T.dv(container * ND + ND_N);
+            n_container = kSolo ? node_d(container, ND_N) : T.dv(container * ND + ND_N);
             if (uf(UF_DISP)) n_container = index_at(container, n_container);
-            cbase = T.iv(container * NI + NI_CSTART); ccount = T.iv(container * NI + NI_CCOUNT);
+            if constexpr (kSolo) {
+                cbase = node_i(container, NI_CSTART); ccount = node_i(container, NI_CCOUNT);
+            } else {
+                cbase = T.iv(container * NI + NI_CSTART); ccount = T.iv(container * NI + NI_CCOUNT);
+            }
             if (uf(UF_BY_NODE)) crec = cbase;
             else crec = T.iv(container * NI + NI_CREC);
             if constexpr (TAIL) {
                 const int hn = hit * ND;
-                hr_t = V3{T.dv(hn + ND_T), T.dv(hn + ND_T + 1), T.dv(hn + ND_T + 2)};
-                hr_g = V3{T.dv(hn + ND_PARAMS), T.dv(hn + ND_PARAMS + 1), T.dv(hn + ND_PARAMS + 2)};
-                hr_bits = pvt_d2u(T.dv(hn + ND_BITS));
-                hr_surf = T.iv(hit * NI + NI_SURF);
+                if constexpr (kSolo) {
+                    hr_t = V3{node_d(hit, ND_T), node_d(hit, ND_T + 1), node_d(hit, ND_T + 2)};
+                    hr_g = V3{node_d(hit, ND_PARAMS), node_d(hit, ND_PARAMS + 1), node_d(hit, ND_PARAMS + 2)};
+                    hr_bits = node_bits(hit);
+                    hr_surf = node_i(hit, NI_SURF);
+                } else {
+                    hr_t = V3{T.dv(hn + ND_T), T.dv(hn + ND_T + 1), T.dv(hn + ND_T + 2)};
+                    hr_g = V3{T.dv(hn + ND_PARAMS), T.dv(hn + ND_PARAMS + 1), T.dv(hn + ND_PARAMS + 2)};
+                    hr_bits = pvt_d2u(T.dv(hn + ND_BITS));
+                    hr_surf = T.iv(hit * NI + NI_SURF);
+                }
                 if (adjacent >= 0) {
                     int kc = container, ka = adjacent;
                     if (!uf(UF_BY_NODE)) { kc = T.iv(container * NI + NI_NCLS); ka = T.iv(adjacent * NI + NI_NCLS); }
-                    hr_n2 = T.dv(adjacent * ND + ND_N);
-                    hr_rn2 = T.dv(L.ncls_d + ka * 2 + 1);
-                    hr_cc = uf(UF_CRIT) ? T.dv(L.ccrit_d + kc * L.n_cls + ka) : __builtin_nan("");
+                    if constexpr (kSolo) {
+                        hr_n2 = node_d(adjacent, ND_N);
+                        hr_rn2 = class_rn(ka);
+                        hr_cc = pair_cc(kc, ka);
+                    } else {
+                        hr_n2 = T.dv(adjacent * ND + ND_N);
+                        hr_rn2 = T.dv(L.ncls_d + ka * 2 + 1);
+                        hr_cc = uf(UF_CRIT) ? T.dv(L.ccrit_d + kc * L.n_cls + ka) : __builtin_nan("");
+                    }
                     if (uf(UF_DISP)) { hr_n2 = index_at(adjacent, hr_n2); hr_rn2 = div_normal(1.0, hr_n2); }
                 }
             }
@@ -2180,7 +2298,10 @@
             const int tr = t_node * ND + ND_T;
             const unsigned long long tb = node_bits(t_node);
             if (node_ident(tb))
-                return V3{pos.x + T.dv(tr), pos.y + T.dv(tr + 1), pos.z + T.dv(tr + 2)};
+            {
+                if constexpr (kSolo) return V3{pos.x + node_d(t_node, ND_T), pos.y + node_d(t_node, ND_T + 1), pos.z + node_d(t_node, ND_T + 2)};
+                else return V3{pos.x + T.dv(tr), pos.y + T.dv(tr + 1), pos.z + T.dv(tr + 2)};
+            }
             const int m = node_rot(tb) + RT_W2L;
             return V3{T.dv(m + 0) * pos.x + T.dv(m + 1) * pos.y + T.dv(m + 2) * pos.z + T.dv(tr),
                       T.dv(m + 3) * pos.x + T.dv(m + 4) * pos.y + T.dv(m + 5) * pos.z + T.dv(tr + 1),
@@ -2191,6 +2312,7 @@
             const int gt = kHoist ? node_geom(hr_bits) : node_geom(node_bits(t_node));
             auto param = [&](int a) -> double {
                 if constexpr (kHoist) return a == 0 ? hr_g.x : (a == 1 ? hr_g.y : hr_g.z);
+                if constexpr (kSolo) return node_d(t_node, ND_PARAMS + a);
                 return T.dv(gp + a);
             };
             if (MESH && gt == PVT_GEOM_MESH) {
@@ -2251,7 +2373,7 @@
             }
         }
         if (alive && t_normal) t_cos = ac_arg;
-        const bool fres = surf && (kHoist ? hr_surf : T.iv(ev_hit * NI + NI_SURF)) == PVT_SURF_FRESNEL;
+        const bool fres = surf && (kHoist ? hr_surf : (kSolo ? node_i(ev_hit, NI_SURF) : T.iv(ev_hit * NI + NI_SURF))) == PVT_SURF_FRESNEL;
         const double c1 = ac_arg, s1 = fres ? sqrt1m2_normal(ac_arg) : 0.0;
 
         PVT_MARK(4);
@@ -2259,12 +2381,12 @@
             const int hit = ev_hit, container = ev_container, adjacent = ev_adjacent;
             double r = 0.0, n1 = 0.0, n2 = 0.0, rn2 = 0.0;
             if (fres) {
-                n1 = kHoist ? n_container : T.dv(container * ND + ND_N);
-                n2 = kHoist ? hr_n2 : T.dv(adjacent * ND + ND_N);
+                n1 = kHoist ? n_container : (kSolo ? node_d(container, ND_N) : T.dv(container * ND + ND_N));
+                n2 = kHoist ? hr_n2 : (kSolo ? node_d(adjacent, ND_N) : T.dv(adjacent * ND + ND_N));
                 int kc = container, ka = adjacent;
                 if (!kHoist && !uf(UF_BY_NODE)) { kc = T.iv(container * NI + NI_NCLS); ka = T.iv(adjacent * NI + NI_NCLS); }
                 const int ncls_d = L.ncls_d, n_cls = L.n_cls;
-                rn2 = kHoist ? hr_rn2 : T.dv(ncls_d + ka * 2 + 1);
+                rn2 = kHoist ? hr_rn2 : (kSolo ? class_rn(ka) : T.dv(ncls_d + ka * 2 + 1));
                 if (!kHoist && uf(UF_DISP)) {
                     n1 = n_container;
                     n2 = index_at(adjacent, n2);
@@ -2272,8 +2394,8 @@
                 }
                 bool tir;
                 const bool crit_tab = uf(UF_CRIT);
-                const double cc = kHoist ? hr_cc : (crit_tab ? T.dv(L.ccrit_d + kc * n_cls + ka) : __builtin_nan(""));
-                if (cc == cc) tir = c1 < cc;
+                const double cc = kHoist ? hr_cc : (crit_tab ? (kSolo ? pair_cc(kc, ka) : T.dv(L.ccrit_d + kc * n_cls + ka)) : __builtin_nan(""));
+                if (kSolo || cc == cc) tir = c1 < cc;
                 else {
                     if (kHoist && !uf(UF_BY_NODE)) { kc = T.iv(container * NI + NI_NCLS); ka = T.iv(adjacent * NI + NI_NCLS); }
                     const double crit = crit_tab ? T.dv(L.crit_d + kc * n_cls + ka) : __builtin_nan("");
@@ -2390,6 +2512,18 @@
             }
             if (!RECORD && !MESH && uf(UF_FUSE_EXIT) && !terminal && count < k_maxsteps &&
                 (ev_kind == PVT_EV_REFLECT ? container == k_root : adjacent == k_root)) {
+                if constexpr (kSolo && !kHoist) {
+                    int box_at = k_box * ND;
+                    asm volatile("" : "+s"(box_at));
+                    const V3 lp{pos.x + T.du(box_at + ND_T), pos.y + T.du(box_at + ND_T + 1), pos.z + T.du(box_at + ND_T + 2)};
+                    const double h = 0.5 * (pvt_fabs(nrm.x) * T.du(box_at + ND_PARAMS) + pvt_fabs(nrm.y) * T.du(box_at + ND_PARAMS + 1) +
+                                            pvt_fabs(nrm.z) * T.du(box_at + ND_PARAMS + 2));
+                    const double g = h - dot3(nrm, lp), dn = dot3(nrm, dir);
+                    if (dn > 0.0 && g <= (0.5 * kEps) * dn) {
+                        terminal = true;
+                        c_fused += 1u;
+                    }
+                } else {
                 const V3 lp = local_point();
                 const int gp = hit * ND + ND_PARAMS;
                 const double h = kHoist ? 0.5 * (pvt_fabs(nrm.x) * hr_g.x + pvt_fabs(nrm.y) * hr_g.y + pvt_fabs(nrm.z) * hr_g.z)
@@ -2398,6 +2532,7 @@
                 if (dn > 0.0 && g <= (0.5 * kEps) * dn) {
                     terminal = true;
                     c_fused += 1u;
+                }
                 }
             }
         }
@@ -2591,4 +2726,9 @@
     trace_body<RECORD, 1, 1, EMIT, false, false, false, false, EVEN ? kLeanEven : kLeanSearched>(A);
 }
 
-}
+template <bool EMIT, bool EVEN>
+__global__ void __launch_bounds__(kBlock) __attribute__((amdgpu_waves_per_eu(4, 4))) trace_kernel_solo_w4(KArgs A) {
+    trace_body<false, 1, 1, EMIT, false, false, false, false, EVEN ? kLeanSoloEven : kLeanSoloSearched>(A);
+}
+
+}
diff --git a/pvtrace_amd/engine/native.py b/pvtrace_amd/engine/native.py
--- a/pvtrace_amd/engine/native.py
+++ b/pvtrace_amd/engine/native.py
@@ -401,6 +401,10 @@
         "pvt_scene_lean_check": ([C.POINTER(PvtSceneTables), C.POINTER(PvtIndexTables), C.POINTER(PvtPhaseTables),
                                   C.POINTER(PvtSurfaceTables), C.POINTER(PvtFieldTables), C.POINTER(PvtMapTables),
                                   C.POINTER(C.c_int32)], C.c_int),
+        "pvt_scene_lean_level": ([vp], C.c_int),
+        "pvt_scene_solo_check": ([C.POINTER(PvtSceneTables), C.POINTER(PvtIndexTables), C.POINTER(PvtPhaseTables),
+                                  C.POINTER(PvtSurfaceTables), C.POINTER(PvtFieldTables), C.POINTER(PvtMapTables),
+                                  C.POINTER(C.c_double), C.POINTER(C.c_int32)], C.c_int),
         "pvt_scene_counters": ([vp, C.POINTER(C.c_uint64), C.c_int], C.c_int),
         "pvt_scene_clock": ([vp, C.POINTER(C.c_uint64)], C.c_int),
         "pvt_scene_launch_span": ([vp, vp, C.POINTER(C.c_uint64)], C.c_int),
@@ -425,7 +429,9 @@
     "pvt_scene_counters", "pvt_scene_clock", "pvt_scene_launch_span", "pvt_release_cached_memory",
     "pvt_scene_create_ex", "pvt_scene_create_phase", "pvt_scene_create_rough", "pvt_scene_create_field",
     "pvt_scene_create_maps", "pvt_scene_map_slots", "pvt_scene_variant", "pvt_scene_lean_check",
+    "pvt_scene_lean_level", "pvt_scene_solo_check",
 )
+LEAN_LEVEL_NAMES = ("off", "searched", "even", "solo")
 VARIANT_NAMES = ("lean", "w4", "grid", "rough", "mesh")
 
 _lib = None
@@ -542,6 +548,19 @@
           "pvt_scene_lean_check")
     del keep, others
     return int(lean.value)
+
+
+def solo_check(compiled, thresholds=None):
+    lib = load_library()
+    st, keep = scene_tables_struct(compiled)
+    others = [f(compiled) for f in (index_tables_struct, phase_tables_struct, surface_tables_struct, field_tables_struct,
+                                    map_tables_struct)]
+    solo = C.c_int32(0)
+    table = None if thresholds is None else (C.c_double * 4)(*[float(v) for v in thresholds])
+    check(lib.pvt_scene_solo_check(C.byref(st), *(None if s is None else C.byref(s) for s, _ in others), table, C.byref(solo)),
+          "pvt_scene_solo_check")
+    del keep, others
+    return bool(solo.value)
 
 
 def node_grid_plan(compiled):
@@ -662,7 +681,11 @@
         variant = int(self.lib.pvt_scene_variant(self.handle))
         if variant < 0:
             check(variant, "pvt_scene_variant")
-        return {"grid": g.value, "block": b.value, "lds_bytes": l.value, "variant": VARIANT_NAMES[variant]}
+        level = int(self.lib.pvt_scene_lean_level(self.handle))
+        if level < 0:
+            check(level, "pvt_scene_lean_level")
+        return {"grid": g.value, "block": b.value, "lds_bytes": l.value, "variant": VARIANT_NAMES[variant],
+                "lean_level": LEAN_LEVEL_NAMES[level]}
 
     def new_tallies(self, sets=1):
         import torch
```

Result: faster. 4.134 billion (median of 6 runs) (+2.9%).
